# catid/tonk

Measured on AMD Instinct MI355X. Metric: Siamese FEC encode+decode GiB/s (device-resident), 1/2/4/8 MI355X, higher is better.
Workload: dtype u8

## Files before the change

### tonk_amd/csrc/decoder.cpp

```cpp
#include "decoder.h"
#include "prof.h"

#include <algorithm>
#include <stdlib.h>
#include <string.h>

namespace tamd {

static const size_t kMergeAbove = 48;

static inline uint32_t popcount64(uint64_t x) { return (uint32_t)__builtin_popcountll(x); }

static inline uint32_t bits_popcount(uint64_t w, uint32_t start, uint32_t end) {
    if (start >= end) return 0;
    const uint32_t n = end - start;
    const uint64_t mask = n >= 64 ? ~0ull : ((1ull << n) - 1);
    return popcount64((w >> start) & mask);
}
static inline uint32_t bits_first_clear(uint64_t w, uint32_t start) {
    const uint64_t v = (~w) >> start;
    if (start >= 64 || v == 0) return 64;
    return start + (uint32_t)__builtin_ctzll(v);
}
static inline uint32_t bits_first_set(uint64_t w, uint32_t start) {
    const uint64_t v = w >> start;
    if (start >= 64 || v == 0) return 64;
    return start + (uint32_t)__builtin_ctzll(v);
}

Decoder::Decoder(Context* ctx, uint32_t row_bytes, HostRelease release, void* user)
    : ctx_(ctx), row_bytes_(row_bytes), release_(release), user_(user) {
    ctx_->attach(this);
}

Decoder::~Decoder() {
    for (Subwindow* s : subs_) {
        for (unsigned i = 0; i < kSubwindow; ++i) drop_original(s->orig[i]);
        delete s;
    }
    subs_.clear();
    for (size_t i = 0; i < segs_.size(); ++i) release_segment(segs_[i], 0, segs_[i].count);
    segs_.clear();
    Recovery* r = head_;
    while (r) { Recovery* n = r->next; free_recovery(r); r = n; }
    for (Recovery* g : graveyard_) delete g;
    graveyard_.clear();
    for (Recovery* g : pool_) delete g;
    pool_.clear();
    pre_flush();
    for (unsigned l = 0; l < kLanes; ++l) lanes_[l].sums.release(ctx_->rows);
    ctx_->detach(this);
}

void Decoder::pre_flush() {
    for (unsigned l = 0; l < kLanes; ++l) lanes_[l].sums.flush(ctx_->rows, ctx_->pb, ctx_->ex);
}

void Decoder::drop_original(StoredOriginal& o) {
    if (o.owned) ctx_->rows.free_deferred(o.row);
    if (o.host && release_) release_(o.host, user_);
    o.row = kNoRow;
    o.bytes = 0;
    o.owned = 0;
    o.host = nullptr;
    o.run = 0;
}

void Decoder::free_recovery(Recovery* r) {
    if (r->row != kNoRow) ctx_->rows.free_deferred(r->row);
    r->row = kNoRow;
    graveyard_.push_back(r);
}

void Decoder::read_original(RowId row, uint32_t len, uint8_t coef, Sym& out) const {
    ctx_->ex.append(ctx_->rows, row, len, coef, out);
}

void Decoder::release_segment(const Segment& s, uint32_t from, uint32_t n) {
    if (s.owned)
        for (uint32_t j = from; j < from + n; ++j) ctx_->rows.free_deferred(s.row(j));
}

void Decoder::append(uint32_t e0, const RowId* rows, uint32_t k, uint32_t framed_bytes, uint32_t header_bytes,
                     uint8_t owned, uint64_t layout) {
    const RowTable& rt = ctx_->rows;
    uint32_t e = e0, col = to_column(e0);
    if (k >= 2 && col + k - 1 < kColumnPeriod && col != 0 && (layout || consecutive_handles(rows, k))) {
        const uint32_t o0 = layout ? (uint32_t)(layout >> 32) : rt.offset(rows[0]);
        const uint32_t o1 = layout ? o0 + (uint32_t)layout : rt.offset(rows[1]);
        const uint32_t stride = o1 - o0;
        if (o1 > o0 && (layout || rt.affine(rows[0], k, stride))) {
            Segment* last = segs_.empty() ? nullptr : &segs_.back();
            const bool cont = last && last->end() == e0 + base_ && last->bytes == framed_bytes &&
                              last->header_bytes == header_bytes && last->owned == owned &&
                              rows[0] == last->row0 + last->count && o0 > last->off0 &&
                              (last->count == 1 ? o0 - last->off0 == stride
                                                : last->stride == stride && o0 == last->off(last->count));
            if (cont) {
                last->stride = stride;
                last->count += k;
            } else {
                Segment sg;
                sg.first = e0 + base_;
                sg.count = k;
                sg.row0 = rows[0];
                sg.off0 = o0;
                sg.stride = stride;
                sg.bytes = framed_bytes;
                sg.column0 = col;
                sg.header_bytes = (uint8_t)header_bytes;
                sg.owned = owned;
                segs_.push_back(sg);
            }
            const uint32_t id = seg_base_ + (uint32_t)segs_.size() - 1;
            for (uint32_t x = e0; x < e0 + k;) {
                const uint32_t bit = x % kSubwindow;
                const uint32_t n = std::min(kSubwindow - bit, e0 + k - x);
                std::fill_n(subs_[x / kSubwindow]->seg + bit, n, id);
                x += n;
            }
            return;
        }
    }
    uint32_t j = 0;
    while (j < k) {
        Segment* last = segs_.empty() ? nullptr : &segs_.back();
        const uint32_t e_abs = e + base_;
        const RowId r = rows[j];
        const uint32_t off = rt.offset(r);
        const bool cont = last && last->end() == e_abs && last->bytes == framed_bytes &&
                          last->header_bytes == header_bytes && last->owned == owned && r == last->row0 + last->count &&
                          off > last->off0 && col != 0 && (last->count == 1 || off == last->off(last->count));
        if (cont) {
            if (last->count == 1) last->stride = off - last->off0;
            ++last->count;
        } else {
            Segment sg;
            sg.first = e_abs;
            sg.count = 1;
            sg.row0 = r;
            sg.off0 = off;
            sg.bytes = framed_bytes;
            sg.column0 = col;
            sg.header_bytes = (uint8_t)header_bytes;
            sg.owned = owned;
            segs_.push_back(sg);
            last = &segs_.back();
        }
        const uint32_t id = seg_base_ + (uint32_t)segs_.size() - 1;
        subs_[e / kSubwindow]->seg[e % kSubwindow] = id;
        ++e;
        ++j;
        col = col_inc(col);
        if (last->count >= 2) {
            uint32_t n = last->count;
            while (j < k && rows[j] == last->row0 + n && col != 0 && rt.offset(rows[j]) == last->off(n)) {
                subs_[e / kSubwindow]->seg[e % kSubwindow] = id;
                ++e;
                ++j;
                ++n;
                col = col_inc(col);
            }
            last->count = n;
        }
    }
}


bool Decoder::mark_got(uint32_t column) {
    const uint32_t e = to_element(column);
    if (invalid_element(e)) { disabled_ = true; return false; }
    Subwindow* s = subs_[e / kSubwindow];
    s->got_count++;
    s->got |= 1ull << (e % kSubwindow);
    return e == next_expected_;
}

uint32_t Decoder::range_lost(uint32_t start, uint32_t end) {
    if (start >= end) return 0;
    uint32_t lost = 0;
    uint32_t sub = start / kSubwindow;
    const uint32_t bit = start % kSubwindow;
    if (bit > 0) {
        uint32_t bit_end = bit + end - start;
        if (bit_end > kSubwindow) bit_end = kSubwindow;
        lost += (bit_end - bit) - bits_popcount(subs_[sub]->got, bit, bit_end);
        ++sub;
    }
    const uint32_t sub_end = end / kSubwindow;
    for (uint32_t i = sub; i < sub_end; ++i) lost += kSubwindow - subs_[i]->got_count;
    if (sub_end >= sub) {
        const uint32_t last_bits = end - sub_end * kSubwindow;
        if (last_bits > 0) lost += last_bits - bits_popcount(subs_[sub_end]->got, 0, last_bits);
    }
    return lost;
}

uint32_t Decoder::find_next_lost(uint32_t start) {
    if (start >= count_) return count_;
    const uint32_t sub_end = (count_ + kSubwindow - 1) / kSubwindow;
    uint32_t sub = start / kSubwindow, bit = start % kSubwindow;
    while (sub < sub_end) {
        if (subs_[sub]->got_count < kSubwindow) {
            bit = bits_first_clear(subs_[sub]->got, bit);
            if (bit < kSubwindow) {
                uint32_t e = sub * kSubwindow + bit;
                if (e > count_) e = count_;
                return e;
            }
        }
        bit = 0;
        ++sub;
    }
    return count_;
}

uint32_t Decoder::find_next_got(uint32_t start) {
    if (start >= count_) return count_;
    const uint32_t sub_end = (count_ + kSubwindow - 1) / kSubwindow;
    uint32_t sub = start / kSubwindow, bit = start % kSubwindow;
    while (sub < sub_end) {
        if (subs_[sub]->got_count > 0) {
            bit = bits_first_set(subs_[sub]->got, bit);
            if (bit < kSubwindow) {
                uint32_t e = sub * kSubwindow + bit;
                if (e > count_) e = count_;
                return e;
            }
        }
        bit = 0;
        ++sub;
    }
    return count_;
}

void Decoder::iterate_next_expected(uint32_t start) {
    if (next_expected_ >= count_) return;
    next_expected_ = find_next_lost(start);
}

bool Decoder::grow_window(uint32_t end) {
    const uint32_t needed = (end + kLanes + kSubwindow - 1) / kSubwindow;
    while (subs_.size() < needed) subs_.push_back(new Subwindow());
    if (end > count_) count_ = end;
    return true;
}

Result Decoder::add_original(uint32_t packet_num, RowId row, uint32_t framed_bytes, uint32_t header_bytes,
                             uint32_t payload_bytes, void* host, bool* took, bool borrowed) {
    *took = false;
    if (disabled_) return kDisabled;
    const uint32_t e = to_element(packet_num);
    if (col_delta_negative(e)) {
        stats_[6]++;
        return kDuplicateData;
    }
    const bool at_end = e >= count_;
    grow_window(e + 1);
    Subwindow* s = subs_[e / kSubwindow];
    const uint32_t bit = e % kSubwindow;
    if ((s->got >> bit) & 1u) {
        stats_[6]++;
        return kDuplicateData;
    }
    if (at_end && !host) {
        append(e, &row, 1, framed_bytes, header_bytes, borrowed ? 0 : 1);
    } else {
        StoredOriginal& o = s->orig[bit];
        drop_original(o);
        o.row = row;
        o.off = ctx_->rows.offset(row);
        o.bytes = framed_bytes;
        o.column = packet_num;
        o.header_bytes = (uint8_t)header_bytes;
        o.owned = borrowed ? 0 : 1;
        o.host = host;
        o.run = 0;
        o.stride = 0;
        if (o.owned || host) s->held |= 1ull << bit;
        s->singles |= 1ull << bit;
    }
    *took = !borrowed;
    s->got_count++;
    s->got |= 1ull << bit;

    if (e == next_expected_) {
        iterate_next_expected(e + 1);
        list_delete_before(next_expected_);
    }
    if (e >= cr_.element_start && e < cr_.next_check_start) checked_reset();

    stats_[0]++;
    stats_[1] += payload_bytes;
    return kSuccess;
}

bool Decoder::add_run_inorder(uint32_t col0, const RowId* rows, uint32_t k, uint32_t framed_bytes,
                              uint32_t header_bytes, uint32_t payload_bytes, bool borrowed, uint64_t layout) {
    if (disabled_ || has_recovered_ || !k) return false;
    const uint32_t e0 = to_element(col0);
    if (col_delta_negative(e0) || e0 < count_) return false;
    if (head_ && (next_expected_ >= e0 || check_recovery_possible())) return false;
    grow_window(e0 + k);
    append(e0, rows, k, framed_bytes, header_bytes, borrowed ? 0 : 1, layout);
    for (uint32_t e = e0; e < e0 + k;) {
        const uint32_t bit = e % kSubwindow;
        const uint32_t n = std::min(kSubwindow - bit, e0 + k - e);
        Subwindow* s = subs_[e / kSubwindow];
        s->got |= (n == 64 ? ~0ull : ((1ull << n) - 1)) << bit;
        s->got_count += n;
        e += n;
    }
    if (e0 == next_expected_) next_expected_ = find_next_lost(e0 + k);
    if (std::max(e0, cr_.element_start) < std::min(e0 + k, cr_.next_check_start)) checked_reset();
    stats_[0] += k;
    stats_[1] += (uint64_t)payload_bytes * k;
    return true;
}

bool Decoder::plug_sum_holes(uint32_t element_start) {
    for (uint32_t column : recovered_columns_) {
        const uint32_t e = to_element(column);
        if (invalid_element(e)) continue;
        const uint32_t lane = column % kLanes;
        const uint32_t lane_start = next_lane_element(element_start, lane);
        LaneSum& sum = lanes_[lane];
        if (e >= lane_start && e < sum.element_end) {
            const StoredOriginal& o = elem(e);
            if (o.bytes <= 0) return false;
            sum.sums.grow(o.bytes);
            sum.sums.accumulate(ctx_->rows, o.row, o.bytes, column);
        }
    }
    recovered_columns_.clear();
    return true;
}

void Decoder::reset_sums(uint32_t element_start) {
    for (unsigned l = 0; l < kLanes; ++l) {
        const uint32_t ls = next_lane_element(element_start, l);
        LaneSum& sum = lanes_[l];
        sum.element_start = ls;
        sum.element_end = ls;
        sum.sums.reset(ctx_->rows);
    }
    recovered_columns_.clear();
}

bool Decoder::start_sums(uint32_t element_start, uint32_t buffer_bytes) {
    for (unsigned l = 0; l < kLanes; ++l) {
        const uint32_t ls = next_lane_element(element_start, l);
        LaneSum& sum = lanes_[l];
        if (sum.sums.bytes == 0) {
            sum.element_end = ls;
        } else if (sum.element_start != ls) {
            sum.element_end = ls;
            sum.sums.reset(ctx_->rows);
        }
        sum.element_start = ls;
        sum.sums.grow(buffer_bytes);
    }
    if (!recovered_columns_.empty() && !plug_sum_holes(element_start)) return false;
    return true;
}

LaneSums& Decoder::get_lane(uint32_t lane, uint32_t element_end) {
    LaneSum& sum = lanes_[lane];
    uint32_t e = sum.element_end;
    if (e >= element_end) return sum.sums;
    do {
        const uint32_t id = seg_id(e);
        if (id != kSingle) {
            const Segment& sg = segs_[id - seg_base_];
            const uint32_t j = e + base_ - sg.first;
            uint32_t stop = sg.end() - base_;
            if (stop > element_end) stop = element_end;
            const uint32_t n = (stop - 1 - e) / kLanes + 1;
            sum.sums.grow(sg.bytes);
            sum.sums.accumulate_run_level0(sg.row(j), sg.off(j), sg.bytes, col_add(sg.column0, j), n, sg.stride * kLanes);
            e += n * kLanes;
            continue;
        }
        const StoredOriginal& o = elem(e);
        if (o.bytes > 0) {
            sum.sums.grow(o.bytes);
            if (ctx_->rows.level(o.row) == 0) sum.sums.accumulate_level0(o.row, ctx_->rows.offset(o.row), o.bytes, o.column);
            else sum.sums.accumulate(ctx_->rows, o.row, o.bytes, o.column);
        }
        e += kLanes;
    } while (e < element_end);
    sum.element_end = e;
    return sum.sums;
}

void Decoder::list_walk(ListWalk& w) const {
    w.min_start = ~0u;
    w.max_bytes = 0;
    w.seen_sum = false;
    w.target_start = w.target_count = 0;
    w.min_fse = ~0u;
    w.invalid = false;
    for (const Recovery* r = head_; r; r = r->next) {
        const uint32_t sc = r->meta.SumCount, cs = r->meta.ColumnStart;
        if (sc > kCauchyThreshold) {
            if (!w.seen_sum) {
                w.target_start = cs;
                w.target_count = sc;
                w.target_end = r->element_end;
                w.seen_sum = true;
            } else if (cs != w.target_start || sc < w.target_count) {
                const uint32_t fse = to_element(cs);
                if (invalid_element(fse)) {
                    w.invalid = true;
                    return;
                }
                if (w.min_fse > fse) w.min_fse = fse;
            }
        }
        if (w.min_start > r->element_start) w.min_start = r->element_start;
        if (w.max_bytes < r->bytes) w.max_bytes = r->bytes;
    }
}

void Decoder::remove_elements() {
    if (next_expected_ < kRemoveThreshold) return;

    uint32_t first_kept = 0, target_start = 0, target_count = 0, initial_bytes = 0;
    bool seen_sum = false;
    const Recovery* r = head_;
    if (!r) {
        const RecoveryMeta m = last_meta_;
        const uint32_t end = to_element(m.ColumnStart + m.SumCount);
        if (col_delta_negative(end) || end < m.LDPCCount) { disabled_ = true; return; }
        first_kept = end - m.LDPCCount;
        target_start = m.ColumnStart;
        target_count = m.SumCount;
        initial_bytes = last_bytes_;
        if (m.SumCount > kCauchyThreshold) seen_sum = true;
    } else {
        if (!(walk_.valid && walk_.gen == list_gen_ && walk_.column_start == column_start_ && walk_.count == count_)) {
            list_walk(walk_);
            walk_.valid = true;
            walk_.gen = list_gen_;
            walk_.column_start = column_start_;
            walk_.count = count_;
        }
        if (walk_.invalid) { disabled_ = true; return; }
        first_kept = walk_.min_start < walk_.min_fse ? walk_.min_start : walk_.min_fse;
        initial_bytes = walk_.max_bytes;
        seen_sum = walk_.seen_sum;
        target_start = walk_.target_start;
        target_count = walk_.target_count;
    }
    if (first_kept < kRemoveThreshold) return;

    const uint32_t first_kept_sub = first_kept / kSubwindow;
    const uint32_t removed = first_kept_sub * kSubwindow;

    if (seen_sum) {
        uint32_t sum_elem = to_element(target_start);
        if (sum_column_start_ != target_start || sum_column_count_ > target_count) {
            if (invalid_element(sum_elem)) { disabled_ = true; return; }
            reset_sums(sum_elem);
            sum_column_start_ = target_start;
            sum_column_count_ = target_count;
        } else {
            if (invalid_element(sum_elem)) sum_elem = 0;
            if (!start_sums(sum_elem, initial_bytes)) { disabled_ = true; return; }
        }
        for (unsigned l = 0; l < kLanes; ++l) {
            get_lane(l, removed);
            LaneSum& sum = lanes_[l];
            if (sum.element_start >= removed) sum.element_start -= removed;
            else sum.element_start = l;
            sum.element_end -= removed;
        }
    } else {
        sum_column_count_ = 0;
    }

    for (uint32_t i = 0; i < first_kept_sub; ++i) {
        Subwindow* s = subs_[i];
        for (uint64_t m = s->held; m; m &= m - 1) drop_original(s->orig[__builtin_ctzll(m)]);
        for (uint64_t m = s->singles | s->held; m; m &= m - 1)
            memset((void*)&s->orig[__builtin_ctzll(m)], 0, sizeof(StoredOriginal));
        memset(s->seg, 0xff, sizeof(s->seg));
        s->got = 0;
        s->got_count = 0;
        s->held = 0;
        s->singles = 0;
    }
    std::rotate(subs_.begin(), subs_.begin() + first_kept_sub, subs_.end());
    const uint32_t cut = base_ + removed;
    while (!segs_.empty() && segs_.front().end() <= cut) {
        release_segment(segs_.front(), 0, segs_.front().count);
        segs_.pop_front(1);
        ++seg_base_;
    }
    if (!segs_.empty() && segs_.front().first < cut) {
        Segment& f = segs_.front();
        const uint32_t d = cut - f.first;
        release_segment(f, 0, d);
        f.first = cut;
        f.count -= d;
        f.row0 += d;
        f.off0 += d * f.stride;
        f.column0 = col_add(f.column0, d);
    }
    base_ = cut;

    count_ -= removed;
    column_start_ = to_column(removed);
    next_expected_ -= removed;

    ++list_gen_;
    for (Recovery* q = head_; q; q = q->next) {
        q->element_end -= removed;
        q->element_start -= removed;
    }
    checked_decrement(removed);
    prev_next_check_start_ = prev_next_check_start_ > removed ? prev_next_check_start_ - removed : 0;
}


void Decoder::list_insert(Recovery* rec, bool out_of_order) {
    Recovery* prev = tail_;
    Recovery* next = nullptr;
    const uint32_t rs = rec->meta.ColumnStart, re = rec->element_end;
    if (ins_gen_ == list_gen_ && ins_end_ == re && ins_start_ == rs) {
        next = ins_last_;
        prev = ins_last_->prev;
    } else {
        for (; prev; next = prev, prev = prev->prev) {
            const uint32_t ps = prev->meta.ColumnStart, pe = prev->element_end;
            if (re >= pe) {
                if (re > pe) break;
                if (col_delta_negative(col_sub(rs, ps))) break;
            }
        }
    }
    const uint32_t sc = rec->meta.SumCount;
    const bool is_sum = sc > kCauchyThreshold;
    const bool same_target = is_sum && walk_.seen_sum && rs == walk_.target_start && sc == walk_.target_count;
    const bool walk_kept = walk_.valid && walk_.gen == list_gen_ && walk_.column_start == column_start_ &&
                           walk_.count == count_ &&
                           (!is_sum || !walk_.seen_sum || same_target || re > walk_.target_end);
    ins_last_ = rec;
    ins_end_ = re;
    ins_start_ = rs;
    ins_gen_ = ++list_gen_;
    if (walk_kept) {
        if (is_sum && !walk_.seen_sum) {
            walk_.seen_sum = true;
            walk_.target_start = rs;
            walk_.target_count = sc;
            walk_.target_end = re;
        } else if (is_sum && !same_target && (rs != walk_.target_start || sc < walk_.target_count)) {
            const uint32_t fse = to_element(rs);
            if (invalid_element(fse)) walk_.invalid = true;
            else if (walk_.min_fse > fse) walk_.min_fse = fse;
        }
        if (walk_.min_start > rec->element_start) walk_.min_start = rec->element_start;
        if (walk_.max_bytes < rec->bytes) walk_.max_bytes = rec->bytes;
        walk_.gen = list_gen_;
    }
    rec->next = next;
    rec->prev = prev;
    if (prev) prev->next = rec; else head_ = rec;
    if (next) next->prev = rec; else tail_ = rec;
    if (!prev || next) checked_reset();
    ++recovery_count_;
    if (!out_of_order) {
        last_meta_ = rec->meta;
        last_bytes_ = rec->bytes;
    }
}

void Decoder::lazy_write() {
    Recovery* r = lazy_from_;
    for (uint32_t i = 0; i < lazy_n_ && r; ++i, r = r->next) r->lost_count = lazy_lost_;
    lazy_n_ = 0;
    lazy_from_ = nullptr;
}

void Decoder::list_delete_before(uint32_t element) {
    if (lazy_n_) lazy_write();
    ++list_gen_;
    Recovery* r = head_;
    uint32_t deleted = 0;
    while (r) {
        if (r->element_end > element) break;
        Recovery* n = r->next;
        free_recovery(r);
        ++deleted;
        r = n;
    }
    head_ = r;
    if (r) {
        r->prev = nullptr;
        recovery_count_ -= deleted;
    } else {
        tail_ = nullptr;
        recovery_count_ = 0;
    }
}

void Decoder::checked_reset() {
    cr_ = Checked();
    lazy_n_ = 0;
    lazy_from_ = nullptr;
    matrix_reset();
    for (Recovery* r : graveyard_) pool_.push_back(r);
    graveyard_.clear();
}

void Decoder::checked_decrement(uint32_t n) {
    if (cr_.element_start < n || cr_.next_check_start < n) {
        checked_reset();
        return;
    }
    cr_.element_start -= n;
    cr_.next_check_start -= n;
}


void Decoder::matrix_reset() {
    mcols_.clear();
    mrows_.clear();
    pivots_.clear();
    mat_rows_ = mat_cols_ = 0;
    prev_next_check_start_ = 0;
    ge_resume_pivot_ = 0;
}

bool Decoder::matrix_resize(uint32_t rows, uint32_t cols, bool keep) {
    if (keep && rows <= mat_alloc_rows_ && cols <= mat_stride_) {
        mat_rows_ = rows;
        mat_cols_ = cols;
        return true;
    }
    const uint32_t arows = rows + 4;
    const uint32_t acols = (cols + 4 + 31) & ~31u;
    std::vector<uint8_t> m((size_t)arows * acols, 0);
    if (keep && mat_cols_ > 0) {
        const uint32_t copy = mat_cols_ < cols ? mat_cols_ : cols;
        for (uint32_t i = 0; i < mat_rows_; ++i)
            memcpy(&m[(size_t)i * acols], &mat_[(size_t)i * mat_stride_], copy);
    }
    mat_.swap(m);
    mat_alloc_rows_ = arows;
    mat_stride_ = acols;
    mat_rows_ = rows;
    mat_cols_ = cols;
    return true;
}

void Decoder::populate_columns(uint32_t old_cols, uint32_t new_cols) {
    if (old_cols >= new_cols) return;
    mcols_.resize(new_cols);
    uint32_t start = prev_next_check_start_;
    prev_next_check_start_ = cr_.next_check_start;
    const uint32_t end = cr_.next_check_start;
    if (start < cr_.element_start) start = cr_.element_start;
    const uint32_t sub_end = (end + kSubwindow - 1) / kSubwindow;
    uint32_t sub = start / kSubwindow, bit = start % kSubwindow, column = old_cols;
    while (sub < sub_end) {
        Subwindow* s = subs_[sub];
        if (s->got_count < kSubwindow) {
            do {
                bit = bits_first_clear(s->got, bit);
                if (bit >= kSubwindow) break;
                const uint32_t e = sub * kSubwindow + bit;
                MatCol& c = mcols_[column];
                c.column = to_column(e);
                c.orig = &s->orig[bit];
                c.cx = column_value(c.column);
                c.orig->column = column;
                s->singles |= 1ull << bit;
                if (++column >= new_cols) return;
            } while (++bit < kSubwindow);
        }
        bit = 0;
        ++sub;
    }
    disabled_ = true;
}

void Decoder::populate_rows(uint32_t old_rows, uint32_t new_rows) {
    if (old_rows >= new_rows) return;
    mrows_.resize(new_rows);
    Recovery* r = old_rows > 0 ? mrows_[old_rows - 1].rec->next : cr_.first;
    for (uint32_t i = old_rows; i < new_rows; ++i, r = r->next) {
        mrows_[i].rec = r;
        mrows_[i].used = false;
        mrows_[i].mcols = r->lost_count;
    }
}

bool Decoder::generate_matrix() {
    if (lazy_n_) lazy_write();
    const uint32_t columns = cr_.lost_count;
    const uint32_t rows = cr_.recovery_count;
    uint32_t old_rows = (uint32_t)mrows_.size();
    uint32_t old_cols = (uint32_t)mcols_.size();
    if (rows < old_rows || columns < old_cols) {
        matrix_reset();
        old_rows = old_cols = 0;
    }
    matrix_resize(rows, columns, old_rows != 0);
    populate_columns(old_cols, columns);
    populate_rows(old_rows, rows);
    if (disabled_) return false;

    const uint32_t start_row = columns <= old_cols ? old_rows : 0;
    for (uint32_t i = start_row; i < rows; ++i) {
        Recovery* rec = mrows_[i].rec;
        const RecoveryMeta m = rec->meta;
        const uint32_t start_col = i < old_rows ? old_cols : 0;
        if (m.SumCount <= kCauchyThreshold) {
            for (uint32_t j = start_col; j < columns; ++j) {
                const uint32_t column = mcols_[j].column;
                const uint32_t e = col_sub(column, m.ColumnStart);
                if (e >= m.SumCount) {
                    for (; j < columns; ++j) mat(i, j) = 0;
                    break;
                }
                mat(i, j) = m.Row == 0 ? 1 : cauchy_element(m.Row - 1, column % kCauchyMaxColumns);
            }
            continue;
        }
        const uint8_t rx = row_value(m.Row);
        for (uint32_t j = start_col; j < columns; ++j) {
            const uint32_t column = mcols_[j].column;
            const uint32_t e = col_sub(column, m.ColumnStart);
            if (e >= m.SumCount) {
                for (; j < columns; ++j) mat(i, j) = 0;
                break;
            }
            const uint8_t cx = mcols_[j].cx, cx2 = gf_sqr(cx);
            const unsigned op = row_opcode(column % kLanes, m.Row);
            uint8_t v = 0;
            if (op & 1) v ^= 1;
            if (op & 2) v ^= cx;
            if (op & 4) v ^= cx2;
            if (op & 8) v ^= rx;
            if (op & 16) v ^= gf_mul(cx, rx);
            if (op & 32) v ^= gf_mul(cx2, rx);
            mat(i, j) = v;
        }
        Pcg32 prng;
        prng.seed(m.Row, m.LDPCCount);
        const uint32_t es = rec->element_start;
        const uint32_t pairs = (m.LDPCCount + kPairRate - 1) / kPairRate;
        const FastMod ldpc_mod(m.LDPCCount);
        for (uint32_t k = 0; k < pairs; ++k) {
            const uint32_t e1 = es + ldpc_mod(prng.next());
            if (!got(e1)) {
                const uint32_t mc = elem(e1).column;
                if (mc >= columns) { disabled_ = true; return false; }
                if (mc >= start_col) mat(i, mc) ^= 1;
            }
            const uint32_t erx = es + ldpc_mod(prng.next());
            if (!got(erx)) {
                const uint32_t mc = elem(erx).column;
                if (mc >= columns) { disabled_ = true; return false; }
                if (mc >= start_col) mat(i, mc) ^= rx;
            }
        }
    }
    pivots_.resize(rows);
    for (uint32_t i = old_rows; i < rows; ++i) pivots_[i] = i;
    if (ge_resume_pivot_ > 0) resume_ge(old_rows, rows);
    return true;
}

bool Decoder::eliminate_row(uint32_t ge_row, uint32_t rem_row, uint32_t pivot_i, uint32_t column_end, uint8_t val_i) {
    uint8_t* rem = &mat_[(size_t)rem_row * mat_stride_];
    const uint8_t* ge = &mat_[(size_t)ge_row * mat_stride_];
    const uint8_t val_j = rem[pivot_i];
    if (val_j == 0) return false;
    const uint8_t y = gf_div(val_j, val_i);
    rem[pivot_i] = y;
    const uint8_t* ymul = g_gf.mul[y];
    for (uint32_t c = pivot_i + 1; c < column_end; ++c) rem[c] ^= ymul[ge[c]];
    return true;
}

void Decoder::resume_ge(uint32_t old_rows, uint32_t rows) {
    if (old_rows >= rows) return;
    for (uint32_t pi = 0; pi < ge_resume_pivot_; ++pi) {
        const uint32_t ri = pivots_[pi];
        const uint8_t val_i = mat(ri, pi);
        const uint32_t pcc = mrows_[ri].mcols;
        for (uint32_t nr = old_rows; nr < rows; ++nr) {
            if (eliminate_row(ri, nr, pi, pcc, val_i)) {
                if (mrows_[nr].mcols < pcc) mrows_[nr].mcols = pcc;
            }
        }
    }
}

bool Decoder::gaussian_elimination() {
    if (ge_resume_pivot_ > 0) return pivoted_ge(ge_resume_pivot_);
    const uint32_t columns = mat_cols_, rows = mat_rows_;
    for (uint32_t pi = 0; pi < columns; ++pi) {
        const uint8_t val_i = mat(pi, pi);
        if (val_i == 0) return pivoted_ge(pi);
        mrows_[pi].used = true;
        const uint32_t pcc = mrows_[pi].mcols;
        for (uint32_t pj = pi + 1; pj < rows; ++pj) eliminate_row(pi, pj, pi, pcc, val_i);
    }
    return true;
}

bool Decoder::pivoted_ge(uint32_t pivot_i) {
    const uint32_t columns = mat_cols_, rows = mat_rows_;
    uint32_t pj = pivot_i + 1;
    bool resume = true;
    for (; pivot_i < columns; ++pivot_i) {
        if (!resume) pj = pivot_i;
        resume = false;
        bool found = false;
        for (; pj < rows; ++pj) {
            const uint32_t rj = pivots_[pj];
            const uint8_t val_i = mat(rj, pivot_i);
            if (val_i == 0) continue;
            if (pivot_i != pj) std::swap(pivots_[pivot_i], pivots_[pj]);
            mrows_[rj].used = true;
            const uint32_t pcc = mrows_[rj].mcols;
            if (pivot_i >= columns - 1) return true;
            for (uint32_t pk = pivot_i + 1; pk < rows; ++pk) {
                const uint32_t rk = pivots_[pk];
                if (eliminate_row(rj, rk, pivot_i, pcc, val_i)) {
                    if (mrows_[rk].mcols < pcc) mrows_[rk].mcols = pcc;
                }
            }
            found = true;
            break;
        }
        if (!found) {
            ge_resume_pivot_ = pivot_i;
            return false;
        }
    }
    return true;
}


Result Decoder::add_recovery(RowId row, uint32_t total_bytes, const uint8_t* tail, const uint8_t* host,
                             bool* took) {
    *took = false;
    if (disabled_) return kDisabled;
    RecoveryMeta m;
    const uint32_t tl = total_bytes < 8 ? total_bytes : 8;
    const int footer = get_recovery_footer(tail, tl, m);
    if (footer < 0) { disabled_ = true; return kDisabled; }

    stats_[2]++;
    stats_[3] += total_bytes;

    const bool out_of_order = col_delta_negative(m.ColumnStart + m.SumCount - latest_column_);
    if (!out_of_order) latest_column_ = (m.ColumnStart + m.SumCount) % kColumnPeriod;

    uint32_t es, ee;
    if (count_ <= 0) {
        if (out_of_order) { stats_[9]++; return kSuccess; }
        column_start_ = m.ColumnStart;
        grow_window(m.SumCount);
        ee = m.SumCount;
        es = ee - m.LDPCCount;
    } else {
        ee = to_element(m.ColumnStart + m.SumCount);
        if (col_delta_negative(ee)) { stats_[9]++; return kSuccess; }
        if (ee < m.LDPCCount) { stats_[9]++; return kSuccess; }
        es = ee - m.LDPCCount;
        if (ee <= next_expected_) {
            if (out_of_order) { stats_[9]++; return kSuccess; }
            if (es >= kRemoveThreshold) {
                last_meta_ = m;
                last_bytes_ = total_bytes - (uint32_t)footer;
                remove_elements();
            }
            stats_[9]++;
            return kSuccess;
        }
        if (m.SumCount > kCauchyThreshold) {
            if (sum_column_count_ == 0 || sum_column_start_ != m.ColumnStart) {
                if (invalid_element(to_element(m.ColumnStart))) { stats_[9]++; return kSuccess; }
            }
        }
        grow_window(ee);
    }

    if (m.SumCount == 1) {
        if (!add_single_recovery(row, total_bytes - (uint32_t)footer, host, m, took)) {
            disabled_ = true;
            return kDisabled;
        }
        return kSuccess;
    }

    Recovery* r;
    if (!pool_.empty()) {
        r = pool_.back();
        pool_.pop_back();
        r->next = r->prev = nullptr;
        r->lost_count = 0;
        r->buf.clear();
    } else {
        r = new Recovery();
    }
    r->bytes = total_bytes - (uint32_t)footer;
    r->row = row;
    *took = true;
    r->buf.push_back(Term{row, r->bytes, 1});
    r->meta = m;
    r->element_start = es;
    r->element_end = ee;
    list_insert(r, out_of_order);
    if (es >= kRemoveThreshold) remove_elements();
    return kSuccess;
}

bool Decoder::add_single_recovery(RowId row, uint32_t data_bytes, const uint8_t* host,
                                  const RecoveryMeta& m, bool* took) {
    const uint32_t e = to_element(m.ColumnStart);
    if (invalid_element(e)) return false;
    if (got(e)) return true;
    StoredOriginal& o = elem(e);

    uint32_t header = 0, payload = 0;
    if (host) {
        unsigned len = 0;
        const int hb = get_length_header(host, data_bytes, len);
        if (hb < 1 || len == 0 || len + (unsigned)hb != data_bytes) return false;
        header = (uint32_t)hb;
        payload = len;
    }
    drop_original(o);
    o.row = row;
    o.off = ctx_->rows.offset(row);
    o.bytes = data_bytes;
    o.column = m.ColumnStart;
    o.header_bytes = (uint8_t)header;
    o.owned = 1;
    o.run = 0;
    o.stride = 0;
    subs_[e / kSubwindow]->held |= 1ull << (e % kSubwindow);
    subs_[e / kSubwindow]->singles |= 1ull << (e % kSubwindow);
    *took = true;

    if (!has_recovered_) {
        has_recovered_ = true;
        recovered_.clear();
    }
    RecoveredPacket rp;
    rp.packet_num = m.ColumnStart;
    rp.row = row;
    rp.framed_upper = data_bytes;
    rp.header_bytes = header;
    rp.data_bytes = payload;
    recovered_.push_back(rp);
    recovered_columns_.push_back(m.ColumnStart);

    if (e >= cr_.element_start && e < cr_.next_check_start) checked_reset();

    if (mark_got(m.ColumnStart)) {
        iterate_next_expected(e + 1);
        list_delete_before(next_expected_);
        if (cr_.next_check_start >= kRemoveThreshold) remove_elements();
    }
    return true;
}

bool Decoder::check_recovery_possible() {
    if (disabled_) return false;
    Recovery* r;
    uint32_t next_check, rcount, lost;
    if (!cr_.last) {
        r = head_;
        if (!r) return false;
        cr_.first = r;
        cr_.element_start = r->element_start;
        rcount = 1;
        next_check = r->element_end;
        lost = range_lost(r->element_start, next_check);
        cr_.solve_failed = false;
        r->lost_count = lost;
    } else {
        rcount = cr_.recovery_count;
        lost = cr_.lost_count;
        if (rcount >= lost && !cr_.solve_failed) return lost <= kMaxLossRecovery;
        r = cr_.last;
        next_check = cr_.next_check_start;
    }
    while ((rcount < lost || cr_.solve_failed) && r->next) {
        r = r->next;
        ++rcount;
        uint32_t ee = r->element_end;
        if (ee < next_check) ee = next_check;
        lost += range_lost(next_check, ee);
        next_check = ee;
        r->lost_count = lost;
        cr_.solve_failed = false;
    }
    cr_.last = r;
    cr_.recovery_count = rcount;
    cr_.lost_count = lost;
    cr_.next_check_start = next_check;
    if (lost > kMaxLossRecovery) return false;
    return rcount >= lost && !cr_.solve_failed;
}

Result Decoder::is_ready() {
    if (has_recovered_ || check_recovery_possible()) return kSuccess;
    return kNeedMoreData;
}

Result Decoder::decode(std::vector<RecoveredPacket*>& out) {
    if (disabled_) return kDisabled;
    if (has_recovered_) {
        has_recovered_ = false;
        for (RecoveredPacket& p : recovered_) out.push_back(&p);
        return kSuccess;
    }
    if (!check_recovery_possible()) return kNeedMoreData;

    Recovery* r = cr_.last;
    uint32_t next_check = cr_.next_check_start, rcount = cr_.recovery_count, lost = cr_.lost_count;
    bool failed = false;
    for (;;) {
        if (rcount >= lost) {
            if (failed) {
                stats_[8]++;
            } else {
                const Result res = decode_checked_region();
                if (res == kSuccess) {
                    for (RecoveredPacket& p : recovered_) out.push_back(&p);
                    return kSuccess;
                }
                if (res != kNeedMoreData) return res;
                failed = true;
            }
        }
        if (!r->next) break;
        if (failed && cr_.first == head_ && tail_->element_end <= next_check && !lazy_n_) {
            const uint32_t rest = recovery_count_ - rcount;
            stats_[8] += rest;
            lazy_from_ = r->next;
            lazy_n_ = rest;
            lazy_lost_ = lost;
            rcount += rest;
            r = tail_;
            break;
        }
        r = r->next;
        ++rcount;
        uint32_t ee = r->element_end;
        if (ee < next_check) ee = next_check;
        lost += range_lost(next_check, ee);
        r->lost_count = lost;
        next_check = ee;
    }
    cr_.last = r;
    cr_.next_check_start = next_check;
    cr_.recovery_count = rcount;
    cr_.lost_count = lost;
    return kNeedMoreData;
}

Result Decoder::decode_checked_region() {
    {
        TAMD_PROF_SCOPE(kGenMatrix);
        if (!generate_matrix()) { disabled_ = true; return kDisabled; }
    }
    bool solved;
    {
        TAMD_PROF_SCOPE(kGE);
        solved = gaussian_elimination();
    }
    if (!solved) {
        cr_.solve_failed = true;
        stats_[8]++;
        return kNeedMoreData;
    }
    {
        TAMD_PROF_SCOPE(kElim);
        if (!eliminate_original_data()) { disabled_ = true; return kDisabled; }
    }
    {
        TAMD_PROF_SCOPE(kLowerTri);
        if (!multiply_lower_triangle()) { disabled_ = true; return kDisabled; }
    }
    Result res;
    {
        TAMD_PROF_SCOPE(kBackSub);
        res = back_substitution();
    }
    checked_reset();
    return res;
}

bool Decoder::eliminate_original_data() {
    const uint32_t rows = cr_.recovery_count;
    drun_valid_ = false;
    for (uint32_t ri = 0; ri < rows; ++ri) {
        if (!mrows_[ri].used) continue;
        Recovery* rec = mrows_[ri].rec;
        const RecoveryMeta m = rec->meta;
        const uint32_t es = rec->element_start, ee = rec->element_end;
        Sym& buf = rec->buf;

        if (m.SumCount <= kCauchyThreshold) {
            const uint32_t mode = m.Row == 0 ? TAMD_R_CONST : TAMD_R_CAUCHY;
            const uint32_t param = m.Row == 0 ? 1u : m.Row - 1;
            for (uint32_t j = es; j < ee; ++j) {
                const uint32_t id = seg_id(j);
                if (id != kSingle) {
                    const Segment& sg = segs_[id - seg_base_];
                    const uint32_t k = j + base_ - sg.first;
                    const uint32_t n = std::min(sg.end() - base_, ee) - j;
                    if (n >= 2) {
                        const uint32_t add = std::min(sg.bytes, rec->bytes);
                        buf.push_back(ctx_->pb.run_term(mode, param, sg.off(k), sg.stride, n, to_column(j), add));
                        j += n - 1;
                        continue;
                    }
                }
                RowId row;
                uint32_t add;
                if (!packet(j, row, add)) continue;
                if (add > rec->bytes) add = rec->bytes;
                const uint8_t y = m.Row == 0 ? 1 : cauchy_element(m.Row - 1, to_column(j) % kCauchyMaxColumns);
                read_original(row, add, y, buf);
            }
        } else {
            const uint32_t rbytes = rec->bytes;
            uint32_t sum_elem = to_element(m.ColumnStart);
            const bool sum_valid = !invalid_element(sum_elem);
            {
            TAMD_PROF_SCOPE(kElimStart);
            if (m.ColumnStart != sum_column_start_ || m.SumCount < sum_column_count_) {
                if (invalid_element(sum_elem)) return false;
                reset_sums(sum_elem);
                sum_column_start_ = m.ColumnStart;
            } else {
                if (invalid_element(sum_elem)) sum_elem = 0;
                if (!start_sums(sum_elem, rbytes)) return false;
            }
            }
            sum_column_count_ = m.SumCount;
            if (sum_valid && ctx_->direct_elim && eliminate_direct(rec, sum_elem, buf)) {
                if (ctx_->oom) return false;
                if (cr_.lost_count == 1) {
                    if (buf.size() > kMergeAbove) sym_merge(buf);
                    continue;
                }
                TAMD_PROF_SCOPE(kElimFold);
                const RowId p = fold_low_levels(ctx_->rows, ctx_->pb, buf, 3, rec->bytes, row_bytes_);
                if (p != kNoRow) ctx_->temps.push_back(p);
                continue;
            }

            const uint8_t rx = row_value(m.Row);
            {
            TAMD_PROF_SCOPE(kElimSums);
            for (unsigned l = 0; l < kLanes; ++l) {
                const unsigned op = row_opcode(l, m.Row);
                if (!op) continue;
                LaneSums& c = get_lane(l, ee);
                const uint32_t n = c.bytes < rbytes ? c.bytes : rbytes;
                if (!n) continue;
                uint8_t k[3];
                opcode_coefs(op, rx, k);
                c.read(ctx_->rows, ctx_->ex, buf, k, n, &ctx_->pb, ctx_->short_scans);
            }
            }
            TAMD_PROF_SCOPE(kElimPairs);
            Pcg32 prng;
            prng.seed(m.Row, m.LDPCCount);
            const uint32_t pairs = (m.LDPCCount + kPairRate - 1) / kPairRate;
            const FastMod ldpc_mod(m.LDPCCount);
            for (uint32_t i = 0; i < pairs; ++i) {
                RowId row;
                uint32_t b;
                const uint32_t e1 = es + ldpc_mod(prng.next());
                if (packet(e1, row, b)) read_original(row, b < rbytes ? b : rbytes, 1, buf);
                const uint32_t erx = es + ldpc_mod(prng.next());
                if (packet(erx, row, b)) read_original(row, b < rbytes ? b : rbytes, rx, buf);
            }
        }
        if (ctx_->oom) return false;
        if (cr_.lost_count == 1) {
            if (buf.size() > kMergeAbove) sym_merge(buf);
            continue;
        }
        TAMD_PROF_SCOPE(kElimFold);
        const RowId p = fold_low_levels(ctx_->rows, ctx_->pb, buf, 3, rec->bytes, row_bytes_);
        if (p != kNoRow) ctx_->temps.push_back(p);
    }
    return !disabled_ && !ctx_->oom;
}

bool Decoder::eliminate_direct(Recovery* rec, uint32_t sum_elem, Sym& buf) {
    const RecoveryMeta m = rec->meta;
    const uint32_t es = rec->element_start, ee = rec->element_end;
    if (ee <= sum_elem || ee - sum_elem > Encoder::kDirectMax || ee > count_) return false;
    TAMD_PROF_SCOPE(kElimSums);
    const uint32_t rbytes = rec->bytes;
    if (!drun_valid_ || drun_start_ != sum_elem || drun_end_ < ee) {
        drun_.clear();
        for (uint32_t j = sum_elem; j < ee;) {
            const uint32_t id = seg_id(j);
            if (id != kSingle) {
                const Segment& sg = segs_[id - seg_base_];
                const uint32_t k = j + base_ - sg.first;
                const uint32_t stop = std::min(sg.end() - base_, ee);
                if (sg.bytes) drun_.push_back(DirectRun{j, stop - j, sg.off(k), sg.stride, sg.bytes,
                                                        col_add(sg.column0, k), kNoRow});
                j = stop;
                continue;
            }
            const StoredOriginal& o = elem(j);
            if (o.bytes > 0) drun_.push_back(DirectRun{j, 0, 0, 0, o.bytes, to_column(j), o.row});
            ++j;
        }
        drun_valid_ = true;
        drun_start_ = sum_elem;
        drun_end_ = ee;
    }
    size_t nrec = drun_.size();
    while (nrec && drun_[nrec - 1].e0 >= ee) --nrec;
    if (nrec * Encoder::kDirectMinRun > ee - sum_elem) return false;
    druns_.clear();
    for (size_t i = 0; i < nrec; ++i) {
        const DirectRun& r = drun_[i];
        if (r.n) druns_.push_back(DenseRun{r.off, r.stride, std::min(r.n, ee - r.e0), std::min(r.len, rbytes), r.col,
                                           r.e0 - sum_elem});
    }
    const uint8_t rx = row_value(m.Row);
    auto loose_pair = [&](uint64_t pr) {
        RowId row;
        uint32_t b;
        if (packet((uint32_t)(pr >> 8), row, b)) read_original(row, b < rbytes ? b : rbytes, (uint8_t)pr, buf);
    };
    draw_dense_pairs(m.Row, m.LDPCCount, rx, es - sum_elem, sum_elem, druns_.data(), druns_.size(), dkeys_, dpairs_);
    const uint32_t span0 = nrec ? drun_[0].e0 : 0u;
    const uint32_t span1 = nrec ? drun_[nrec - 1].e0 + (drun_[nrec - 1].n ? std::min(drun_[nrec - 1].n, ee - drun_[nrec - 1].e0) : 1u) : 0u;
    {
        size_t keep = 0;
        for (uint64_t pr : dpairs_) {
            const uint32_t e = (uint32_t)(pr >> 8);
            if (e >= span0 && e < span1) dpairs_[keep++] = pr;
            else loose_pair(pr);
        }
        dpairs_.resize(keep);
        sort_pair_keys(dpairs_);
    }
    uint64_t ops = 0;
    uint8_t lk[kLanes][3];
    for (unsigned l = 0; l < kLanes; ++l) {
        const unsigned op = row_opcode(l, m.Row);
        ops |= (uint64_t)op << (6 * l);
        opcode_coefs(op, rx, lk[l]);
    }
    const uint32_t split = ctx_->dense_split;
    const bool chunked = split && ee - sum_elem > split;
    ProgramBuilder& pb = ctx_->pb;
    if (chunked) dparts_.assign((ee - sum_elem + split - 1) / split, kNoRow);
    uint32_t chunk = ~0u;
    size_t pi = 0, ki = 0;
    for (size_t i = 0; i < nrec; ++i) {
        const DirectRun& r = drun_[i];
        while (pi < dpairs_.size() && (uint32_t)(dpairs_[pi] >> 8) < r.e0) loose_pair(dpairs_[pi++]);
        if (!r.n) {
            const uint8_t* k = lk[r.col % kLanes];
            const uint8_t cx = column_value(r.col);
            const uint8_t c = (uint8_t)(k[0] ^ gf_mul(k[1], cx) ^ gf_mul(k[2], gf_sqr(cx)));
            if (c) read_original(r.row, std::min(r.len, rbytes), c, buf);
            continue;
        }
        const uint32_t a = r.e0 - sum_elem, end = a + std::min(r.n, ee - r.e0);
        if (!chunked) {
            const size_t k0 = ki;
            while (ki < dkeys_.size() && (dkeys_[ki] >> 8) < end) ++ki;
            buf.push_back(pb.dense_run_term(r.off, r.stride, end - a, r.col, ops, rx, dkeys_.data() + k0,
                                            (uint32_t)(ki - k0), a, std::min(r.len, rbytes)));
            continue;
        }
        for (uint32_t c = a / split; c * split < end; ++c) {
            if (c == chunk) continue;
            if (chunk != ~0u) buf.push_back(Term{dparts_[chunk], rbytes, 1});
            const RowId part = ctx_->alloc_temp(rbytes);
            if (part == kNoRow) return true;
            dparts_[c] = part;
            chunk = c;
        }
    }
    if (chunk != ~0u) {
        buf.push_back(Term{dparts_[chunk], rbytes, 1});
        const ProgramBuilder::DenseTarget t{ops, rx, ee - sum_elem, dkeys_.data(), (uint32_t)dkeys_.size(), kNoRow,
                                            dparts_.data(), (uint32_t)dparts_.size(), nullptr, 0, nullptr, 0};
        pb.emit_dense_range(druns_.data(), druns_.size(), &t, 1, split, rbytes, true);
    }
    while (pi < dpairs_.size()) loose_pair(dpairs_[pi++]);
    return true;
}

bool Decoder::multiply_lower_triangle() {
    const uint32_t L = cr_.lost_count;
    tri_.assign((size_t)L * L, 0);
    tri_b_.resize(L);
    for (uint32_t i = 0; i < L; ++i) {
        tri_[(size_t)i * L + i] = 1;
        Recovery* r = mrows_[pivots_[i]].rec;
        if (L > 1) sym_merge(r->buf);
        tri_b_[i] = r->bytes;
    }
    for (uint32_t ci = 0; ci + 1 < L; ++ci) {
        const uint8_t* src = &tri_[(size_t)ci * L];
        for (uint32_t cj = ci + 1; cj < L; ++cj) {
            const uint8_t y = mat(pivots_[cj], ci);
            if (y == 0) continue;
            if (tri_b_[cj] < tri_b_[ci]) tri_b_[cj] = tri_b_[ci];
            uint8_t* dst = &tri_[(size_t)cj * L];
            const uint8_t* my = g_gf.mul[y];
            for (uint32_t k = 0; k <= ci; ++k)
                if (src[k]) dst[k] ^= my[src[k]];
        }
    }
    return true;
}

Result Decoder::back_substitution() {
    const uint32_t L = cr_.lost_count;
    recovered_.assign(L, RecoveredPacket());
    if (L == 1) return back_substitution_one();
    tri_clips_.assign(tri_b_.begin(), tri_b_.end());
    std::sort(tri_clips_.begin(), tri_clips_.end());
    tri_clips_.erase(std::unique(tri_clips_.begin(), tri_clips_.end()), tri_clips_.end());
    const uint32_t D = (uint32_t)tri_clips_.size();
    auto clip_index = [this](uint32_t len) {
        return (uint32_t)(std::lower_bound(tri_clips_.begin(), tri_clips_.end(), len) - tri_clips_.begin());
    };
    tri_groups_.clear();
    tri_gstart_.assign((size_t)L + 1, 0);
    std::vector<uint32_t>& gpos = tri_gstart_;
    std::vector<uint32_t> gend(L, 0);
    tri_acc_.resize((size_t)L * D);
    if (L >= ctx_->backsub_rows) {
        for (uint32_t k = 0; k < L; ++k) {
            Recovery* r = mrows_[pivots_[k]].rec;
            if (r->buf.size() <= 1) continue;
            const RowId row = ctx_->alloc_temp(r->bytes);
            if (row == kNoRow) { disabled_ = true; return kDisabled; }
            ctx_->pb.combine(row, r->buf.data(), r->buf.size(), r->bytes);
            r->buf.clear();
            r->buf.push_back(Term{row, r->bytes, 1});
        }
    }
    bool iterate = false;
    for (int ci = (int)L - 1; ci >= 0; --ci) {
        const uint32_t ri = pivots_[ci];
        const uint8_t y = mat(ri, (uint32_t)ci);
        if (y == 0) { disabled_ = true; return kDisabled; }
        const uint8_t inv_y = gf_inv(y);
        const uint32_t bytes = tri_b_[ci];
        const uint32_t bidx = clip_index(bytes);

        std::fill(tri_acc_.begin(), tri_acc_.end(), 0);
        const uint8_t* trow = &tri_[(size_t)ci * L];
        for (uint32_t k = 0; k <= (uint32_t)ci; ++k)
            if (trow[k]) tri_acc_[(size_t)k * D + bidx] ^= trow[k];
        for (uint32_t cj = ci + 1; cj < L; ++cj) {
            const uint8_t x = mat(ri, cj);
            if (x == 0) continue;
            const uint8_t* mx = g_gf.mul[x];
            for (uint32_t g = gpos[cj]; g < gend[cj]; ++g) {
                const Group& gr = tri_groups_[g];
                const uint32_t c = gr.clip < bidx ? gr.clip : bidx;
                tri_acc_[(size_t)gr.k * D + c] ^= mx[gr.coef];
            }
        }
        gpos[ci] = (uint32_t)tri_groups_.size();
        const uint8_t* my = g_gf.mul[inv_y];
        for (uint32_t k = 0; k < L; ++k)
            for (uint32_t c = 0; c < D; ++c) {
                const uint8_t a = tri_acc_[(size_t)k * D + c];
                if (a) tri_groups_.push_back(Group{k, c, my[a]});
            }
        gend[ci] = (uint32_t)tri_groups_.size();

        Sym& value = value_;
        value.clear();
        for (uint32_t g = gpos[ci]; g < gend[ci]; ++g) {
            const Group& gr = tri_groups_[g];
            sym_add(value, mrows_[pivots_[gr.k]].rec->buf, tri_clips_[gr.clip], gr.coef);
        }
        sym_merge(value);
        if (!store_recovered((uint32_t)ci, value, bytes, iterate)) return kDisabled;
    }
    return finish_solve(iterate);
}

Result Decoder::back_substitution_one() {
    const uint32_t ri = pivots_[0];
    const uint8_t y = mat(ri, 0);
    if (y == 0) { disabled_ = true; return kDisabled; }
    Recovery* rec = mrows_[ri].rec;
    Sym& value = value_;
    value.swap(rec->buf);
    sym_scale(value, gf_inv(y));
    bool iterate = false;
    if (!store_recovered(0, value, tri_b_[0], iterate)) return kDisabled;
    return finish_solve(iterate);
}

bool Decoder::store_recovered(uint32_t ci, Sym& value, uint32_t bytes, bool& iterate) {
    StoredOriginal* o = mcols_[ci].orig;
    const RowId out_row = ctx_->alloc(bytes);
    if (out_row == kNoRow) { disabled_ = true; return false; }
    ctx_->pb.combine(out_row, value.data(), value.size(), bytes);
    ctx_->ex.take(out_row, value);

    drop_original(*o);
    o->row = out_row;
    o->off = ctx_->rows.offset(out_row);
    o->bytes = bytes;
    o->column = mcols_[ci].column;
    o->header_bytes = 0;
    o->owned = 1;
    o->run = 0;
    o->stride = 0;
    {
        const uint32_t e = to_element(o->column);
        subs_[e / kSubwindow]->held |= 1ull << (e % kSubwindow);
        subs_[e / kSubwindow]->singles |= 1ull << (e % kSubwindow);
    }

    RecoveredPacket& rp = recovered_[ci];
    rp.packet_num = o->column;
    rp.row = out_row;
    rp.framed_upper = bytes;
    recovered_columns_.push_back(o->column);
    iterate |= mark_got(o->column);
    return true;
}

Result Decoder::finish_solve(bool iterate) {
    const uint32_t L = cr_.lost_count;
    for (uint32_t ci = 0; ci < L; ++ci) {
        Recovery* rec = mrows_[pivots_[ci]].rec;
        rec->buf.clear();
        rec->bytes = 0;
    }
    if (!iterate) { disabled_ = true; return kDisabled; }
    iterate_next_expected(cr_.next_check_start);
    list_delete_before(next_expected_);
    if (cr_.next_check_start >= kRemoveThreshold) remove_elements();
    stats_[7]++;
    return kSuccess;
}

void Decoder::set_recovered_length(uint32_t packet_num, uint32_t framed_bytes, uint32_t header_bytes, void* host) {
    const uint32_t e = to_element(packet_num);
    if (invalid_element(e) || seg_id(e) != kSingle) { if (host && release_) release_(host, user_); return; }
    StoredOriginal& o = elem(e);
    if (o.column != packet_num || o.bytes == 0) { if (host && release_) release_(host, user_); return; }
    o.bytes = framed_bytes;
    o.header_bytes = (uint8_t)header_bytes;
    if (o.host && release_) release_(o.host, user_);
    o.host = host;
}

Result Decoder::get(uint32_t packet_num, StoredOriginal** out, bool recovered_now) {
    *out = nullptr;
    if (disabled_ && !recovered_now) return kDisabled;
    const uint32_t e = to_element(packet_num);
    if (invalid_element(e)) return kNeedMoreData;
    const uint32_t id = seg_id(e);
    if (id != kSingle) {
        const Segment& sg = segs_[id - seg_base_];
        const uint32_t j = e + base_ - sg.first;
        view_ = StoredOriginal();
        view_.row = sg.row(j);
        view_.off = sg.off(j);
        view_.bytes = sg.bytes;
        view_.column = packet_num;
        view_.header_bytes = sg.header_bytes;
        *out = &view_;
        return kSuccess;
    }
    StoredOriginal& o = elem(e);
    if (o.bytes <= 0) return kNeedMoreData;
    *out = &o;
    return kSuccess;
}

Result Decoder::ack(uint8_t* buffer, uint32_t limit, uint32_t* used) {
    if (disabled_) return kDisabled;
    const uint32_t wc = count_;
    if (wc == 0) { *used = 0; return kNeedMoreData; }
    uint8_t* start = buffer;
    const uint32_t nee = next_expected_;
    const uint32_t hb = put_pnum_header(to_column(nee), buffer);
    buffer += hb;
    limit -= hb;
    if (invalid_element(nee)) {
        *used = (uint32_t)(buffer - start);
        stats_[4]++;
        stats_[5] += *used;
        return kSuccess;
    }
    uint32_t off = nee;
    while (limit >= kMaxLossRangeBytes) {
        const uint32_t rs = find_next_lost(off);
        if (rs >= wc) {
            if (wc >= off) buffer += put_nack_range(wc - off, 0, buffer);
            break;
        }
        const uint32_t re = find_next_got(rs + 1);
        const uint32_t n = put_nack_range(rs - off, re - rs - 1, buffer);
        off = re + 1;
        buffer += n;
        limit -= n;
    }
    *used = (uint32_t)(buffer - start);
    stats_[4]++;
    stats_[5] += *used;
    return kSuccess;
}

void Decoder::stats(uint64_t* out, unsigned n) {
    if (n > 11) n = 11;
    stats_[10] = ctx_->rows.bytes_in_use();
    for (unsigned i = 0; i < n; ++i) out[i] = stats_[i];
}

}
```

### tonk_amd/csrc/encoder.cpp

```cpp
#include "encoder.h"
#include "prof.h"

#include <algorithm>
#include <stdlib.h>
#include <string.h>
#include <time.h>

namespace tamd {

static uint64_t (*g_clock_fn)() = nullptr;
void set_clock_source(uint64_t (*fn)()) { g_clock_fn = fn; }

uint64_t time_msec() {
    if (g_clock_fn) return g_clock_fn();
    timespec ts;
    clock_gettime(CLOCK_REALTIME, &ts);
    return (uint64_t)ts.tv_sec * 1000u + (uint64_t)ts.tv_nsec / 1000000u;
}

Encoder::Encoder(Context* ctx, uint32_t row_bytes, HostRelease release, void* user)
    : ctx_(ctx), row_bytes_(row_bytes), release_(release), user_(user) {
    for (unsigned l = 0; l < kLanes; ++l) lanes_[l].next_abs = l;
    ctx_->attach(this);
}

Encoder::~Encoder() {
    pre_flush();
    drop_all();
    for (unsigned l = 0; l < kLanes; ++l) lanes_[l].sums.release(ctx_->rows);
    ctx_->detach(this);
}

void Encoder::release_segment(const Segment& s, uint32_t from, uint32_t n) {
    if (s.owned)
        for (uint32_t j = from; j < from + n; ++j) ctx_->rows.free_deferred(s.row(j));
    if (s.host && release_ && from == 0 && n == s.count) release_(s.host, user_);
}

void Encoder::drop_all() {
    if (held_)
        for (size_t i = 0; i < segs_.size(); ++i) release_segment(segs_[i], 0, segs_[i].count);
    held_ = 0;
    seg_base_ += (uint32_t)segs_.size();
    segs_.clear();
    win_.clear();
    base_ = 0;
}

StoredOriginal Encoder::view(uint32_t e) const {
    const Segment& s = seg_of(e);
    const uint32_t j = e + base_ - s.first;
    StoredOriginal o;
    o.row = s.row(j);
    o.bytes = s.bytes;
    o.column = to_column(e);
    o.send_msec = win_[e].send_msec;
    o.off = s.off(j);
    o.header_bytes = s.header_bytes;
    o.owned = s.owned;
    o.host = s.host;
    return o;
}

void Encoder::pre_flush() {
    emit_cauchy_group();
    emit_dense_group();
    for (unsigned l = 0; l < kLanes; ++l) lanes_[l].sums.flush(ctx_->rows, ctx_->pb, ctx_->ex);
}

void Encoder::append(const RowId* rows, uint32_t k, uint32_t framed_bytes, uint32_t header_bytes, uint8_t owned,
                     void* host, uint32_t now, uint64_t layout) {
    const RowTable& rt = ctx_->rows;
    uint32_t e_abs = base_ + (uint32_t)win_.size();
    uint32_t col = next_column_;
    win_.reserve_more(k);
    Slot* wb = win_.slot_base();
    const size_t mask = win_.slot_mask();
    size_t idx = win_.slot_index(win_.size());
    if (k >= 2 && !host && col + k - 1 < kColumnPeriod && col != 0 && (layout || consecutive_handles(rows, k))) {
        const uint32_t o0 = layout ? (uint32_t)(layout >> 32) : rt.offset(rows[0]);
        const uint32_t o1 = layout ? o0 + (uint32_t)layout : rt.offset(rows[1]);
        const uint32_t stride = o1 - o0;
        if (o1 > o0 && (layout || rt.affine(rows[0], k, stride))) {
            Segment* last = segs_.empty() ? nullptr : &segs_.back();
            const bool cont = last && !last->host && last->row0 != kNoRow && last->end() == e_abs &&
                              last->bytes == framed_bytes && last->header_bytes == header_bytes &&
                              last->owned == owned && rows[0] == last->row0 + last->count && o0 > last->off0 &&
                              (last->count == 1 ? o0 - last->off0 == stride
                                                : last->stride == stride && o0 == last->off(last->count));
            if (cont) {
                last->stride = stride;
                last->count += k;
            } else {
                Segment sg;
                sg.first = e_abs;
                sg.count = k;
                sg.row0 = rows[0];
                sg.off0 = o0;
                sg.stride = stride;
                sg.bytes = framed_bytes;
                sg.column0 = col;
                sg.header_bytes = (uint8_t)header_bytes;
                sg.owned = owned;
                segs_.push_back(sg);
                if (owned) ++held_;
            }
            const Slot v{seg_base_ + (uint32_t)segs_.size() - 1, now};
            for (uint32_t x = 0; x < k; ++x) wb[(idx + x) & mask] = v;
            win_.commit(k);
            return;
        }
    }
    uint32_t j = 0;
    while (j < k) {
        Segment* last = segs_.empty() ? nullptr : &segs_.back();
        const RowId r = rows[j];
        const uint32_t off = rt.offset(r);
        const bool cont = last && !host && !last->host && last->row0 != kNoRow && last->end() == e_abs &&
                          last->bytes == framed_bytes && last->header_bytes == header_bytes && last->owned == owned &&
                          r == last->row0 + last->count && off > last->off0 && col != 0 &&
                          (last->count == 1 || off == last->off(last->count));
        if (cont) {
            if (last->count == 1) last->stride = off - last->off0;
            ++last->count;
        } else {
            Segment sg;
            sg.first = e_abs;
            sg.count = 1;
            sg.row0 = r;
            sg.off0 = off;
            sg.bytes = framed_bytes;
            sg.column0 = col;
            sg.header_bytes = (uint8_t)header_bytes;
            sg.owned = owned;
            sg.host = host;
            segs_.push_back(sg);
            if (owned || host) ++held_;
            last = &segs_.back();
        }
        const uint32_t id = seg_base_ + (uint32_t)segs_.size() - 1;
        wb[idx] = Slot{id, now};
        idx = (idx + 1) & mask;
        ++e_abs;
        col = col_inc(col);
        ++j;
        if (last->count >= 2) {
            uint32_t n = last->count;
            while (j < k && rows[j] == last->row0 + n && col != 0 && rt.offset(rows[j]) == last->off(n)) {
                wb[idx] = Slot{id, now};
                idx = (idx + 1) & mask;
                ++n;
                ++j;
                col = col_inc(col);
            }
            e_abs += n - last->count;
            last->count = n;
        }
    }
    win_.commit(k);
}

Result Encoder::add(RowId row, uint32_t framed_bytes, uint32_t header_bytes, uint32_t payload_bytes,
                    void* host, uint32_t* packet_num, bool borrowed) {
    if (disabled_) return kDisabled;
    if (remaining_slots() <= 0) return kMaxPacketsReached;
    *packet_num = add_first(row, framed_bytes, header_bytes, payload_bytes, host, borrowed);
    return kSuccess;
}

uint32_t Encoder::add_first(RowId row, uint32_t framed_bytes, uint32_t header_bytes, uint32_t payload_bytes,
                            void* host, bool borrowed) {
    const uint32_t column = next_column_;
    const uint32_t now = (uint32_t)now_msec();
    if (count_ > 0) {
        ++count_;
    } else {
        start_new_window(column);
        const uint32_t element = column % kLanes;
        if (element) {
            Segment ph;
            ph.first = base_;
            ph.count = element;
            ph.column0 = column - element;
            segs_.push_back(ph);
            for (uint32_t e = 0; e < element; ++e)
                win_.push_back(Slot{seg_base_ + (uint32_t)segs_.size() - 1, placeholder_msec_[e]});
        }
    }
    append(&row, 1, framed_bytes, header_bytes, borrowed ? 0 : 1, host, now);
    next_column_ = col_inc(next_column_);
    Lane& lane = lanes_[column % kLanes];
    if (lane.longest < framed_bytes) lane.longest = framed_bytes;
    if (longest_ < framed_bytes) longest_ = framed_bytes;
    stats_[0]++;
    stats_[1] += payload_bytes;
    return column;
}

bool Encoder::add_run(const RowId* rows, uint32_t k, uint32_t framed_bytes, uint32_t header_bytes,
                      uint32_t payload_bytes, bool borrowed, uint32_t* first_col, uint64_t layout) {
    if (disabled_ || remaining_slots() < k || !k) return false;
    uint32_t skip = 0;
    if (count_ == 0) {
        *first_col = add_first(rows[0], framed_bytes, header_bytes, payload_bytes, nullptr, borrowed);
        if (k == 1) return true;
        skip = 1;
    } else {
        *first_col = next_column_;
    }
    const uint32_t m = k - skip;
    append(rows + skip, m, framed_bytes, header_bytes, borrowed ? 0 : 1, nullptr, (uint32_t)now_msec(),
           layout && skip ? layout + ((layout & 0xffffffffull) << 32) : layout);
    count_ += m;
    const uint32_t first = next_column_;
    next_column_ = col_add(next_column_, m);
    for (uint32_t j = 0; j < m && j < kLanes; ++j) {
        Lane& lane = lanes_[(first + j) % kLanes];
        if (lane.longest < framed_bytes) lane.longest = framed_bytes;
    }
    if (longest_ < framed_bytes) longest_ = framed_bytes;
    stats_[0] += m;
    stats_[1] += (uint64_t)payload_bytes * m;
    return true;
}

void Encoder::start_new_window(uint32_t column) {
    for (uint32_t e = 0; e < kLanes; ++e) placeholder_msec_[e] = e < win_.size() ? win_[e].send_msec : placeholder_msec_[e];
    ++window_gen_;
    drop_all();
    const uint32_t element = column % kLanes;
    column_start_ = column - element;
    sum_start_ = element;
    sum_end_ = element;
    first_unremoved_ = element;
    count_ = element + 1;
    longest_ = 0;
    for (unsigned l = 0; l < kLanes; ++l) lanes_[l].longest = 0;
}

void Encoder::remove_before(uint32_t first_kept_column) {
    if (disabled_) return;
    const uint32_t e = to_element(first_kept_column);
    if (e >= count_) {
        if (!col_delta_negative(e)) count_ = 0;
    } else if (first_unremoved_ < e) {
        first_unremoved_ = e;
    }
}

void Encoder::reset_sums(uint32_t element_start) {
    for (unsigned l = 0; l < kLanes; ++l) {
        lanes_[l].next_abs = base_ + next_lane_element(element_start, l);
        lanes_[l].sums.reset(ctx_->rows);
    }
    sum_start_ = element_start;
    sum_end_ = element_start;
    sum_column_start_ = to_column(element_start);
    sum_erased_ = 0;
    drop_segments_below(base_);
}

void Encoder::drop_segments_below(uint32_t drop) {
    while (!segs_.empty() && (int32_t)(segs_.front().end() - drop) <= 0) {
        const Segment& f = segs_.front();
        if (f.owned || f.host) {
            release_segment(f, 0, f.count);
            --held_;
        }
        segs_.pop_front(1);
        ++seg_base_;
    }
    if (!segs_.empty() && (int32_t)(segs_.front().first - drop) < 0) {
        Segment& f = segs_.front();
        const uint32_t d = drop - f.first;
        release_segment(f, 0, d);
        f.first = drop;
        f.count -= d;
        if (f.row0 != kNoRow) f.row0 += d;
        f.off0 += d * f.stride;
        f.column0 = col_add(f.column0, d);
    }
}

void Encoder::remove_elements() {
    TAMD_PROF_SCOPE(kEncRemove);
    const uint32_t first_kept_sub = first_unremoved_ / kSubwindow;
    const uint32_t removed = first_kept_sub * kSubwindow;

    const uint32_t cut = base_ + removed;
    uint32_t drop = cut;
    if (sum_end_ > sum_start_) {
        const uint32_t keep = sum_abs_start();
        if ((int32_t)(keep - drop) < 0) drop = keep;
        if (removed > sum_start_) sum_erased_ += removed - sum_start_;
        sum_end_ = sum_end_ > removed ? sum_end_ - removed : 0;
        sum_start_ = sum_start_ > removed ? sum_start_ - removed : 0;
    }

    drop_segments_below(drop);
    win_.pop_front(removed);
    base_ = cut;
    count_ -= removed;
    column_start_ = to_column(removed);
    first_unremoved_ -= removed;

    uint32_t longest = 0, lane_longest[kLanes] = {0, 0, 0, 0, 0, 0, 0, 0};
    if (first_unremoved_ < count_) {
        const uint32_t lo = base_ + first_unremoved_, hi = base_ + count_;
        for (uint32_t i = win_[first_unremoved_].seg - seg_base_; i < segs_.size(); ++i) {
            const Segment& sg = segs_[i];
            if (sg.first >= hi) break;
            const uint32_t a = sg.first > lo ? sg.first : lo, b = sg.end() < hi ? sg.end() : hi;
            if (a >= b || !sg.bytes) continue;
            if (longest < sg.bytes) longest = sg.bytes;
            for (uint32_t x = a; x < b && x < a + kLanes; ++x) {
                const uint32_t l = (x - base_) % kLanes;
                if (lane_longest[l] < sg.bytes) lane_longest[l] = sg.bytes;
            }
        }
    }
    longest_ = longest;
    for (unsigned l = 0; l < kLanes; ++l) lanes_[l].longest = lane_longest[l];

    if (sum_end_ <= sum_start_) reset_sums(first_unremoved_);
}

LaneSums& Encoder::get_lane(uint32_t lane_index, uint32_t element_end) {
    Lane& lane = lanes_[lane_index];
    LaneSums& sums = lane.sums;
    uint32_t a = lane.next_abs;
    const uint32_t end = base_ + element_end;
    if ((int32_t)(end - a) > 0) {
        if (lane.longest > 0) sums.grow(lane.longest);
        size_t si = seg_index_at(a);
        do {
            const Segment& sg = segs_[si];
            const uint32_t j = a - sg.first;
            const uint32_t stop = (int32_t)(sg.end() - end) < 0 ? sg.end() : end;
            const uint32_t n = (stop - 1 - a) / kLanes + 1;
            if (sg.bytes) {
                sums.grow(sg.bytes);
                sums.accumulate_run_level0(sg.row(j), sg.off(j), sg.bytes, col_add(sg.column0, j), n,
                                           sg.stride * kLanes);
            }
            a += n * kLanes;
            while (si + 1 < segs_.size() && (int32_t)(segs_[si].end() - a) <= 0) ++si;
        } while ((int32_t)(end - a) > 0);
        lane.next_abs = a;
    }
    return sums;
}


bool Encoder::on_ack_data(const uint8_t* data, uint32_t bytes) {
    unsigned next = 0;
    const int hb = get_pnum_header(data, (int)bytes, next);
    if (hb < 1) return false;
    data += hb;
    bytes -= (uint32_t)hb;

    if (col_delta_negative(col_sub(next, ack_.next_expected))) return true;

    if (ack_.next_expected == next && ack_.have_data && bytes == ack_.data_bytes &&
        (bytes == 0 || memcmp(data, ack_.data.data(), bytes) == 0))
        return true;

    ack_.next_expected = next;
    ack_.offset = 0;
    ack_.loss_column = next;
    ack_.loss_count = 0;
    ack_.data_bytes = bytes;
    if (bytes > 0) {
        ack_.data.assign(data, data + bytes);
        ack_.data.resize((size_t)bytes + 8, 0);
        ack_.have_data = true;
        if (!decode_next_range()) return false;
    }
    update_rto();
    remove_before(ack_.next_expected);
    return true;
}

void Encoder::rtt_update(uint32_t value, uint64_t now, uint64_t window) {
    auto* s = ack_.max_rtt;
    auto expired = [&](int i, uint64_t w) { return (uint64_t)(now - s[i].ts) > w; };
    if (s[0].value == 0 || value >= s[0].value || expired(2, window)) {
        s[0].value = s[1].value = s[2].value = value;
        s[0].ts = s[1].ts = s[2].ts = now;
        return;
    }
    if (value >= s[1].value) { s[1].value = s[2].value = value; s[1].ts = s[2].ts = now; }
    else if (value >= s[2].value) { s[2].value = value; s[2].ts = now; }
    if (expired(0, window)) {
        if (expired(1, window)) { s[0] = s[2]; s[1].value = value; s[1].ts = now; }
        else { s[0] = s[1]; s[1] = s[2]; }
        s[2].value = value;
        s[2].ts = now;
        return;
    }
    if (s[1].value == s[0].value && expired(1, window / 4)) {
        s[1].value = s[2].value = value;
        s[1].ts = s[2].ts = now;
        return;
    }
    if (s[2].value == s[1].value && expired(2, window / 2)) { s[2].value = value; s[2].ts = now; }
}

void Encoder::update_rto() {
    const uint32_t window_count = count_;
    uint32_t first_loss = to_element(ack_.next_expected);
    if (first_loss >= window_count) return;

    const uint64_t now64 = now_msec();
    const uint32_t now = (uint32_t)now64;
    uint32_t longest = 0;

    uint32_t element = to_element(ack_.next_rto_column);
    if (element >= window_count) element = first_unremoved_;

    for (; element < first_loss; ++element) {
        const int32_t d = (int32_t)(now - win_[element].send_msec);
        if ((uint32_t)d > longest && d > 0) longest = (uint32_t)d;
    }

    uint32_t remaining = ack_.data_bytes;
    const uint8_t* data = ack_.data.data();
    while (remaining > 0) {
        unsigned rel = 0, lossM1 = 0;
        const int n = get_nack_range(data, remaining + 8, rel, lossM1);
        if (n < 0 || n > (int)remaining) return;
        data += n;
        remaining -= (uint32_t)n;
        if (element + 1 < first_loss) element = first_loss - 1;
        first_loss += rel;
        for (; element < first_loss; ++element) {
            if (element >= window_count) return;
            const int32_t d = (int32_t)(now - win_[element].send_msec);
            if ((uint32_t)d > longest && d > 0) longest = (uint32_t)d;
        }
        first_loss += lossM1 + 2;
    }
    ack_.next_rto_column = to_column(element);
    if (longest <= 0) return;

    uint64_t window = (uint64_t)ack_.rto_msec * 2;
    if (window < 100) window = 100;
    else if (window > 4000) window = 4000;
    rtt_update(longest, now64, window);
    ack_.rto_msec = (ack_.max_rtt[0].value * 3) / 2;
    if (ack_.rto_msec < 20) ack_.rto_msec = 20;
}

bool Encoder::decode_next_range() {
    if (ack_.offset >= ack_.data_bytes) return false;
    unsigned rel = 0, lossM1 = 0;
    const int n = get_nack_range(ack_.data.data() + ack_.offset, ack_.data_bytes + 8 - ack_.offset, rel, lossM1);
    if (n < 0) return false;
    ack_.offset += (uint32_t)n;
    if (ack_.offset > ack_.data_bytes) return false;
    ack_.loss_column = col_add(ack_.loss_column, rel);
    ack_.loss_count = lossM1 + 1;
    return true;
}

bool Encoder::next_loss_column(uint32_t& column) {
    if (ack_.loss_count <= 0) {
        ack_.loss_column = col_inc(ack_.loss_column);
        if (!decode_next_range()) return false;
    }
    column = ack_.loss_column;
    ack_.loss_column = col_inc(ack_.loss_column);
    --ack_.loss_count;
    return true;
}

void Encoder::restart_loss_iterator() {
    ack_.offset = 0;
    ack_.loss_column = ack_.next_expected;
    ack_.loss_count = 0;
    decode_next_range();
}

Result Encoder::acknowledge(const uint8_t* data, uint32_t bytes, uint32_t* next_expected) {
    if (disabled_) return kDisabled;
    if (!on_ack_data(data, bytes)) return kInvalidInput;
    *next_expected = ack_.next_expected;
    stats_[6]++;
    stats_[7] += bytes;
    return kSuccess;
}

Result Encoder::attempt_retransmit(uint32_t e, StoredOriginal* out) {
    const StoredOriginal o = view(e);
    if (o.header_bytes == 0 || o.bytes <= o.header_bytes) { disabled_ = true; return kDisabled; }
    *out = o;
    stats_[4]++;
    stats_[5] += o.bytes - o.header_bytes;
    return kSuccess;
}

Result Encoder::retransmit(StoredOriginal* out) {
    if (disabled_) return kDisabled;
    if (unacked() == 0) {
        ack_.found_oldest = false;
        return kNeedMoreData;
    }
    const uint32_t first = col_sub(ack_.next_expected, column_start_);
    const uint32_t count = count_;
    if (col_delta_negative(first) || first < first_unremoved_ || first >= count) return kNeedMoreData;

    const uint32_t now = (uint32_t)now_msec();
    const uint32_t rto = ack_.rto_msec;

    if (ack_.found_oldest) {
        const uint32_t e = col_sub(ack_.oldest_column, column_start_);
        if (!col_delta_negative(e) && e >= first && e < count) {
            Slot& o = win_[e];
            if ((uint32_t)(now - o.send_msec) < rto) return kNeedMoreData;
            o.send_msec = now;
            ack_.found_oldest = false;
            return attempt_retransmit(e, out);
        }
        ack_.found_oldest = false;
    }

    uint32_t nack_element = first;
    uint32_t oldest = nack_element;
    uint32_t oldest_msec = win_[oldest].send_msec;
    if ((uint32_t)(now - oldest_msec) >= rto) {
        win_[oldest].send_msec = now;
        return attempt_retransmit(oldest, out);
    }

    if (ack_.data_bytes > 0) {
        restart_loss_iterator();
        uint32_t column = 0;
        while (next_loss_column(column)) {
            nack_element = to_element(column);
            if (nack_element >= count) break;
            Slot& o = win_[nack_element];
            const uint32_t last = o.send_msec;
            if ((uint32_t)(now - last) >= rto) {
                o.send_msec = now;
                return attempt_retransmit(nack_element, out);
            }
            if ((int32_t)(oldest_msec - last) > 0) { oldest = nack_element; oldest_msec = last; }
        }
    }

    for (uint32_t e = nack_element + 1; e < count; ++e) {
        Slot& o = win_[e];
        const uint32_t last = o.send_msec;
        if ((uint32_t)(now - last) >= rto) {
            o.send_msec = now;
            return attempt_retransmit(e, out);
        }
        if ((int32_t)(oldest_msec - last) > 0) { oldest = e; oldest_msec = last; }
    }
    ack_.found_oldest = true;
    ack_.oldest_column = to_column(oldest);
    return kNeedMoreData;
}

Result Encoder::get(uint32_t packet_num, StoredOriginal* out) {
    if (disabled_) return kDisabled;
    const uint32_t e = to_element(packet_num);
    if (e >= count_) return kNeedMoreData;
    const StoredOriginal o = view(e);
    if (o.bytes == 0) return kNeedMoreData;
    if (o.header_bytes == 0 || o.bytes <= o.header_bytes) { disabled_ = true; return kDisabled; }
    *out = o;
    return kSuccess;
}


Result Encoder::emit(Sym& terms, uint32_t len, const RecoveryMeta& meta, RecoveryOut& out, bool distinct) {
    TAMD_PROF_SCOPE(kEncEmit);
    if (!distinct) sym_merge(terms);
    out.meta = meta;
    out.footer_len = put_recovery_footer(meta, out.footer);
    out.data_len = len;
    out.row = ctx_->alloc(len + out.footer_len);
    if (out.row == kNoRow) { disabled_ = true; return kDisabled; }
    ctx_->pb.combine(out.row, terms.data(), terms.size(), len, out.footer, out.footer_len);
    stats_[2]++;
    stats_[3] += out.total();
    return kSuccess;
}

Result Encoder::generate_single(RecoveryOut& out) {
    const StoredOriginal o = view(first_unremoved_);
    RecoveryMeta m;
    m.SumCount = 1;
    m.LDPCCount = 1;
    m.ColumnStart = o.column;
    m.Row = 0;
    Sym& t = scratch_;
    t.clear();
    t.push_back(Term{o.row, o.bytes, 1});
    return emit(t, o.bytes, m, out, true);
}

Result Encoder::generate_cauchy(RecoveryOut& out) {
    TAMD_PROF_SCOPE(kEncCauchy);
    const uint32_t first = first_unremoved_;
    RecoveryMeta m;
    m.SumCount = unacked();
    m.LDPCCount = m.SumCount;
    m.ColumnStart = to_column(first);
    uint32_t mode, crow = 0;
    const uint32_t next_parity = to_element(next_parity_column_);
    if (next_parity <= first || col_delta_negative(next_parity)) {
        next_parity_column_ = col_add(m.ColumnStart, m.SumCount);
        m.Row = 0;
        mode = TAMD_R_CONST;
    } else {
        crow = next_cauchy_row_;
        m.Row = crow + 1;
        if (++next_cauchy_row_ >= kCauchyMaxRows) next_cauchy_row_ = 0;
        mode = TAMD_R_CAUCHY;
    }

    std::vector<Run>& runs = runs_;
    runs.clear();
    uint32_t used = 0;
    {
        const uint32_t lo = base_ + first, hi = base_ + count_;
        for (uint32_t i = win_[first].seg - seg_base_; i < segs_.size(); ++i) {
            const Segment& sg = segs_[i];
            if (sg.first >= hi) break;
            const uint32_t a = sg.first > lo ? sg.first : lo, b = sg.end() < hi ? sg.end() : hi;
            if (a >= b || !sg.bytes) continue;
            const uint32_t j = a - sg.first;
            if (used < sg.bytes) used = sg.bytes;
            runs.push_back(Run{sg.row(j), sg.off(j), sg.stride, b - a, sg.bytes, col_add(sg.column0, j)});
        }
    }

    out.meta = m;
    out.footer_len = put_recovery_footer(m, out.footer);
    out.data_len = used;
    out.row = ctx_->alloc(used + out.footer_len);
    if (out.row == kNoRow) { disabled_ = true; return kDisabled; }
    ctx_->rows.set_level(out.row, 1);
    const uint32_t max_group = 3;
    const uint32_t span = kGroupSpan;
    const uint32_t end_col = to_column(count_);
    const bool alone = count_ - first >= span || runs.size() * 4 > count_ - first;
    if (grp_n_ && (alone || grp_n_ >= max_group || grp_gen_ != window_gen_ ||
                   col_sub(end_col, grp_[0].first_col) >= span))
        emit_cauchy_group();
    grp_gen_ = window_gen_;
    CauchyTarget& t = grp_[grp_n_++];
    t.row = out.row;
    t.used = used;
    t.first_col = m.ColumnStart;
    t.end_col = end_col;
    t.kind = mode;
    t.param = mode == TAMD_R_CONST ? 1 : crow;
    t.flen = out.footer_len;
    memcpy(t.footer, out.footer, sizeof(t.footer));
    t.runs.swap(runs);
    if (alone) emit_cauchy_group();
    stats_[2]++;
    stats_[3] += out.total();
    return kSuccess;
}

void Encoder::emit_cauchy_group() {
    const uint32_t n = grp_n_;
    if (!n) return;
    grp_n_ = 0;
    ProgramBuilder& pb = ctx_->pb;
    pb.begin_op();
    if (n == 1) {
        const CauchyTarget& t = grp_[0];
        for (const Run& r : t.runs) {
            if (r.count == 1) {
                const uint8_t c = t.kind == TAMD_R_CONST ? 1 : cauchy_element(t.param, r.col % kCauchyMaxColumns);
                pb.op_acc(r.row, c, r.len);
            } else {
                pb.op_accr(t.kind, t.param, r.off, r.stride, r.count, r.len, r.col, 1);
            }
        }
        pb.finish_combine(t.row, t.used, t.footer, t.flen);
        return;
    }
    const uint32_t base = grp_[0].first_col;
    std::vector<Run>& u = grp_union_;
    u.clear();
    for (uint32_t a = 0; a < n; ++a) {
        const uint32_t stop = a + 1 < n ? col_sub(grp_[a + 1].first_col, base) : ~0u;
        for (const Run& r : grp_[a].runs) {
            const uint32_t at = col_sub(r.col, base);
            if (at >= stop) continue;
            Run c = r;
            if (at + c.count > stop) c.count = stop - at;
            u.push_back(c);
        }
    }
    for (const Run& r : u) {
        const uint32_t at = col_sub(r.col, base);
        uint32_t tw[3] = {0, 0, 0};
        for (uint32_t a = 0; a < n; ++a) {
            const uint32_t f = col_sub(grp_[a].first_col, base), e = col_sub(grp_[a].end_col, base);
            const uint32_t lo = f > at ? f - at : 0u;
            const uint32_t hi = e - at < r.count ? e - at : r.count;
            if (e > at && lo < hi) tw[a] = grp_[a].kind | grp_[a].param << 2 | lo << 10 | hi << 21;
        }
        if (tw[0] | tw[1] | tw[2]) pb.op_accr_multi(r.off, r.stride, r.count, r.len, r.col, 1, tw);
    }
    for (uint32_t a = 0; a < n; ++a) pb.op_store(grp_[a].row, grp_[a].used, a, grp_[a].footer, grp_[a].flen);
    pb.end_op(1);
}

void Encoder::add_dense(uint32_t row, uint32_t recovery_bytes, Sym& rec) {
    const uint8_t rx = row_value(row);
    for (unsigned l = 0; l < kLanes; ++l) {
        const unsigned op = row_opcode(l, row);
        if (!op) continue;
        LaneSums& c = get_lane(l, count_);
        const uint32_t n = c.bytes < recovery_bytes ? c.bytes : recovery_bytes;
        if (!n) continue;
        uint8_t k[3];
        opcode_coefs(op, rx, k);
        c.read(ctx_->rows, ctx_->ex, rec, k, n, nullptr, ctx_->short_scans);
    }
    sum_end_ = count_;
}

bool Encoder::defer_dense(uint32_t row, uint32_t recovery_bytes, const RecoveryOut& out) {
    const uint32_t max_group = 3;
    const uint32_t max_work = kDenseGroupWork;
    const uint32_t lo = sum_abs_start(), hi = base_ + count_;
    const uint32_t split = ctx_->dense_split;
    const uint32_t rows = split && hi - lo > split ? split : hi - lo;
    if (dgrp_n_ && (lo != dgrp_lo_ || recovery_bytes != dgrp_len_ || window_gen_ != dgrp_gen_ ||
                    rows * (dgrp_n_ + 1) > max_work))
        emit_dense_group();
    std::vector<DenseRun>& runs = dgrp_runs_;
    runs.clear();
    for (size_t i = seg_index_at(lo); i < segs_.size(); ++i) {
        const Segment& sg = segs_[i];
        if ((int32_t)(sg.first - hi) >= 0) break;
        const uint32_t a = (int32_t)(sg.first - lo) > 0 ? sg.first : lo;
        const uint32_t b = (int32_t)(sg.end() - hi) < 0 ? sg.end() : hi;
        if ((int32_t)(b - a) <= 0 || !sg.bytes) continue;
        const uint32_t j = a - sg.first;
        runs.push_back(DenseRun{sg.off(j), sg.stride, b - a, sg.bytes < recovery_bytes ? sg.bytes : recovery_bytes,
                                col_add(sg.column0, j), a - lo});
    }
    if (!dgrp_n_) {
        dgrp_lo_ = lo;
        dgrp_len_ = recovery_bytes;
        dgrp_gen_ = window_gen_;
    }
    DenseTarget& t = dgrp_[dgrp_n_];
    t.row = out.row;
    t.ops = 0;
    for (unsigned l = 0; l < kLanes; ++l) t.ops |= (uint64_t)row_opcode(l, row) << (6 * l);
    t.rx = row_value(row);
    t.hi = hi - lo;
    t.flen = out.footer_len;
    memcpy(t.footer, out.footer, sizeof(t.footer));
    {
        TAMD_PROF_SCOPE(kEncLight);
        const uint32_t start = base_ + first_unremoved_;
        draw_dense_pairs(row, sum_end_ - first_unremoved_, t.rx, start - lo, lo, runs.data(), runs.size(), t.pairs,
                         pairs_);
        sort_pair_keys(pairs_);
        t.loose.clear();
        for (uint64_t pr : pairs_) {
            const uint32_t e = (uint32_t)(pr >> 8);
            const Segment& sg = seg_of(e - base_);
            t.loose.push_back(Term{sg.row(e - sg.first), sg.bytes, (uint8_t)(pr & 0xffu)});
        }
    }
    const uint32_t chunks = split && t.hi > split ? (t.hi + split - 1) / split : 1u;
    t.parts.clear();
    for (uint32_t c = 1; chunks > 1 && c <= chunks; ++c) {
        const RowId pr = ctx_->alloc_temp(recovery_bytes);
        if (pr == kNoRow) return false;
        t.parts.push_back(pr);
    }
    ctx_->rows.set_level(out.row, chunks > 1 ? 2 : 1);
    if (++dgrp_n_ >= max_group) emit_dense_group();
    return true;
}

void Encoder::emit_dense_group() {
    const uint32_t n = dgrp_n_;
    if (!n) return;
    dgrp_n_ = 0;
    ProgramBuilder::DenseTarget tg[3];
    for (uint32_t a = 0; a < n; ++a) {
        const DenseTarget& d = dgrp_[a];
        tg[a] = ProgramBuilder::DenseTarget{d.ops, d.rx, d.hi, d.pairs.data(), (uint32_t)d.pairs.size(), d.row,
                                            d.parts.empty() ? nullptr : d.parts.data(), (uint32_t)d.parts.size(),
                                            d.loose.data(), (uint32_t)d.loose.size(), d.footer, d.flen};
    }
    ctx_->pb.emit_dense_range(dgrp_runs_.data(), dgrp_runs_.size(), tg, n, ctx_->dense_split, dgrp_len_, false);
}

void Encoder::add_light(uint32_t row, Sym& rec) {
    const uint32_t start = first_unremoved_;
    const uint32_t count = sum_end_ - start;
    const uint8_t rx = row_value(row);
    Pcg32 prng;
    prng.seed(row, count);
    const uint32_t pairs = (count + kPairRate - 1) / kPairRate;
    const size_t at = rec.size();
    rec.resize(at + 2 * (size_t)pairs);
    Term* t = rec.data() + at;
    const FastMod mod(count);
    for (uint32_t i = 0; i < pairs; ++i) {
        const uint32_t e1 = start + mod(prng.next());
        const uint32_t erx = start + mod(prng.next());
        const Segment& s1 = seg_of(e1);
        const Segment& srx = seg_of(erx);
        t[2 * i] = Term{s1.row(e1 + base_ - s1.first), s1.bytes, 1};
        t[2 * i + 1] = Term{srx.row(erx + base_ - srx.first), srx.bytes, rx};
    }
}

bool Encoder::direct_sums() const {
    const uint32_t range = count_ + sum_erased_ - sum_start_;
    bool direct = range <= kDirectMax;
    if (direct && range) direct = (segs_.size() - seg_index_at(sum_abs_start())) * kDirectMinRun <= range;
    return direct;
}

bool Encoder::encode_is_quiet() const {
    if (disabled_ || count_ <= 0 || first_unremoved_ >= kRemoveThreshold) return false;
    const uint32_t un = unacked();
    if (un == 1) return true;
    const uint32_t ub = count_ - sum_start_ + sum_erased_;
    if (sum_end_ <= sum_start_ || ub >= kMaxPackets) return un <= kCauchyThreshold;
    if (un <= kSumResetThreshold || ub <= kCauchyThreshold) return true;
    if (direct_sums()) return true;
    for (unsigned l = 0; l < kLanes; ++l)
        if ((int32_t)(base_ + count_ - lanes_[l].next_abs) > 0 || !lanes_[l].sums.idle()) return false;
    return true;
}

Result Encoder::encode(RecoveryOut& out) {
    out = RecoveryOut();
    if (disabled_) return kDisabled;
    if (count_ <= 0) return kNeedMoreData;
    if (first_unremoved_ >= kRemoveThreshold) remove_elements();

    const uint32_t un = unacked();
    if (un == 1) return generate_single(out);

    const uint32_t ub = count_ - sum_start_ + sum_erased_;
    if (sum_end_ <= sum_start_ || ub >= kMaxPackets) {
        if (un <= kCauchyThreshold) return generate_cauchy(out);
        reset_sums(first_unremoved_);
    } else if (un <= kSumResetThreshold || ub <= kCauchyThreshold) {
        sum_end_ = sum_start_;
        return generate_cauchy(out);
    }

    const uint32_t row = next_row_;
    if (++next_row_ >= kRowPeriod) next_row_ = 0;

    const uint32_t recovery_bytes = longest_;
    Sym& rec = rec_;
    rec.clear();
    const bool direct = direct_sums();
    if (!direct) {
        TAMD_PROF_SCOPE(kEncDense);
        add_dense(row, recovery_bytes, rec);
    } else {
        sum_end_ = count_;
    }
    if (!direct) {
        TAMD_PROF_SCOPE(kEncLight);
        add_light(row, rec);
    }

    RecoveryMeta m;
    m.SumCount = sum_end_ - sum_start_ + sum_erased_;
    m.LDPCCount = un;
    m.ColumnStart = sum_column_start_;
    m.Row = row;
    if (direct) {
        out.meta = m;
        out.footer_len = put_recovery_footer(m, out.footer);
        out.data_len = recovery_bytes;
        out.row = ctx_->alloc(recovery_bytes + out.footer_len);
        if (out.row == kNoRow) { disabled_ = true; return kDisabled; }
        if (!defer_dense(row, recovery_bytes, out)) {
            disabled_ = true;
            ctx_->rows.free_deferred(out.row);
            out = RecoveryOut();
            return kDisabled;
        }
        stats_[2]++;
        stats_[3] += out.total();
        return kSuccess;
    }
    return emit(rec, recovery_bytes, m, out, true);
}

void Encoder::stats(uint64_t* out, unsigned n) {
    if (n > 9) n = 9;
    stats_[8] = ctx_->rows.bytes_in_use();
    for (unsigned i = 0; i < n; ++i) out[i] = stats_[i];
}

}
```

### tonk_amd/csrc/encoder.h

```cpp
#pragma once

#include <stdio.h>

#include "engine.h"
#include "ring.h"
#include "serial.h"

#include <stdint.h>

namespace tamd {

enum Result {
    kSuccess = 0, kInvalidInput = 1, kNeedMoreData = 2, kMaxPacketsReached = 3,
    kDuplicateData = 4, kDisabled = 5
};

struct RecoveryOut {
    RowId row = kNoRow;
    uint32_t data_len = 0;
    uint32_t footer_len = 0;
    uint8_t footer[8] = {0, 0, 0, 0, 0, 0, 0, 0};
    RecoveryMeta meta;
    uint32_t total() const { return data_len + footer_len; }
};

struct StoredOriginal {
    RowId row = kNoRow;
    uint32_t bytes = 0;
    uint32_t column = 0;
    uint32_t send_msec = 0;
    uint32_t off = 0;
    uint32_t stride = 0;
    uint16_t run = 0;
    uint8_t header_bytes = 0;
    uint8_t owned = 0;
    void* host = nullptr;
};

typedef void (*HostRelease)(void* host, void* user);

inline bool consecutive_handles(const RowId* rows, uint32_t k) {
    uint32_t bad = 0;
    for (uint32_t j = 0; j < k; ++j) bad |= rows[j] ^ (rows[0] + j);
    return bad == 0;
}

struct Segment {
    uint32_t first = 0;
    uint32_t count = 0;
    RowId row0 = kNoRow;
    uint32_t off0 = 0, stride = 0;
    uint32_t bytes = 0;
    uint32_t column0 = 0;
    uint8_t header_bytes = 0;
    uint8_t owned = 0;
    void* host = nullptr;
    uint32_t end() const { return first + count; }
    RowId row(uint32_t j) const { return row0 == kNoRow ? kNoRow : row0 + j; }
    uint32_t off(uint32_t j) const { return off0 + j * stride; }
};

class Encoder : public FlushClient {
public:
    static const uint32_t kDenseSplit = 48;
    static const uint32_t kDirectMax = 512;
    static const uint32_t kDirectMinRun = 8;
    Encoder(Context* ctx, uint32_t row_bytes, HostRelease release = nullptr, void* user = nullptr);
    ~Encoder();

    unsigned remaining_slots() const { return kMaxPackets - count_; }

    Result add(RowId row, uint32_t framed_bytes, uint32_t header_bytes, uint32_t payload_bytes,
               void* host, uint32_t* packet_num, bool borrowed = false);
    bool add_run(const RowId* rows, uint32_t k, uint32_t framed_bytes, uint32_t header_bytes,
                 uint32_t payload_bytes, bool borrowed, uint32_t* first_col,
                 uint64_t layout = 0);
    Result get(uint32_t packet_num, StoredOriginal* out);
    void remove_before(uint32_t first_kept_column);
    Result acknowledge(const uint8_t* data, uint32_t bytes, uint32_t* next_expected);
    Result retransmit(StoredOriginal* out);
    Result encode(RecoveryOut& out);
    void stats(uint64_t* out, unsigned n);
    struct Mark {
        uint32_t next_row, next_parity_column, next_cauchy_row, sum_end;
        uint64_t recoveries, recovery_bytes;
        bool disabled;
    };
    bool encode_is_quiet() const;
    Mark mark() const {
        return Mark{next_row_, next_parity_column_, next_cauchy_row_, sum_end_, stats_[2], stats_[3], disabled_};
    }
    void rewind(const Mark& m) {
        next_row_ = m.next_row;
        next_parity_column_ = m.next_parity_column;
        next_cauchy_row_ = m.next_cauchy_row;
        sum_end_ = m.sum_end;
        stats_[2] = m.recoveries;
        stats_[3] = m.recovery_bytes;
        disabled_ = m.disabled;
    }
    void set_clock(const uint64_t* msec) { clock_ = msec; }

    bool disabled() const { return disabled_; }
    void set_disabled() { disabled_ = true; }
    uint64_t stat(unsigned i) const { return stats_[i]; }

    void pre_flush() override;
    void post_flush() override {}

private:
    Context* ctx_;
    uint32_t row_bytes_;
    HostRelease release_;
    void* user_;
    uint64_t stats_[9] = {0, 0, 0, 0, 0, 0, 0, 0, 0};
    bool disabled_ = false;
    const uint64_t* clock_ = nullptr;
    uint64_t now_msec() const;

    struct Slot { uint32_t seg, send_msec; };
    Ring<Slot> win_;
    Ring<Segment> segs_;
    uint32_t seg_base_ = 0;
    uint32_t base_ = 0;
    const Segment& seg_of(uint32_t e) const { return segs_[win_[e].seg - seg_base_]; }
    RowId row_of(uint32_t e) const {
        const Segment& s = seg_of(e);
        return s.row(e + base_ - s.first);
    }
    StoredOriginal view(uint32_t e) const;
    size_t seg_index_at(uint32_t a) const {
        if ((int32_t)(a - base_) >= 0) return win_[a - base_].seg - seg_base_;
        size_t i = 0;
        while (i + 1 < segs_.size() && (int32_t)(segs_[i].end() - a) <= 0) ++i;
        return i;
    }
    uint32_t sum_abs_start() const { return base_ + sum_start_ - sum_erased_; }
    void append(const RowId* rows, uint32_t k, uint32_t framed_bytes, uint32_t header_bytes, uint8_t owned,
                void* host, uint32_t now,
                uint64_t layout = 0);
    void release_segment(const Segment& s, uint32_t from, uint32_t n);
    void drop_all();
    void drop_segments_below(uint32_t drop);
    uint32_t placeholder_msec_[8] = {0, 0, 0, 0, 0, 0, 0, 0};
    uint32_t next_column_ = 0, count_ = 0, column_start_ = 0, longest_ = 0;
    uint32_t held_ = 0;
    uint32_t first_unremoved_ = 0;
    uint32_t sum_start_ = 0, sum_end_ = 0, sum_column_start_ = 0, sum_erased_ = 0;
    struct Lane {
        uint32_t next_abs = 0;
        LaneSums sums;
        uint32_t longest = 0;
    } lanes_[kLanes];

    struct Ack {
        std::vector<uint8_t> data;
        bool have_data = false;
        uint32_t data_bytes = 0, offset = 0, loss_column = 0, loss_count = 0;
        uint32_t next_expected = 0, next_rto_column = 0;
        bool found_oldest = false;
        uint32_t oldest_column = 0;
        uint32_t rto_msec = 500;
        struct Sample { uint32_t value; uint64_t ts; } max_rtt[3] = {{0, 0}, {0, 0}, {0, 0}};
    } ack_;

    uint32_t next_row_ = 0, next_parity_column_ = 0, next_cauchy_row_ = 0;

    uint32_t to_element(uint32_t column) const { return col_sub(column, column_start_); }
    uint32_t to_column(uint32_t element) const { return col_add(element, column_start_); }
    uint32_t unacked() const { return count_ - first_unremoved_; }
public:
    int debug_state(char* buf, size_t n) const {
        const uint32_t now = (uint32_t)now_msec();
        const uint32_t first = col_sub(ack_.next_expected, column_start_);
        const uint32_t age = first < count_ && first < win_.size() ? now - win_[first].send_msec : 0;
        return snprintf(buf, n,
                        "count=%u first_unremoved=%u next_column=%u column_start=%u ack_next=%u ack_bytes=%u "
                        "rto=%u found_oldest=%d first_age_ms=%u disabled=%d",
                        count_, first_unremoved_, next_column_, column_start_, ack_.next_expected, ack_.data_bytes,
                        ack_.rto_msec, (int)ack_.found_oldest, age, (int)disabled_);
    }
private:
    uint32_t next_lane_element(uint32_t element, uint32_t lane) const {
        uint32_t n = element - (element % kLanes) + lane;
        if (n < element) n += kLanes;
        return n;
    }

    uint32_t add_first(RowId row, uint32_t framed_bytes, uint32_t header_bytes, uint32_t payload_bytes, void* host,
                       bool borrowed);
    void start_new_window(uint32_t column);
    void reset_sums(uint32_t element_start);
    void remove_elements();
    LaneSums& get_lane(uint32_t lane, uint32_t element_end);

    bool decode_next_range();
    bool next_loss_column(uint32_t& column);
    void restart_loss_iterator();
    bool on_ack_data(const uint8_t* data, uint32_t bytes);
    void update_rto();
    void rtt_update(uint32_t value, uint64_t now, uint64_t window);
    Result attempt_retransmit(uint32_t e, StoredOriginal* out);

    Result generate_single(RecoveryOut& out);
    Result generate_cauchy(RecoveryOut& out);
    bool direct_sums() const;
    void add_dense(uint32_t row, uint32_t recovery_bytes, Sym& rec);
    void add_light(uint32_t row, Sym& rec);
    std::vector<uint64_t> pairs_;
    Result emit(Sym& terms, uint32_t len, const RecoveryMeta& meta, RecoveryOut& out, bool distinct);
    Sym scratch_, rec_;
    struct Run { RowId row; uint32_t off, stride, count, len, col; };
    std::vector<Run> runs_;
    struct CauchyTarget {
        RowId row = kNoRow;
        uint32_t used = 0, first_col = 0, end_col = 0, kind = 0, param = 0, flen = 0;
        uint8_t footer[8] = {0, 0, 0, 0, 0, 0, 0, 0};
        std::vector<Run> runs;
    };
    static const uint32_t kGroupSpan = 160;
    CauchyTarget grp_[3];
    uint32_t grp_n_ = 0, grp_gen_ = 0, window_gen_ = 0;
    std::vector<Run> grp_union_;
    void emit_cauchy_group();

    struct DenseTarget {
        RowId row = kNoRow;
        uint64_t ops = 0;
        uint32_t hi = 0, flen = 0;
        uint8_t rx = 0;
        uint8_t footer[8] = {0, 0, 0, 0, 0, 0, 0, 0};
        std::vector<uint32_t> pairs;
        Sym loose;
        std::vector<RowId> parts;
    };
    static const uint32_t kDenseGroupWork = 144;
    DenseTarget dgrp_[3];
    uint32_t dgrp_n_ = 0, dgrp_lo_ = 0, dgrp_len_ = 0, dgrp_gen_ = 0;
    std::vector<DenseRun> dgrp_runs_;
    bool defer_dense(uint32_t row, uint32_t recovery_bytes, const RecoveryOut& out);
    void emit_dense_group();
};

uint64_t time_msec();
void set_clock_source(uint64_t (*fn)());
inline uint64_t Encoder::now_msec() const { return clock_ ? *clock_ : time_msec(); }

}
```

### tonk_amd/csrc/engine.h

```cpp
#pragma once

#include "program.h"
#include "gf256.h"

#include <stdint.h>
#include <vector>
#include <algorithm>
#include <memory>
#include <utility>

namespace tamd {

using RowId = uint32_t;
static const RowId kNoRow = 0xffffffffu;

struct Term {
    RowId row;
    uint32_t len;
    uint8_t coef;
};
static const RowId kRunFlag = 0x80000000u;
inline bool is_run(RowId r) { return (r & kRunFlag) != 0; }

template <class T>
struct NoInitAlloc : std::allocator<T> {
    template <class U>
    struct rebind { typedef NoInitAlloc<U> other; };
    NoInitAlloc() = default;
    template <class U>
    NoInitAlloc(const NoInitAlloc<U>&) noexcept {}
    template <class U>
    void construct(U* p) noexcept { ::new ((void*)p) U; }
    template <class U, class... A>
    void construct(U* p, A&&... a) { ::new ((void*)p) U(std::forward<A>(a)...); }
};

typedef std::vector<Term, NoInitAlloc<Term>> Sym;
typedef std::vector<tamd_instr, NoInitAlloc<tamd_instr>> InstrVec;

extern const uint32_t g_slice_bytes;
inline uint32_t slice_bytes() { return g_slice_bytes; }
inline uint32_t op_slices(uint32_t span) {
    const uint32_t n = g_slice_bytes == TAMD_SLICE_BYTES_X ? (span + TAMD_SLICE_BYTES_X - 1) / TAMD_SLICE_BYTES_X
                                                            : (span + TAMD_SLICE_BYTES - 1) / TAMD_SLICE_BYTES;
    return n ? n : 1u;
}

class SegmentSource {
public:
    virtual ~SegmentSource() {}
    virtual bool get(uint32_t min_units, uint64_t* base_units, uint32_t* units) = 0;
    virtual void put(uint64_t base_units, uint32_t units) = 0;
};

class RowTable {
public:
    ~RowTable();
    void init(uint64_t bytes, uint64_t base_units = 0);
    void init_segmented(SegmentSource* src);

    RowId alloc(uint32_t bytes);
    void free_deferred(RowId r) {
        if (r != kNoRow) pending_.push_back(Pending{open_epoch_, r});
    }
    void release_up_to(uint64_t completed_epoch);
    void seal_epoch(uint64_t epoch);

    uint32_t offset(RowId r) const { return off_[r]; }
    bool affine(RowId r0, uint32_t k, uint32_t stride) const {
        if ((size_t)r0 + k > off_.size()) return false;
        const uint32_t* o = off_.data() + r0;
        const uint32_t o0 = o[0];
        uint32_t bad = 0;
        for (uint32_t j = 0; j < k; ++j) bad |= o[j] ^ (o0 + j * stride);
        return bad == 0;
    }
    uint32_t cap_bytes(RowId r) const { return units_[r] * TAMD_ROW_UNIT; }
    uint32_t units(RowId r) const { return units_[r]; }
    uint32_t level(RowId r) const { return ((hot_[r >> 6] >> (r & 63)) & 1u) ? level_[r] : 0u; }
    void set_level(RowId r, uint32_t l) {
        if (l) {
            hot_[r >> 6] |= 1ull << (r & 63);
            level_[r] = l;
        } else {
            hot_[r >> 6] &= ~(1ull << (r & 63));
        }
    }
    size_t live_rows() const { return live_; }
    uint64_t bytes_in_use() const { return (uint64_t)used_units_ * TAMD_ROW_UNIT; }
    void leak_segments() { src_ = nullptr; segments_.clear(); }

private:
    std::vector<uint32_t> off_, units_, level_;
    std::vector<uint64_t> hot_;
    std::vector<RowId> free_handles_;
    std::vector<std::vector<uint32_t>> free_offsets_;
    std::vector<std::pair<uint32_t, uint32_t>> free_big_;
    struct Pending { uint64_t epoch; RowId row; };
    std::vector<Pending> pending_;
    size_t pending_head_ = 0;
    uint64_t open_epoch_ = 1;
    uint32_t bump_ = 0, bump_end_ = 0;
    SegmentSource* src_ = nullptr;
    std::vector<std::pair<uint64_t, uint32_t>> segments_;
    uint64_t used_units_ = 0;
    size_t live_ = 0;
    void release(RowId r);
};

struct DenseRun { uint32_t off, stride, count, len, col, e0; };

void draw_dense_pairs(uint32_t row, uint32_t count, uint8_t rx, uint32_t first_rel, uint32_t origin,
                      const DenseRun* runs, size_t nruns, std::vector<uint32_t>& in, std::vector<uint64_t>& loose);
inline void sort_pair_keys(std::vector<uint64_t>& v) {
    for (size_t i = 1; i < v.size(); ++i) {
        const uint64_t x = v[i];
        size_t j = i;
        for (; j > 0 && v[j - 1] > x; --j) v[j] = v[j - 1];
        v[j] = x;
    }
}

class ProgramBuilder {
public:
    explicit ProgramBuilder(RowTable* rows);

    tamd_instr* reserve(size_t n) {
        const size_t at = instrs_.size();
        instrs_.resize(at + n);
        return instrs_.data() + at;
    }
    void commit(const tamd_instr* end) { instrs_.resize((size_t)(end - instrs_.data())); }

    uint32_t combine(RowId dst, const Term* terms, size_t n, uint32_t len,
                     const uint8_t* footer = nullptr, uint32_t footer_len = 0);

    void begin_op();
    void op_acc(RowId src, uint8_t coef, uint32_t len, uint32_t acc = 0);
    void op_acc3_off(uint32_t off, uint8_t c1, uint8_t c2, uint32_t len);
    void op_accr(uint32_t mode, uint32_t param, uint32_t row0, uint32_t stride, uint32_t count, uint32_t len,
                 uint32_t col0, uint32_t cstep);
    void op_accr_multi(uint32_t row0, uint32_t stride, uint32_t count, uint32_t len, uint32_t col0, uint32_t cstep,
                       const uint32_t t[3]);
    void op_accr_dense(uint32_t row0, uint32_t stride, uint32_t count, uint32_t len, uint32_t col0, uint64_t ops,
                       uint8_t rx, const uint32_t* adj = nullptr, uint32_t nadj = 0, uint8_t scale = 1);
    struct DenseTarget {
        uint64_t ops;
        uint8_t rx;
        uint32_t hi;
        const uint32_t* pairs;
        uint32_t npairs;
        RowId dst;
        const RowId* parts;
        uint32_t nparts;
        const Term* loose;
        uint32_t nloose;
        const uint8_t* footer;
        uint32_t flen;
    };
    void emit_dense_range(const DenseRun* runs, size_t nruns, const DenseTarget* t, uint32_t n, uint32_t split,
                          uint32_t len, bool skip_empty);
    void op_store_shared(RowId dst, uint32_t len, uint32_t acc, const uint8_t* footer, uint32_t footer_len);
    Term run_term(uint32_t mode, uint32_t p, uint32_t off0, uint32_t stride, uint32_t count, uint32_t col0,
                  uint32_t len) {
        runs_.push_back(RunRef{mode, p, off0, stride, count, col0, 0, 0, 0});
        return Term{kRunFlag | (uint32_t)(runs_.size() - 1), len, 1};
    }
    Term dense_run_term(uint32_t off0, uint32_t stride, uint32_t count, uint32_t col0, uint64_t ops, uint8_t rx,
                        const uint32_t* keys, uint32_t nadj, uint32_t rel0, uint32_t len) {
        const uint32_t at = (uint32_t)run_adj_.size();
        run_adj_.resize(at + nadj);
        for (uint32_t i = 0; i < nadj; ++i) run_adj_[at + i] = ((keys[i] >> 8) - rel0) << 16 | (keys[i] & 0xffu) << 8;
        runs_.push_back(RunRef{TAMD_R_DENSE, rx, off0, stride, count, col0, ops, at, nadj});
        return Term{kRunFlag | (uint32_t)(runs_.size() - 1), len, 1};
    }
    uint32_t finish_combine(RowId dst, uint32_t len, const uint8_t* footer, uint32_t footer_len);
    void op_store(RowId dst, uint32_t len, uint32_t acc = 0, const uint8_t* footer = nullptr, uint32_t footer_len = 0);
    void op_storec(RowId dst, uint32_t len, const uint8_t* c);
    void op_storec_part(RowId dst, uint32_t units, uint32_t len, uint32_t cap, const uint8_t* c, bool first);
    void op_acc_part(RowId src, uint32_t units, uint8_t coef, uint32_t len, uint32_t acc);
    uint32_t end_op(uint32_t min_level = 1) {
        return close_op((uint32_t)instrs_.size(), min_level);
    }

    bool empty() const { return ops_.empty(); }
    void clear();
    void swap_contents(ProgramBuilder& o) {
        ops_.swap(o.ops_);
        instrs_.swap(o.instrs_);
        levels_.swap(o.levels_);
        pure_.swap(o.pure_);
        written_.swap(o.written_);
        level_ops_.swap(o.level_ops_);
        level_items_.swap(o.level_items_);
        std::swap(max_level_, o.max_level_);
        std::swap(acc_bytes_, o.acc_bytes_);
        std::swap(store_bytes_, o.store_bytes_);
    }
    uint32_t max_level() const { return max_level_; }

    const std::vector<tamd_op>& ops() const { return ops_; }
    const InstrVec& instrs() const { return instrs_; }
    const std::vector<uint32_t>& op_levels() const { return levels_; }
    const std::vector<uint8_t>& op_pure() const { return pure_; }
    const std::vector<RowId>& written_rows() const { return written_; }
    const std::vector<uint32_t>& level_ops() const { return level_ops_; }
    const std::vector<uint32_t>& level_items() const { return level_items_; }

    uint64_t acc_bytes() const { return acc_bytes_; }
    uint64_t store_bytes() const { return store_bytes_; }

private:
    RowTable* rows_;
    std::vector<tamd_op> ops_;
    InstrVec instrs_;
    std::vector<uint32_t> levels_;
    std::vector<uint8_t> pure_;
    std::vector<RowId> written_;
    std::vector<uint32_t> level_ops_, level_items_;
    uint32_t max_level_ = 0;
    uint32_t cur_first_ = 0, cur_span_ = 0, cur_level_in_ = 0, cur_full_ = ~0u, cur_runs_ = 0;
    bool cur_pure_ = true;
    bool cur_multi_ = false;
    struct RunRef { uint32_t mode, p, off0, stride, count, col0; uint64_t ops; uint32_t adj0, nadj; };
    std::vector<RunRef> runs_;
    std::vector<uint32_t> run_adj_;
    size_t cur_written_begin_ = 0;
    uint64_t acc_bytes_ = 0, store_bytes_ = 0, cur_acc_begin_ = 0;
    static constexpr uint64_t kClsRowsDiv = 2, kClsT1 = 64, kClsT2 = 32, kClsT3 = 12, kClsRows0 = 48;
    uint32_t close_op(uint32_t end, uint32_t min_level);
};

inline void sym_add(Sym& dst, const Term* src, size_t n, uint32_t limit, uint8_t coef = 1) {
    if (coef == 0) return;
    for (size_t i = 0; i < n; ++i) {
        Term t = src[i];
        if (t.len > limit) t.len = limit;
        if (t.len == 0) continue;
        t.coef = coef == 1 ? t.coef : gf_mul(t.coef, coef);
        if (t.coef) dst.push_back(t);
    }
}
inline void sym_add(Sym& dst, const Sym& src, uint32_t limit, uint8_t coef = 1) {
    sym_add(dst, src.data(), src.size(), limit, coef);
}
inline void sym_scale(Sym& s, uint8_t coef) {
    if (coef == 1) return;
    size_t k = 0;
    for (size_t i = 0; i < s.size(); ++i) {
        Term t = s[i];
        t.coef = gf_mul(t.coef, coef);
        if (t.coef) s[k++] = t;
    }
    s.resize(k);
}
inline void sym_clip(Sym& s, uint32_t limit) {
    size_t k = 0;
    for (size_t i = 0; i < s.size(); ++i) {
        Term t = s[i];
        if (t.len > limit) t.len = limit;
        if (t.len) s[k++] = t;
    }
    s.resize(k);
}
void sym_merge(Sym& s);

class ExpansionTable;

class LaneSums {
public:
    uint32_t bytes = 0;

    void reset(RowTable& rows);
    void grow(uint32_t b) { if (b > bytes) bytes = b; }
    void accumulate(RowTable& rows, RowId row, uint32_t len, uint32_t column) {
        if (!len) return;
        if (rows.level(row) != 0) {
            if (len > content_) content_ = len;
            dyn_.push_back(T{row, len, 0, 0, 1, column});
            return;
        }
        accumulate_level0(row, rows.offset(row), len, column);
    }
    void accumulate_level0(RowId row, uint32_t off, uint32_t len, uint32_t column) {
        if (!len) return;
        if (len > content_) content_ = len;
        if (!terms_.empty()) {
            T& b = terms_.back();
            if (b.len == len && b.col + 8u * b.count == column) {
                if (b.count == 1 && off > b.off) {
                    b.stride = off - b.off;
                    b.count = 2;
                    ++n_;
                    return;
                }
                if (b.count > 1 && off == b.off + b.stride * b.count) {
                    ++b.count;
                    ++n_;
                    return;
                }
            }
        }
        terms_.push_back(T{row, len, off, 0, 1, column});
        ++n_;
    }
    void accumulate_run_level0(RowId row, uint32_t off, uint32_t len, uint32_t column, uint32_t count,
                               uint32_t stride) {
        if (!len || !count) return;
        if (count == 1) {
            accumulate_level0(row, off, len, column);
            return;
        }
        if (len > content_) content_ = len;
        n_ += count;
        if (!terms_.empty()) {
            T& b = terms_.back();
            if (b.len == len && b.col + 8u * b.count == column) {
                if (b.count == 1 && off > b.off && off - b.off == stride) {
                    b.stride = stride;
                    b.count = 1 + count;
                    return;
                }
                if (b.count > 1 && b.stride == stride && off == b.off + b.stride * b.count) {
                    b.count += count;
                    return;
                }
            }
        }
        terms_.push_back(T{row, len, off, stride, count, column});
    }
    void read(RowTable& rows, const ExpansionTable& ex, Sym& out, const uint8_t* c, uint32_t limit,
              ProgramBuilder* pb = nullptr, bool short_scan = false);
    bool idle() const { return terms_.empty() && dyn_.empty(); }
    void flush(RowTable& rows, ProgramBuilder& pb, const ExpansionTable& ex);
    void release(RowTable& rows);

private:
public:
    struct T { RowId row; uint32_t len, off, stride, count, col; };
    static constexpr uint32_t kChunk = 64;
    static constexpr uint32_t kDynFoldAbove = 2;
    static constexpr uint32_t kInlineMax = 3;
    static const uint32_t kSnapLevel = 2;
    static uint32_t snap_level(const RowTable& rows, const RowId* base, uint32_t l = kSnapLevel) {
        for (unsigned s = 0; s < 3; ++s)
            if (base[s] != kNoRow && rows.level(base[s]) + 1 > l) l = rows.level(base[s]) + 1;
        return l;
    }

private:
    struct Snap { RowId row; uint32_t after; uint8_t c[3]; uint8_t level; };
    uint32_t n_ = 0;
    RowId base_[3] = {kNoRow, kNoRow, kNoRow};
    uint32_t content_ = 0;
    std::vector<T> terms_;
    std::vector<Snap> snaps_;
    std::vector<T> dyn_;
    RowId fold_[3] = {kNoRow, kNoRow, kNoRow};
    uint32_t fold_len_ = 0;
    bool fold_dyn(RowTable& rows, ProgramBuilder& pb, const ExpansionTable& ex);
    void drop_fold(RowTable& rows);
    struct Closed { RowId base[3]; std::vector<T> terms; std::vector<Snap> snaps; };
    std::vector<Closed> closed_;
    size_t n_closed_ = 0;
    static void emit_scan(RowTable& rows, ProgramBuilder& pb, const RowId* base, const std::vector<T>& terms,
                          const std::vector<Snap>& snaps, const RowId* final_rows);
};

inline uint8_t sum_coef(unsigned s, uint8_t cx) { return s == 0 ? 1 : (s == 1 ? cx : gf_sqr(cx)); }
inline void opcode_coefs(unsigned op, uint8_t rx, uint8_t* c) {
    for (unsigned s = 0; s < 3; ++s)
        c[s] = (uint8_t)(((op >> s) & 1u) ^ (((op >> (s + 3)) & 1u) ? rx : 0u));
}

class ExpansionTable {
public:
    uint32_t expand_limit = ~0u;
    void set(RowId r, const Sym& s);
    void take(RowId r, Sym& s);
    bool has(RowId r) const { return r < index_.size() && index_[r] >= 0; }
    const Sym& get(RowId r) const { return pool_[index_[r]]; }
    void clear();
    void append(const RowTable& rows, RowId r, uint32_t len, uint8_t coef, Sym& out) const;

private:
    std::vector<int32_t> index_;
    std::vector<Sym> pool_;
    size_t n_pool_ = 0;
    std::vector<RowId> used_;
};

RowId fold_low_levels(RowTable& rows, ProgramBuilder& pb, Sym& s, uint32_t keep_level,
                      uint32_t len, uint32_t row_bytes);

class FlushClient {
public:
    virtual ~FlushClient() {}
    virtual void pre_flush() = 0;
    virtual void post_flush() = 0;
    bool dirty = false;
};

struct Context {
    RowTable rows;
    ProgramBuilder pb{&rows};
    ProgramBuilder closed{&rows};
    ExpansionTable ex;
    std::vector<RowId> temps;
    std::vector<FlushClient*> clients;
    uint64_t epoch = 1;
    uint64_t arena_base_units = 0;
    bool oom = false;
    uint32_t backsub_rows = ~0u;
    uint32_t dense_split = 0;
    bool direct_elim = default_direct_elim();
    static bool default_direct_elim() {
        static const bool on = !(getenv("TONK_AMD_DEC_DIRECT") && atoi(getenv("TONK_AMD_DEC_DIRECT")) == 0);
        return on;
    }
    bool short_scans = false;
    static const uint32_t kPipeDepth = 1;
    bool pipeline = false;
    std::vector<RowId> inherited;
    std::vector<uint64_t> written_mark;

    RowId alloc(uint32_t bytes) {
        const RowId r = rows.alloc(bytes);
        if (r == kNoRow) oom = true;
        return r;
    }
    RowId alloc_temp(uint32_t bytes) {
        const RowId r = alloc(bytes);
        if (r != kNoRow) temps.push_back(r);
        return r;
    }
    void attach(FlushClient* c) { clients.push_back(c); }
    void detach(FlushClient* c) {
        clients.erase(std::remove(clients.begin(), clients.end(), c), clients.end());
        dirty.erase(std::remove(dirty.begin(), dirty.end(), c), dirty.end());
    }
    bool track_dirty = false;
    std::vector<FlushClient*> dirty;
    void touch(FlushClient* c) {
        if (!c->dirty) {
            c->dirty = true;
            dirty.push_back(c);
        }
    }
    void prepare_flush() {
        for (FlushClient* c : track_dirty ? dirty : clients) c->pre_flush();
    }
    void finish_flush(bool keep_closed = false) {
        const std::vector<RowId>& w = pb.written_rows();
        if (pipeline) {
            if (!inherited.empty()) {
                for (RowId r : w) {
                    if ((r >> 6) >= written_mark.size()) written_mark.resize((r >> 6) + 1024, 0);
                    written_mark[r >> 6] |= 1ull << (r & 63);
                }
                size_t keep = 0;
                for (RowId r : inherited) {
                    if ((r >> 6) < written_mark.size() && ((written_mark[r >> 6] >> (r & 63)) & 1u)) continue;
                    const uint32_t l = rows.level(r);
                    if (l > kPipeDepth) {
                        rows.set_level(r, l - kPipeDepth);
                        inherited[keep++] = r;
                    } else {
                        rows.set_level(r, 0);
                    }
                }
                inherited.resize(keep);
                for (RowId r : w) written_mark[r >> 6] = 0;
            }
            for (RowId r : w) {
                const uint32_t l = rows.level(r);
                if (l > kPipeDepth) {
                    rows.set_level(r, l - kPipeDepth);
                    inherited.push_back(r);
                } else {
                    rows.set_level(r, 0);
                }
            }
        } else {
            for (RowId r : w) rows.set_level(r, 0);
        }
        for (RowId r : temps) rows.free_deferred(r);
        temps.clear();
        ex.clear();
        for (FlushClient* c : track_dirty ? dirty : clients) c->post_flush();
        for (FlushClient* c : dirty) c->dirty = false;
        dirty.clear();
        rows.seal_epoch(epoch);
        ++epoch;
        if (keep_closed) closed.swap_contents(pb);
        pb.clear();
    }
};

}
```

### tonk_amd/csrc/gf256.cpp

```cpp
#include "gf256.h"

#include <string.h>

namespace tamd {

GF g_gf;

static bool self_test() {
    for (unsigned i = 0; i < 256; ++i) {
        for (unsigned j = 0; j < 256; ++j) {
            const uint8_t p = gf_mul((uint8_t)i, (uint8_t)j);
            if (i && j) {
                if (gf_div(p, (uint8_t)i) != j || gf_div(p, (uint8_t)j) != i) return false;
            } else if (p != 0) {
                return false;
            }
            if (j == 1 && p != i) return false;
        }
    }
    return gf_mul(2, 0x80) == 0x4d && gf_mul(0xaa, 0x6c) == 0x7c && gf_inv(2) == 0xa6 && gf_sqr(3) == 5;
}

bool gf_init() {
    if (g_gf.ready) return true;
    const unsigned poly = 0x14d;
    uint8_t exp[1024];
    uint16_t log[256];
    memset(exp, 0, sizeof(exp));
    log[0] = 512;
    unsigned v = 1;
    for (unsigned j = 0; j < 255; ++j) {
        exp[j] = (uint8_t)v;
        log[v] = (uint16_t)j;
        v <<= 1;
        if (v & 0x100) v ^= poly;
    }
    for (unsigned j = 255; j < 510; ++j) exp[j] = exp[j - 255];
    exp[510] = 1;

    for (unsigned x = 0; x < 256; ++x) {
        g_gf.mul[0][x] = 0;
        g_gf.div[0][x] = 0;
    }
    for (unsigned y = 1; y < 256; ++y) {
        const unsigned ly = log[y];
        for (unsigned x = 0; x < 256; ++x) {
            if (x == 0) { g_gf.mul[y][0] = 0; g_gf.div[y][0] = 0; continue; }
            g_gf.mul[y][x] = exp[log[x] + ly];
            g_gf.div[y][x] = exp[log[x] + 255 - ly];
        }
    }
    for (unsigned x = 0; x < 256; ++x) {
        g_gf.inv[x] = g_gf.div[x][1];
        g_gf.sqr[x] = g_gf.mul[x][x];
    }
    for (unsigned c = 0; c < 256; ++c) {
        uint8_t t[3][8];
        for (unsigned i = 0; i < 8; ++i) {
            t[0][i] = g_gf.mul[c][i];
            t[1][i] = g_gf.mul[c][i << 3];
            t[2][i] = i < 4 ? g_gf.mul[c][i << 6] : 0;
        }
        memcpy(&g_gf.perm[c][0], t, 24);
        g_gf.perm[c][6] = 0;
        g_gf.perm[c][7] = 0;
    }
    g_gf.ready = self_test();
    return g_gf.ready;
}

}
```

### tonk_amd/csrc/gf256.h

```cpp
#pragma once
#include <stdint.h>

namespace tamd {

struct GF {
    uint8_t mul[256][256];
    uint8_t div[256][256];
    uint8_t inv[256];
    uint8_t sqr[256];
    uint32_t perm[256][8];
    bool ready = false;
};

extern GF g_gf;

bool gf_init();

inline uint8_t gf_mul(uint8_t x, uint8_t y) { return g_gf.mul[y][x]; }
inline uint8_t gf_div(uint8_t x, uint8_t y) { return g_gf.div[y][x]; }
inline uint8_t gf_inv(uint8_t x) { return g_gf.inv[x]; }
inline uint8_t gf_sqr(uint8_t x) { return g_gf.sqr[x]; }

static const unsigned kMaxLossRecovery = 255;
static const unsigned kColumnPeriod    = 0x400000;
static const unsigned kRowPeriod       = 255;
static const unsigned kLanes           = 8;
static const unsigned kSums            = 3;
static const unsigned kPairRate        = 16;
static const unsigned kSubwindow       = 64;
static const unsigned kCauchyThreshold = 64;
static const unsigned kSumResetThreshold = 32;
static const unsigned kCauchyMaxColumns = 64;
static const unsigned kCauchyMaxRows   = 256 - 64;
static const unsigned kMaxPackets      = 16000;
static const unsigned kRemoveThreshold = 2 * kSubwindow;

inline uint8_t column_value(unsigned column) { return (uint8_t)(3u + (column * 199u) % 253u); }
inline uint8_t row_value(unsigned row) { return (uint8_t)(1u + (row + 1u) % 255u); }

inline unsigned row_opcode(unsigned lane, unsigned row) {
    uint32_t k = lane + (row + 3u) * kLanes;
    k += ~(k << 15);
    k ^= (k >> 10);
    k += (k << 3);
    k ^= (k >> 6);
    k += ~(k << 11);
    k ^= (k >> 16);
    const uint32_t op = k & 63u;
    return op == 0 ? 16u : op;
}

inline uint8_t cauchy_element(unsigned row, unsigned column) {
    return gf_inv((uint8_t)((uint8_t)column ^ (uint8_t)(row + kCauchyMaxColumns)));
}

inline bool col_delta_negative(unsigned d) { return d >= kColumnPeriod / 2; }
inline unsigned col_sub(unsigned a, unsigned b) { return (a - b) % kColumnPeriod; }
inline unsigned col_add(unsigned a, unsigned b) { return (a + b) % kColumnPeriod; }
inline unsigned col_inc(unsigned a) { return col_add(a, 1); }

struct Pcg32 {
    uint64_t state = 0, inc = 0;
    void seed(uint64_t y, uint64_t x) {
        state = 0;
        inc = (y << 1u) | 1u;
        next();
        state += x;
        next();
    }
    uint32_t next() {
        const uint64_t old = state;
        state = old * 6364136223846793005ULL + inc;
        const uint32_t xs = (uint32_t)(((old >> 18) ^ old) >> 27);
        const uint32_t rot = (uint32_t)(old >> 59);
        return (xs >> rot) | (xs << ((uint32_t)(-(int32_t)rot) & 31u));
    }
};

struct FastMod {
    uint64_t m;
    uint32_t d;
    explicit FastMod(uint32_t divisor) : m(divisor ? ~0ull / divisor + 1 : 0), d(divisor) {}
    uint32_t operator()(uint32_t x) const { return (uint32_t)(((unsigned __int128)(m * x) * d) >> 64); }
};

}
```

### tonk_amd/csrc/resident_backend.h

```cpp
#pragma once

#include "decoder.h"
#include "prof.h"
#include "workload.h"

#include <memory>

namespace tamd {

struct ResidentBackend {
    struct RecRef { RecoveryOut out; };
    struct DecRef {};

    Context* ctx = nullptr;
    std::unique_ptr<Encoder> enc;
    std::unique_ptr<Decoder> dec;
    std::vector<RowId> enc_rows, dec_rows;
    uint32_t pool = 0;
    bool pool_affine = false;
    uint32_t pool_off[2] = {0, 0}, pool_stride = 0;
    bool nobatch = false;
    bool contig = true;
    uint64_t alg_bytes = 0, payload_bytes = 0;
    std::vector<RecoveredPacket*> got_;

    bool alloc_inputs(uint32_t n, uint32_t pool_n, uint32_t row_bytes) {
        enc_rows.assign(n, kNoRow);
        dec_rows.assign(n, kNoRow);
        for (int side = 0; side < 2; ++side) {
            std::vector<RowId>& rows = side ? dec_rows : enc_rows;
            for (uint32_t i = 0; i < pool_n; ++i)
                if ((rows[i] = ctx->alloc(row_bytes)) == kNoRow) return false;
            for (uint32_t i = pool_n; i < n; ++i) rows[i] = rows[i - pool_n];
        }
        pool = pool_n;
        pool_affine = pool >= 2;
        for (int side = 0; side < 2 && pool_affine; ++side) {
            const std::vector<RowId>& rows = side ? dec_rows : enc_rows;
            const uint32_t o0 = ctx->rows.offset(rows[0]), stride = ctx->rows.offset(rows[1]) - o0;
            pool_affine = consecutive_handles(rows.data(), pool) && stride > 0 &&
                          ctx->rows.affine(rows[0], pool, stride) && (!side || stride == pool_stride);
            pool_off[side] = o0;
            pool_stride = stride;
        }
        return true;
    }
    uint64_t layout(int side, uint32_t index, uint32_t k) const {
        if (!pool_affine || !contig || index % pool + k > pool) return 0;
        return (uint64_t)(pool_off[side] + (index % pool) * pool_stride) << 32 | pool_stride;
    }

    int enc_add(uint32_t index, uint32_t len, uint32_t* col) {
        const uint32_t hb = length_header_bytes(len);
        TAMD_PROF_SCOPE(kEncAdd);
        const Result r = enc->add(enc_rows[index], hb + len, hb, len, nullptr, col, true);
        if (r == kSuccess) {
            alg_bytes += hb + len;
            payload_bytes += len;
        }
        return r;
    }
    bool enc_add_run(uint32_t index, uint32_t k, uint32_t len, uint32_t* col0) {
        if (nobatch) return false;
        const uint32_t hb = length_header_bytes(len);
        TAMD_PROF_SCOPE(kEncAdd);
        if (!enc->add_run(&enc_rows[index], k, hb + len, hb, len, true, col0, layout(0, index, k))) return false;
        alg_bytes += (uint64_t)(hb + len) * k;
        payload_bytes += (uint64_t)len * k;
        return true;
    }
    bool dec_add_run(uint32_t col0, uint32_t index, uint32_t k, uint32_t len) {
        if (nobatch) return false;
        const uint32_t hb = length_header_bytes(len);
        TAMD_PROF_SCOPE(kDecAddOrig);
        if (!dec->add_run_inorder(col0, &dec_rows[index], k, hb + len, hb, len, true, layout(1, index, k))) return false;
        alg_bytes += (uint64_t)(hb + len) * k;
        return true;
    }
    int enc_encode(RecRef& r) {
        TAMD_PROF_SCOPE(kEncEncode);
        const Result rc = enc->encode(r.out);
        if (rc == kSuccess) alg_bytes += r.out.total();
        return rc;
    }
    int enc_ack(const uint8_t* buf, uint32_t n, uint32_t* next) {
        TAMD_PROF_SCOPE(kEncAck);
        return enc->acknowledge(buf, n, next);
    }
    int enc_is_ready() { return enc->remaining_slots() <= 2 ? (int)kMaxPacketsReached : 0; }
    int dec_add_original(uint32_t col, uint32_t index, uint32_t len) {
        const uint32_t hb = length_header_bytes(len);
        TAMD_PROF_SCOPE(kDecAddOrig);
        bool took = false;
        const Result r = dec->add_original(col, dec_rows[index], hb + len, hb, len, nullptr, &took, true);
        alg_bytes += hb + len;
        return r;
    }
    void recovery_lost(const RecRef& r) { ctx->rows.free_deferred(r.out.row); }
    int dec_add_recovery(const RecRef& r) {
        uint8_t tail[8] = {0, 0, 0, 0, 0, 0, 0, 0};
        const uint32_t tl = r.out.total() < 8 ? r.out.total() : 8;
        memcpy(tail + tl - r.out.footer_len, r.out.footer, r.out.footer_len);
        TAMD_PROF_SCOPE(kDecAddRec);
        bool took = false;
        const Result rc = dec->add_recovery(r.out.row, r.out.total(), tail, nullptr, &took);
        if (!took) ctx->rows.free_deferred(r.out.row);
        alg_bytes += r.out.total();
        return rc;
    }
    int dec_is_ready() {
        TAMD_PROF_SCOPE(kDecIsReady);
        return dec->is_ready();
    }
    int dec_decode(std::vector<uint32_t>& nums, DecRef&) {
        TAMD_PROF_SCOPE(kDecDecode);
        got_.clear();
        const Result rc = dec->decode(got_);
        if (rc != kSuccess) got_.clear();
        for (RecoveredPacket* rp : got_) {
            nums.push_back(rp->packet_num);
            alg_bytes += rp->framed_upper;
        }
        return rc;
    }
    int dec_ack(uint8_t* buf, uint32_t limit, uint32_t* used) {
        TAMD_PROF_SCOPE(kDecAck);
        return dec->ack(buf, limit, used);
    }
    void stats(uint64_t e[9], uint64_t d[11]) { enc->stats(e, 9); dec->stats(d, 11); }
    uint64_t vclock = 0;
    void set_time(uint64_t ms) {
        if (!vclock) enc->set_clock(&vclock);
        vclock = ms;
    }
    int enc_retransmit(uint32_t* num, uint32_t* bytes, const uint8_t** data) {
        StoredOriginal o;
        const Result rc = enc->retransmit(&o);
        if (rc == kSuccess) {
            *num = o.column;
            *bytes = o.bytes - o.header_bytes;
            *data = nullptr;
        }
        return rc;
    }
};

}
```

### tonk_amd/csrc/ring.h

```cpp
#pragma once
#include <stddef.h>
#include <vector>

namespace tamd {

template <class T>
class Ring {
public:
    size_t size() const { return n_; }
    bool empty() const { return n_ == 0; }
    T& back() { return buf_[(head_ + n_ - 1) & mask_]; }
    const T& back() const { return buf_[(head_ + n_ - 1) & mask_]; }
    T& front() { return buf_[head_]; }
    T& operator[](size_t i) { return buf_[(head_ + i) & mask_]; }
    const T& operator[](size_t i) const { return buf_[(head_ + i) & mask_]; }
    void push_back(const T& v) {
        if (n_ == buf_.size()) grow();
        buf_[(head_ + n_) & mask_] = v;
        ++n_;
    }
    void reserve_more(size_t k) {
        while (n_ + k > buf_.size()) grow();
    }
    T* slot_base() { return buf_.data(); }
    size_t slot_index(size_t i) const { return (head_ + i) & mask_; }
    size_t slot_mask() const { return mask_; }
    void commit(size_t k) { n_ += k; }
    T& push_slot() {
        if (n_ == buf_.size()) grow();
        return buf_[(head_ + n_++) & mask_];
    }
    void pop_front(size_t k) {
        if (k > n_) k = n_;
        head_ = (head_ + k) & mask_;
        n_ -= k;
    }
    void clear() { pop_front(n_); head_ = 0; }

private:
    std::vector<T> buf_;
    size_t head_ = 0, n_ = 0, mask_ = 0;
    void grow() {
        const size_t cap = buf_.empty() ? 64 : buf_.size() * 2;
        std::vector<T> nb(cap);
        for (size_t i = 0; i < n_; ++i) nb[i] = (*this)[i];
        buf_.swap(nb);
        head_ = 0;
        mask_ = cap - 1;
    }
};

}
```

### tonk_amd/csrc/session.cpp

```cpp
#include "../../include/tonk_amd.h"

#include "device.h"
#include "resident_backend.h"
#include "transcript.h"

#include <hip/hip_runtime.h>

#include <chrono>
#include <atomic>
#include <algorithm>
#include <condition_variable>
#include <functional>
#include <memory>
#include <mutex>
#include <string>
#include <thread>
#include <pthread.h>
#include <sched.h>
#include <stdio.h>
#include <stdlib.h>
#include <string.h>

using namespace tamd;

namespace {

std::vector<int> parse_cpulist(const char* text) {
    std::vector<int> out;
    std::string line(text ? text : "");
    size_t at = 0;
    while (at < line.size()) {
        size_t end = line.find_first_of(",\n", at);
        if (end == std::string::npos) end = line.size();
        int a = 0, b = 0;
        const int n = sscanf(line.substr(at, end - at).c_str(), "%d-%d", &a, &b);
        if (n >= 1) {
            if (n == 1) b = a;
            for (int c = a; c <= b && c >= 0 && c < CPU_SETSIZE; ++c) out.push_back(c);
        }
        at = end + 1;
    }
    return out;
}

std::vector<int> node_core_share(const std::vector<std::string>& dev_cpulists, unsigned device,
                                 const std::vector<int>& node_cores, const char* slot_override,
                                 unsigned* slot_out = nullptr, unsigned* nslots_out = nullptr) {
    unsigned slot = 0, nslots = 1;
    unsigned k = 0, n = 0;
    if (slot_override && sscanf(slot_override, "%u/%u", &k, &n) == 2 && n >= 1 && k < n) {
        slot = k;
        nslots = n;
    } else if (device < dev_cpulists.size()) {
        nslots = 0;
        for (size_t d = 0; d < dev_cpulists.size(); ++d) {
            if (dev_cpulists[d] != dev_cpulists[device]) continue;
            if (d < device) ++slot;
            ++nslots;
        }
    }
    if (slot_out) *slot_out = slot;
    if (nslots_out) *nslots_out = nslots;
    const size_t N = node_cores.size();
    if (nslots <= 1 || N < nslots) return node_cores;
    const size_t base = N / nslots, extra = N % nslots;
    const size_t begin = slot * base + (slot < extra ? slot : extra);
    const size_t len = base + (slot < extra ? 1 : 0);
    return std::vector<int>(node_cores.begin() + begin, node_cores.begin() + begin + len);
}

std::string read_line(const std::string& path) {
    FILE* f = fopen(path.c_str(), "r");
    if (!f) return std::string();
    char line[4096] = {0};
    const bool ok = fgets(line, sizeof(line), f) != nullptr;
    fclose(f);
    std::string s = ok ? std::string(line) : std::string();
    while (!s.empty() && (s.back() == '\n' || s.back() == ' ')) s.pop_back();
    return s;
}

std::string device_cpulist(int device) {
    char bus[64] = {0};
    if (hipDeviceGetPCIBusId(bus, sizeof(bus), device) != hipSuccess) return std::string();
    for (char* c = bus; *c; ++c) *c = (char)tolower(*c);
    return read_line(std::string("/sys/bus/pci/devices/") + bus + "/local_cpulist");
}

std::vector<int> device_local_cpus(int device) {
    std::vector<int> out;
    const std::string mine = device_cpulist(device);
    if (mine.empty()) return out;
    cpu_set_t allowed;
    CPU_ZERO(&allowed);
    if (sched_getaffinity(0, sizeof(allowed), &allowed) != 0) return out;
    for (int c : parse_cpulist(mine.c_str())) {
        if (!CPU_ISSET(c, &allowed)) continue;
        char tp[128];
        snprintf(tp, sizeof(tp), "/sys/devices/system/cpu/cpu%d/topology/thread_siblings_list", c);
        const std::vector<int> sib = parse_cpulist(read_line(tp).c_str());
        if (!sib.empty() && sib[0] != c) continue;
        out.push_back(c);
    }
    int n = 0;
    if (hipGetDeviceCount(&n) != hipSuccess) n = 0;
    std::vector<std::string> lists;
    for (int d = 0; d < n; ++d) lists.push_back(device_cpulist(d));
    return node_core_share(lists, (unsigned)device, out, getenv("TONK_AMD_CPU_SLOT"));
}

std::vector<uint64_t> cpu_busy_jiffies() {
    std::vector<uint64_t> busy;
    FILE* f = fopen("/proc/stat", "r");
    if (!f) return busy;
    char line[512];
    while (fgets(line, sizeof(line), f)) {
        if (strncmp(line, "cpu", 3) != 0 || line[3] < '0' || line[3] > '9') continue;
        unsigned c = 0;
        unsigned long long v[8] = {0, 0, 0, 0, 0, 0, 0, 0};
        if (sscanf(line + 3, "%u %llu %llu %llu %llu %llu %llu %llu %llu", &c, &v[0], &v[1], &v[2], &v[3], &v[4],
                   &v[5], &v[6], &v[7]) < 5)
            continue;
        if (c >= busy.size()) busy.resize(c + 1, 0);
        busy[c] = v[0] + v[1] + v[2] + v[5] + v[6] + v[7];
    }
    fclose(f);
    return busy;
}

std::vector<int> pick_idle(const std::vector<int>& share, const std::vector<uint64_t>& busy_delta, size_t want) {
    if (share.size() <= want) return share;
    std::vector<int> order(share);
    auto busy = [&](int c) { return (size_t)c < busy_delta.size() ? busy_delta[c] : 0; };
    std::stable_sort(order.begin(), order.end(), [&](int a, int b) { return busy(a) < busy(b); });
    order.resize(want);
    std::sort(order.begin(), order.end());
    return order;
}

std::vector<int> idle_cpus(const std::vector<int>& share, size_t want) {
    if (share.size() <= want) return share;
    const std::vector<uint64_t> a = cpu_busy_jiffies();
    std::this_thread::sleep_for(std::chrono::milliseconds(50));
    const std::vector<uint64_t> b = cpu_busy_jiffies();
    std::vector<uint64_t> d(b.size(), 0);
    for (size_t i = 0; i < b.size() && i < a.size(); ++i) d[i] = b[i] - a[i];
    return pick_idle(share, d, want);
}

struct Stream : ResidentBackend {
    wl::Params p;
    bool record = false;
    wl::DeferredTranscript tr;
    size_t reg_enc = 0, reg_dec = 0;
    uint32_t stage = 0;
    std::vector<std::pair<RowId, uint32_t>> out_rows;
    uint64_t recv_bytes = 0;

    int enc_encode(RecRef& r) {
        const int rc = ResidentBackend::enc_encode(r);
        if (rc == 0 && (stage & 1u)) out_rows.push_back(std::make_pair(r.out.row, r.out.total()));
        return rc;
    }
    int dec_add_recovery(const RecRef& r) {
        if (stage & 2u) recv_bytes += r.out.total();
        return ResidentBackend::dec_add_recovery(r);
    }
    int dec_decode(std::vector<uint32_t>& nums, DecRef& d) {
        const int rc = ResidentBackend::dec_decode(nums, d);
        if ((stage & 2u) || record)
            for (RecoveredPacket* rp : got_) {
                if (stage & 2u) out_rows.push_back(std::make_pair(rp->row, rp->framed_upper));
                if (record) tr.recovered(rp->row, rp->framed_upper);
            }
        return rc;
    }

    void on_encode(int rc, const RecRef& r) {
        if (record)
            tr.encode(rc, r.out.row, r.out.total(), r.out.meta.Row, r.out.meta.ColumnStart, r.out.meta.SumCount,
                      r.out.meta.LDPCCount);
    }
    void on_decode(int rc, const std::vector<uint32_t>& nums, const DecRef&) { if (record) tr.decode(rc, nums); }
    void on_ack(int rd, const uint8_t* buf, uint32_t used, int re, uint32_t next) {
        if (record) tr.ack(rd, buf, used, re, next);
    }
    void on_event(char kind, int rc, uint32_t a, uint32_t b) { if (record) tr.event(kind, rc, a, b); }
    void on_retransmit(int rc, uint32_t num, uint32_t bytes, uint64_t h) { if (record) tr.retransmit(rc, num, bytes, h); }
    void on_stats(const uint64_t e[9], const uint64_t d[11]) { if (record) tr.stats(e, d); }
    template <class NextTag>
    void register_verify(std::vector<Device::VerifyDesc>& d, NextTag next_tag) {
        for (; reg_enc < tr.pend_enc.size(); ++reg_enc) {
            wl::DeferredTranscript::Enc& e = tr.pend_enc[reg_enc];
            e.tag = next_tag();
            d.push_back(Device::VerifyDesc{(uint32_t)ctx->rows.offset(e.row), e.total, 0, 0});
        }
        for (; reg_dec < tr.pend_dec.size(); ++reg_dec) {
            wl::DeferredTranscript::Dec& e = tr.pend_dec[reg_dec];
            e.tag = next_tag();
            d.push_back(Device::VerifyDesc{(uint32_t)ctx->rows.offset(e.row), e.upper, 1, 0});
        }
    }

    std::unique_ptr<wl::Runner<Stream, Stream>> runner;

    std::atomic<uint32_t> next_step{0};
    std::atomic<uint8_t> busy{0};
    uint64_t clock = 0;
    static const unsigned kParts = 8;
    Device::Part parts[kParts];
};

struct Session {
    tamd_session_params prm;
    Device dev;
    std::vector<std::unique_ptr<Stream>> streams;
    std::vector<std::unique_ptr<Context>> ctxs;
    std::vector<double> busy_ms;
    std::vector<double> fill_ms;
    std::vector<std::pair<uint64_t, uint64_t>> epoch_ticket;
    uint64_t last_ticket = 0, released_epoch = 0;
    double host_ms[6] = {0, 0, 0, 0, 0, 0};
    uint64_t clock_msec = 0;
    uint32_t row_cap = 0;
    uint8_t* host_in = nullptr;
    size_t host_in_bytes = 0;
    uint8_t* host_out = nullptr;
    size_t host_out_cap = 0;
    uint64_t h2d_bytes = 0, d2h_bytes = 0;
    bool finished = false;
    std::string error;

    std::vector<std::thread> threads;
    std::vector<int> cpus;
    size_t threads_wanted = 0;
    std::mutex mu;
    std::condition_variable cv_start, cv_done;
    std::atomic<bool> main_sleeping{false};
    const std::function<void(size_t, size_t)>* job = nullptr;
    std::atomic<bool> quit{false};

    ~Session() {
        if (fr_running) fr_drain();
        quit.store(true);
        {
            std::lock_guard<std::mutex> lk(mu);
            gen.fetch_add(1);
        }
        cv_start.notify_all();
        for (auto& t : threads) t.join();
        dev.synchronize();
        dev.sync_staging();
        if (host_in) hipHostFree(host_in);
        if (host_out) hipHostFree(host_out);
        for (auto& s : streams) {
            s->runner.reset();
            s->enc.reset();
            s->dec.reset();
        }
    }

    std::vector<uint32_t> order;
    std::vector<double> stream_ms;

    std::vector<std::atomic<uint8_t>> claimed;
    void drain(const std::function<void(size_t, size_t)>& f, size_t ti) {
        const size_t T = threads.size(), n = streams.size();
        if (T == 0) {
            for (size_t k = 0; k < n; ++k) f(order.empty() ? k : order[k], ti);
            return;
        }
        if (order.empty()) {
            for (size_t s = ti; s < n; s += T)
                if (!claimed[s].exchange(1)) f(s, ti);
        } else {
            for (size_t k = 0; k < n; ++k) {
                const size_t s = order[k];
                if (s % T == ti && !claimed[s].exchange(1)) f(s, ti);
            }
        }
        for (size_t k = 0; k < n; ++k) {
            const size_t s = order.empty() ? k : order[k];
            if (!claimed[s].exchange(1)) f(s, ti);
        }
    }

    static constexpr uint64_t kSpinNs = 100000;
    std::atomic<uint64_t> gen{0};
    std::atomic<size_t> left{0};
    std::atomic<int> sleepers{0};

    void pool_loop(size_t ti) {
        dev.bind_thread();
        if (!cpus.empty()) {
            cpu_set_t set;
            CPU_ZERO(&set);
            if (cpus.size() < threads_wanted) {
                for (int c : cpus) CPU_SET(c, &set);
            } else {
                CPU_SET(cpus[ti % cpus.size()], &set);
            }
            pthread_setaffinity_np(pthread_self(), sizeof(set), &set);
        }
        uint64_t seen = 0;
        for (;;) {
            if (gen.load(std::memory_order_acquire) == seen) {
                const auto until = std::chrono::steady_clock::now() + std::chrono::nanoseconds(kSpinNs);
                unsigned k = 0;
                while (gen.load(std::memory_order_acquire) == seen) {
                    __builtin_ia32_pause();
                    if ((++k & 255) == 0 && std::chrono::steady_clock::now() > until) break;
                }
            }
            if (gen.load(std::memory_order_acquire) == seen) {
                std::unique_lock<std::mutex> lk(mu);
                sleepers.fetch_add(1);
                cv_start.wait(lk, [&] { return gen.load() != seen; });
                sleepers.fetch_sub(1);
            }
            seen = gen.load(std::memory_order_acquire);
            if (quit.load(std::memory_order_acquire)) return;
            if (job_kind.load(std::memory_order_acquire) == 1) fr_loop(ti);
            else drain(*job, ti);
            if (left.fetch_sub(1, std::memory_order_acq_rel) == 1 && main_sleeping.load()) {
                std::lock_guard<std::mutex> lk(mu);
                cv_done.notify_one();
            }
        }
    }

    void run_all(const std::function<void(size_t, size_t)>& f) {
        if (fr_running) fr_drain();
        if (threads.empty()) {
            drain(f, 0);
            return;
        }
        if (claimed.size() != streams.size()) claimed = std::vector<std::atomic<uint8_t>>(streams.size());
        for (auto& c : claimed) c.store(0, std::memory_order_relaxed);
        job = &f;
        job_kind.store(0, std::memory_order_relaxed);
        left.store(threads.size(), std::memory_order_relaxed);
        gen.fetch_add(1, std::memory_order_seq_cst);
        if (sleepers.load(std::memory_order_seq_cst) > 0) {
            std::lock_guard<std::mutex> lk(mu);
            cv_start.notify_all();
        }
        wait_pass_end();
    }

    void wait_pass_end() {
        const auto until = std::chrono::steady_clock::now() + std::chrono::microseconds(20);
        unsigned k = 0;
        while (left.load(std::memory_order_acquire) != 0) {
            __builtin_ia32_pause();
            if ((++k & 255) == 0 && std::chrono::steady_clock::now() > until) {
                std::unique_lock<std::mutex> lk(mu);
                main_sleeping.store(true);
                cv_done.wait(lk, [&] { return left.load() == 0; });
                main_sleeping.store(false);
                break;
            }
        }
    }

    struct FrProg {
        uint32_t originals = 0;
        bool finish = false;
        int handle = -1;
        uint64_t epoch = 0, clock = 0;
        std::atomic<uint32_t> remaining{0};
    };
    static const unsigned kFrRing = Stream::kParts;
    FrProg fr_progs[kFrRing];
    bool fr_mode = false, fr_running = false;
    std::atomic<int> job_kind{0};
    std::atomic<bool> fr_stop{false};
    std::atomic<uint32_t> fr_published{0};
    uint32_t fr_launched = 0;
    static constexpr uint32_t fr_ahead = 2;
    uint64_t fr_next_epoch = 1;
    std::atomic<uint64_t> fr_released{0};
    std::mutex fr_mu;
    std::condition_variable cv_fr, cv_main;
    std::atomic<int> fr_sleepers{0};
    std::atomic<bool> fr_main_waiting{false};
    std::vector<std::vector<uint64_t>> fr_vbase;

    void start_fr() {
        if (fr_running) return;
        fr_stop.store(false);
        job_kind.store(1, std::memory_order_relaxed);
        left.store(threads.size(), std::memory_order_relaxed);
        gen.fetch_add(1, std::memory_order_seq_cst);
        if (sleepers.load(std::memory_order_seq_cst) > 0) {
            std::lock_guard<std::mutex> lk(mu);
            cv_start.notify_all();
        }
        fr_running = true;
    }

    void stop_fr() {
        if (!fr_running) return;
        fr_stop.store(true, std::memory_order_seq_cst);
        {
            std::lock_guard<std::mutex> lk(fr_mu);
            cv_fr.notify_all();
        }
        wait_pass_end();
        fr_running = false;
        job_kind.store(0);
        double sum = 0, mx = 0;
        for (double b : busy_ms) {
            sum += b;
            if (b > mx) mx = b;
        }
        host_ms[1] += sum;
        host_ms[5] += mx;
        std::fill(busy_ms.begin(), busy_ms.end(), 0.0);
        for (double f : fill_ms) host_ms[3] += f;
        std::fill(fill_ms.begin(), fill_ms.end(), 0.0);
    }

    std::atomic<uint32_t> fr_launched_pub{0};
    int fr_pick(size_t ti) {
        const int best = fr_scan(ti);
        if (best < 0) return -1;
        const uint32_t pub = fr_published.load(std::memory_order_acquire);
        Stream& st = *streams[best];
        if (st.busy.exchange(1, std::memory_order_acq_rel)) return -2;
        if (st.next_step.load(std::memory_order_acquire) < pub) return best;
        st.busy.store(0, std::memory_order_release);
        return -2;
    }
    int fr_scan(size_t ti) {
        const uint32_t pub = fr_published.load(std::memory_order_acquire);
        const uint32_t oldest = fr_launched_pub.load(std::memory_order_acquire);
        const size_t T = threads.size(), n = streams.size();
        const size_t group = ti / 8;
        for (int pass = 0; pass < 3; ++pass) {
            int best = -1;
            uint32_t bk = ~0u;
            for (size_t s = pass ? 0 : ti; s < n; s += pass ? 1 : T) {
                if (pass == 1 && (s % T) / 8 != group) continue;
                Stream& st = *streams[s];
                const uint32_t k = st.next_step.load(std::memory_order_acquire);
                if (pass == 2 && k != oldest) continue;
                if (k < pub && k < bk && !st.busy.load(std::memory_order_relaxed)) {
                    best = (int)s;
                    bk = k;
                }
            }
            if (best >= 0) return best;
        }
        return -1;
    }

    void fr_loop(size_t ti) {
        for (;;) {
            if (fr_stop.load(std::memory_order_acquire)) return;
            const int s = fr_pick(ti);
            if (s >= 0) {
                fr_run(s, ti);
                continue;
            }
            if (s == -2) continue;
            const uint32_t seen = fr_published.load(std::memory_order_acquire);
            const uint32_t seen_l = fr_launched_pub.load(std::memory_order_acquire);
            const uint32_t seen_h = fr_handback.load(std::memory_order_acquire);
            auto changed = [&] {
                return fr_stop.load(std::memory_order_acquire) || fr_published.load(std::memory_order_acquire) != seen ||
                       fr_launched_pub.load(std::memory_order_acquire) != seen_l ||
                       fr_handback.load(std::memory_order_acquire) != seen_h;
            };
            const auto until = std::chrono::steady_clock::now() + std::chrono::nanoseconds(kSpinNs);
            unsigned k = 0;
            bool woke = false;
            while (!(woke = changed())) {
                __builtin_ia32_pause();
                if ((++k & 255) == 0 && std::chrono::steady_clock::now() > until) break;
            }
            if (woke) continue;
            std::unique_lock<std::mutex> lk(fr_mu);
            fr_sleepers.fetch_add(1);
            cv_fr.wait(lk, [&] { return changed() || fr_scan(ti) >= 0; });
            fr_sleepers.fetch_sub(1);
        }
    }
    std::atomic<uint32_t> fr_handback{0};
    void fr_wake_workers() {
        if (fr_sleepers.load(std::memory_order_seq_cst) > 0) {
            std::lock_guard<std::mutex> lk(fr_mu);
            cv_fr.notify_all();
        }
    }

    void fr_run(int s, size_t ti) {
        typedef std::chrono::steady_clock clk;
        const auto w0 = clk::now();
        Stream& st = *streams[s];
        const uint32_t k = st.next_step.load(std::memory_order_relaxed);
        FrProg& P = fr_progs[k % kFrRing];
        Context& c = *ctxs[s];
        c.rows.release_up_to(fr_released.load(std::memory_order_acquire));
        st.clock = P.clock;
        if (P.finish) st.runner->finish();
        else st.runner->advance(P.originals);
        c.prepare_flush();
        Device::Part& part = st.parts[k % kFrRing];
        dev.add_part(P.handle, c.pb, part);
        part.verify.clear();
        if (st.record) {
            uint64_t local = 0;
            st.register_verify(part.verify, [&] { return ((uint64_t)k << 32) | local++; });
        }
        c.finish_flush(false);
        busy_ms[ti] += std::chrono::duration<double, std::milli>(clk::now() - w0).count();
        const bool stolen = (size_t)s % threads.size() != ti;
        if (stolen) fill_ms[ti] += 1.0;
        st.next_step.store(k + 1, std::memory_order_release);
        st.busy.store(0, std::memory_order_release);
        if (stolen && k + 1 < fr_published.load(std::memory_order_acquire)) {
            fr_handback.fetch_add(1, std::memory_order_seq_cst);
            fr_wake_workers();
        }
        if (P.remaining.fetch_sub(1, std::memory_order_acq_rel) == 1 && fr_main_waiting.load()) {
            std::lock_guard<std::mutex> lk(fr_mu);
            cv_main.notify_one();
        }
    }

    void fr_launch_ready() {
        typedef std::chrono::steady_clock clk;
        const uint32_t pub = fr_published.load(std::memory_order_relaxed);
        std::vector<Device::Part*> parts(streams.size());
        while (fr_launched < pub) {
            FrProg& P = fr_progs[fr_launched % kFrRing];
            if (P.remaining.load(std::memory_order_acquire) != 0) break;
            const auto t0 = clk::now();
            for (size_t i = 0; i < streams.size(); ++i) parts[i] = &streams[i]->parts[fr_launched % kFrRing];
            if (prm.record) {
                std::vector<uint64_t> base(streams.size());
                for (size_t i = 0; i < streams.size(); ++i) {
                    base[i] = verify_count;
                    verify_count += parts[i]->verify.size();
                }
                if (fr_vbase.size() <= fr_launched) fr_vbase.resize(fr_launched + 1);
                fr_vbase[fr_launched].swap(base);
            }
            last_ticket = dev.close_program(P.handle, parts.data(), parts.size());
            epoch_ticket.push_back(std::make_pair(P.epoch, last_ticket));
            ++fr_launched;
            fr_launched_pub.store(fr_launched, std::memory_order_seq_cst);
            fr_wake_workers();
            fr_released.store(completed_epoch(), std::memory_order_release);
            host_ms[4] += std::chrono::duration<double, std::milli>(clk::now() - t0).count();
        }
    }

    void fr_wait_one() {
        typedef std::chrono::steady_clock clk;
        const auto t0 = clk::now();
        FrProg& P = fr_progs[fr_launched % kFrRing];
        const auto until = t0 + std::chrono::microseconds(20);
        unsigned k = 0;
        while (P.remaining.load(std::memory_order_acquire) != 0) {
            __builtin_ia32_pause();
            if ((++k & 255) == 0 && clk::now() > until) {
                std::unique_lock<std::mutex> lk(fr_mu);
                fr_main_waiting.store(true);
                cv_main.wait(lk, [&] { return P.remaining.load() == 0; });
                fr_main_waiting.store(false);
                break;
            }
        }
        host_ms[0] += std::chrono::duration<double, std::milli>(clk::now() - t0).count();
        fr_launch_ready();
    }

    void fr_bounds(uint32_t originals, bool finish, size_t* recs, size_t* items) const {
        uint64_t n = originals;
        if (finish) {
            n = 0;
            for (const auto& sp : streams) {
                const uint64_t left = sp->p.n_originals - sp->runner->position() + sp->p.flush_max;
                if (left > n) n = left;
            }
        }
        *recs = streams.size() * (size_t)(16 * n + 8192);
        *items = streams.size() * (size_t)(n / 2 + 2048);
    }

    void fr_step(uint32_t originals, bool finish) {
        typedef std::chrono::steady_clock clk;
        size_t recs = 0, items = 0;
        fr_bounds(originals, finish, &recs, &items);
        if (!dev.assembly_fits(recs, items)) {
            fr_drain();
            if (!dev.ensure_assembly(recs, items)) error = dev.error();
        }
        start_fr();
        while (fr_published.load(std::memory_order_relaxed) - fr_launched >= fr_ahead) fr_wait_one();
        const uint32_t k = fr_published.load(std::memory_order_relaxed);
        FrProg& P = fr_progs[k % kFrRing];
        P.originals = originals;
        P.finish = finish;
        P.clock = time_msec();
        P.epoch = fr_next_epoch++;
        const auto t0 = clk::now();
        P.handle = dev.open_program();
        host_ms[2] += std::chrono::duration<double, std::milli>(clk::now() - t0).count();
        P.remaining.store((uint32_t)streams.size(), std::memory_order_relaxed);
        fr_published.store(k + 1, std::memory_order_seq_cst);
        fr_wake_workers();
        fr_launch_ready();
    }

    void fr_drain() {
        if (!fr_mode) return;
        while (fr_launched < fr_published.load(std::memory_order_relaxed)) fr_wait_one();
        stop_fr();
    }

    uint64_t completed_epoch() {
        size_t k = 0;
        while (k < epoch_ticket.size() && dev.completed(epoch_ticket[k].second)) {
            released_epoch = epoch_ticket[k].first;
            ++k;
        }
        epoch_ticket.erase(epoch_ticket.begin(), epoch_ticket.begin() + k);
        return released_epoch;
    }

    bool deferred = false;
    bool have_closed = false;
    std::atomic<size_t> fills_left{0};
    uint64_t closed_epoch = 0;

    void step(uint32_t originals, bool finish) {
        if (fr_mode) { fr_step(originals, finish); return; }
        if (deferred) { step_deferred(originals, finish); return; }
        typedef std::chrono::steady_clock clk;
        auto ms = [](clk::time_point a, clk::time_point b) {
            return std::chrono::duration<double, std::milli>(b - a).count();
        };
        const auto t0 = clk::now();
        clock_msec = time_msec();
        if (host_in && !finish) stage_inputs(originals);
        const uint64_t rel = completed_epoch();
        std::fill(busy_ms.begin(), busy_ms.end(), 0.0);
        init_order();
        run_all([this, originals, finish, rel, &ms](size_t i, size_t ti) {
            const auto w0 = clk::now();
            Context& c = *ctxs[i];
            streams[i]->clock = clock_msec;
            c.rows.release_up_to(rel);
            if (finish) streams[i]->runner->finish();
            else streams[i]->runner->advance(originals);
            c.prepare_flush();
            const double t = ms(w0, clk::now());
            busy_ms[ti] += t;
            stream_ms[i] = t;
        });
        sort_order();
        const auto t1 = clk::now();
        account_busy();
        std::vector<Context*> cs;
        for (auto& c : ctxs) cs.push_back(c.get());
        dev.begin(cs.data(), cs.size());
        const auto t2 = clk::now();
        const uint64_t epoch = ctxs.empty() ? 0 : ctxs[0]->epoch;
        run_all([this](size_t i, size_t) {
            dev.fill(i);
            ctxs[i]->finish_flush();
        });
        const auto t3 = clk::now();
        if (host_in) dev.h2d_fence();
        if (prm.record) register_verify();
        last_ticket = dev.launch();
        if (host_in) stage_outputs();
        const auto t4 = clk::now();
        host_ms[0] += ms(t0, t1);
        host_ms[2] += ms(t1, t2);
        host_ms[3] += ms(t2, t3);
        host_ms[4] += ms(t3, t4);
        epoch_ticket.push_back(std::make_pair(epoch, last_ticket));
    }

    void init_order() {
        if (order.size() != streams.size()) {
            order.resize(streams.size());
            for (size_t i = 0; i < order.size(); ++i) order[i] = (uint32_t)i;
            stream_ms.assign(streams.size(), 0.0);
        }
    }
    void sort_order() {
        std::sort(order.begin(), order.end(), [this](uint32_t a, uint32_t b) { return stream_ms[a] > stream_ms[b]; });
    }
    void account_busy() {
        double mx = 0;
        for (double b : busy_ms) {
            host_ms[1] += b;
            if (b > mx) mx = b;
        }
        host_ms[5] += mx;
    }

    void step_deferred(uint32_t originals, bool finish) {
        typedef std::chrono::steady_clock clk;
        auto ms = [](clk::time_point a, clk::time_point b) {
            return std::chrono::duration<double, std::milli>(b - a).count();
        };
        const auto t0 = clk::now();
        clock_msec = time_msec();
        const uint64_t rel = completed_epoch();
        std::fill(busy_ms.begin(), busy_ms.end(), 0.0);
        std::fill(fill_ms.begin(), fill_ms.end(), 0.0);
        init_order();
        const bool fill = have_closed;
        if (fill) fills_left.store(streams.size(), std::memory_order_relaxed);
        run_all([this, originals, finish, rel, fill, &ms](size_t i, size_t ti) {
            const auto w0 = clk::now();
            Context& c = *ctxs[i];
            if (fill) {
                dev.fill(i);
                fill_ms[ti] += ms(w0, clk::now());
                if (fills_left.fetch_sub(1, std::memory_order_acq_rel) == 1) launch_closed();
            }
            c.rows.release_up_to(rel);
            streams[i]->clock = clock_msec;
            if (finish) streams[i]->runner->finish();
            else streams[i]->runner->advance(originals);
            c.prepare_flush();
            c.finish_flush(true);
            const double t = ms(w0, clk::now());
            busy_ms[ti] += t;
            stream_ms[i] = t;
        });
        sort_order();
        const auto t1 = clk::now();
        account_busy();
        for (double f : fill_ms) host_ms[3] += f / (double)fill_ms.size();
        const auto t2 = clk::now();
        std::vector<Context*> cs;
        for (auto& c : ctxs) cs.push_back(c.get());
        dev.begin(cs.data(), cs.size(), true);
        if (prm.record) register_verify();
        have_closed = true;
        closed_epoch = ctxs.empty() ? 0 : ctxs[0]->epoch - 1;
        const auto t3 = clk::now();
        host_ms[0] += ms(t0, t1);
        host_ms[4] += ms(t1, t2);
        host_ms[2] += ms(t2, t3);
    }

    void launch_closed() {
        last_ticket = dev.launch();
        have_closed = false;
        epoch_ticket.push_back(std::make_pair(closed_epoch, last_ticket));
    }

    void flush_closed() {
        fr_drain();
        if (!have_closed) return;
        run_all([this](size_t i, size_t) { dev.fill(i); });
        launch_closed();
    }

    void stage_inputs(uint32_t originals) {
        const size_t side_bytes = (size_t)streams[0]->p.n_originals * row_cap;
        for (size_t i = 0; i < streams.size(); ++i) {
            Stream& st = *streams[i];
            const uint32_t next = (uint32_t)st.runner->summary().originals;
            const uint32_t n = next + originals <= st.p.n_originals ? originals : st.p.n_originals - next;
            if (!n) continue;
            for (int side = 0; side < 2; ++side) {
                if (!((prm.stage_host >> side) & 1u)) continue;
                const RowId r = (side ? st.dec_rows : st.enc_rows)[next];
                const uint8_t* src = host_in + (2 * i + side) * side_bytes + (size_t)next * row_cap;
                dev.h2d((uint64_t)st.ctx->rows.offset(r) * TAMD_ROW_UNIT, src, (size_t)n * row_cap);
                h2d_bytes += (uint64_t)n * row_cap;
            }
        }
    }

    void stage_outputs() {
        std::vector<Device::GatherDesc> d;
        size_t bytes = 0, recv = 0;
        for (auto& sp : streams) {
            for (const auto& o : sp->out_rows) {
                Device::GatherDesc g;
                g.row = sp->ctx->rows.offset(o.first);
                g.len = o.second;
                g.out = (uint32_t)bytes;
                d.push_back(g);
                bytes += (o.second + 15u) & ~15u;
            }
            sp->out_rows.clear();
            recv += sp->recv_bytes;
            sp->recv_bytes = 0;
        }
        if (bytes > host_out_cap) {
            dev.sync_staging();
            if (host_out) hipHostFree(host_out);
            host_out_cap = bytes + bytes / 2 + 4096;
            if (hipHostMalloc((void**)&host_out, host_out_cap, hipHostMallocDefault) != hipSuccess) {
                host_out = nullptr;
                host_out_cap = 0;
                error = "pinned staging allocation failed";
                return;
            }
        }
        dev.d2h_gather(d, bytes, host_out);
        d2h_bytes += bytes;
        if (recv > bytes) recv = bytes;
        dev.h2d_after_d2h(host_out, recv);
        h2d_bytes += recv;
    }

    void release_all() {
        const uint64_t rel = completed_epoch();
        run_all([this, rel](size_t i, size_t) { ctxs[i]->rows.release_up_to(rel); });
    }

    uint64_t verify_count = 0, verify_base = 0;
    void register_verify() {
        std::vector<Device::VerifyDesc> d;
        for (auto& sp : streams) sp->register_verify(d, [this] { return verify_count++; });
        dev.verify_next(d);
    }

    void resolve_transcripts() {
        if (!fr_mode) register_verify();
        std::vector<Device::VerifyOut> res;
        dev.verify_results(res);
        if (verify_base + res.size() != verify_count) {
            error = "verification digests missing";
            return;
        }
        size_t si = 0;
        auto get = [&](uint64_t v) -> const Device::VerifyOut& {
            if (fr_mode) v = fr_vbase[v >> 32][si] + (v & 0xffffffffu);
            return res[v - verify_base];
        };
        for (auto& sp : streams) {
            Stream& s = *sp;
            for (size_t k = 0; k < s.tr.pend_enc.size(); ++k) s.tr.resolve_enc(k, get(s.tr.pend_enc[k].tag).hash);
            for (size_t k = 0; k < s.tr.pend_dec.size(); ++k) {
                const Device::VerifyOut& o = get(s.tr.pend_dec[k].tag);
                if (o.ok) s.tr.resolve_dec(k, o.len, o.hash);
                else error = "recovered row with a corrupt length header";
            }
            s.tr.resolved();
            s.reg_enc = s.reg_dec = 0;
            ++si;
        }
        verify_base = verify_count;
        dev.verify_reset();
    }
};

}

extern "C" {

void* tamd_session_create(const tamd_session_params* p, char* err, size_t err_len) {
    auto fail = [&](const std::string& m) -> void* {
        if (err && err_len) snprintf(err, err_len, "%s", m.c_str());
        return nullptr;
    };
    if (!p || p->n_streams == 0) return fail("bad parameters");
    if (!gf_init()) return fail("gf self test failed");
    std::unique_ptr<Session> s(new Session());
    s->prm = *p;
    const bool pipe = !p->stage_host;
    uint32_t nthreads = p->n_threads ? (p->n_threads < p->n_streams ? p->n_threads : p->n_streams) : 1;
    std::vector<int> share;
    if (nthreads > 1) {
        share = device_local_cpus((int)p->device);
        if (!share.empty() && share.size() < nthreads) nthreads = (uint32_t)share.size();
    }
    s->fr_mode = pipe && nthreads > 1;
    s->dev.set_small_uploads(p->n_streams <= 4);
    if (s->fr_mode) s->dev.set_assembly_slots(8, p->n_streams <= 4 ? 8 : 24);
    else {
        const size_t slots = pipe ? (p->n_streams <= 4 ? 12 : 6) : 2;
        s->dev.set_program_slots(slots, (p->n_streams <= 4 ? 2u : 16u) << 20);
    }
    if (!s->dev.init((int)p->device, p->arena_bytes)) return fail(s->dev.error());
    s->dev.set_pipelined(pipe);
    if (!s->dev.gf_selftest()) return fail("device GF(256) self test failed");

    const uint64_t range = (s->dev.arena_bytes() / p->n_streams) & ~(uint64_t)(TAMD_ROW_UNIT - 1);
    s->row_cap = ((p->payload_max + 4 + 63) / 64) * 64;
    s->busy_ms.assign(nthreads, 0.0);
    s->fill_ms.assign(nthreads, 0.0);
    s->deferred = pipe;
    Session* raw = s.get();
    if (nthreads > 1) {
        raw->cpus = idle_cpus(share.empty() ? device_local_cpus((int)p->device) : share, nthreads);
        raw->threads_wanted = nthreads;
        for (uint32_t t = 0; t < nthreads; ++t) raw->threads.emplace_back([raw, t] { raw->pool_loop(t); });
    }
    s->streams.resize(p->n_streams);
    s->ctxs.resize(p->n_streams);
    s->run_all([raw, p, range, pipe](size_t i, size_t) {
        std::unique_ptr<Context> ctx(new Context());
        ctx->rows.init(range, (range / TAMD_ROW_UNIT) * i);
        ctx->pipeline = pipe;
        if (pipe) ctx->ex.expand_limit = p->n_streams <= 4 ? 16u : ~0u;
        ctx->backsub_rows = p->n_streams <= 4 ? 2u : ~0u;
        ctx->dense_split = p->n_streams <= 4 ? 0u : Encoder::kDenseSplit;
        ctx->short_scans = p->n_streams <= 4;
        std::unique_ptr<Stream> st(new Stream());
        st->ctx = ctx.get();
        wl::Params& q = st->p;
        q.stream_id = p->stream_base + (uint32_t)i;
        q.n_originals = p->n_originals;
        q.payload_min = p->payload_min;
        q.payload_max = p->payload_max;
        q.loss_thresh = p->loss_thresh;
        q.ge_enable = p->ge_enable;
        q.gb_thresh = p->gb_thresh;
        q.bg_thresh = p->bg_thresh;
        q.loss_on_recovery = p->loss_on_recovery;
        q.fec_rate_q16 = p->fec_rate_q16;
        q.ack_every = p->ack_every;
        q.ack_bytes = p->ack_bytes ? p->ack_bytes : 256;
        q.arq_lag = p->arq_lag;
        q.flush_max = p->flush_max;
        q.rtx_every = p->rtx_every;
        q.rtx_msec = p->rtx_msec ? p->rtx_msec : 1;
        q.hold_full = p->hold_full;
        q.seed_data = 1000 + q.stream_id;
        q.seed_loss = 2000 + q.stream_id;
        st->enc.reset(new Encoder(ctx.get(), raw->row_cap));
        st->enc->set_clock(&st->clock);
        st->dec.reset(new Decoder(ctx.get(), raw->row_cap));
        st->record = p->record != 0;
        st->runner.reset(new wl::Runner<Stream, Stream>(st->p, *st, *st));
        raw->streams[i] = std::move(st);
        raw->ctxs[i] = std::move(ctx);
    });
    return s.release();
}

int tamd_session_generate(void* sp) {
    Session* s = (Session*)sp;
    std::vector<std::vector<Device::GenDesc>> per(s->streams.size());
    std::atomic<bool> full{false};
    s->run_all([s, &per, &full](size_t si, size_t) {
        Stream& st = *s->streams[si];
        std::vector<Device::GenDesc>& d = per[si];
        const uint32_t n = st.p.n_originals;
        st.runner->pregenerate();
        const uint32_t pool = s->prm.input_pool && s->prm.input_pool < n && !s->prm.record &&
                                      !s->prm.stage_host && st.p.payload_min == st.p.payload_max
                                  ? s->prm.input_pool : n;
        if (!st.alloc_inputs(n, pool, s->row_cap)) { full = true; return; }
        d.reserve(2 * (size_t)pool);
        for (int side = 0; side < 2; ++side)
            for (uint32_t i = 0; i < pool; ++i) {
                const RowId r = (side ? st.dec_rows : st.enc_rows)[i];
                Device::GenDesc g;
                g.row = st.ctx->rows.offset(r);
                g.index = i;
                g.len = wl::payload_length(st.p, i);
                g.cap = st.ctx->rows.cap_bytes(r);
                g.seed = st.p.seed_data;
                d.push_back(g);
            }
    });
    if (full) { s->error = "arena too small for the session inputs"; return -1; }
    std::vector<Device::GenDesc> d;
    size_t total = 0;
    for (auto& v : per) total += v.size();
    d.reserve(total);
    for (auto& v : per) {
        d.insert(d.end(), v.begin(), v.end());
        std::vector<Device::GenDesc>().swap(v);
    }
    s->dev.generate_rows(d, s->row_cap);
    if (!s->dev.error().empty()) return -2;
    if (s->prm.stage_host) {
        const size_t side_bytes = (size_t)s->streams[0]->p.n_originals * s->row_cap;
        s->host_in_bytes = 2 * s->streams.size() * side_bytes;
        if (!s->dev.enable_staging() ||
            hipHostMalloc((void**)&s->host_in, s->host_in_bytes, hipHostMallocDefault) != hipSuccess) {
            s->host_in = nullptr;
            s->error = "pinned input staging allocation failed";
            return -3;
        }
        for (size_t i = 0; i < s->streams.size(); ++i) {
            Stream& st = *s->streams[i];
            st.stage = s->prm.stage_host & 3u;
            for (int side = 0; side < 2; ++side) {
                const std::vector<RowId>& rows = side ? st.dec_rows : st.enc_rows;
                const uint64_t base = st.ctx->rows.offset(rows[0]);
                for (uint32_t k = 0; k < st.p.n_originals; ++k)
                    if (st.ctx->rows.offset(rows[k]) != base + (uint64_t)k * (s->row_cap / TAMD_ROW_UNIT)) {
                        s->error = "input rows are not contiguous";
                        return -3;
                    }
                s->dev.download(s->host_in + (2 * i + side) * side_bytes, base * TAMD_ROW_UNIT, side_bytes);
            }
        }
    }
    return 0;
}

int tamd_session_step(void* sp, uint32_t originals) {
    Session* s = (Session*)sp;
    s->step(originals, false);
    for (auto& c : s->ctxs) if (c->oom) { s->error = "arena exhausted"; return -1; }
    return s->error.empty() && s->dev.error().empty() ? 0 : -1;
}

int tamd_session_wait(void* sp) {
    Session* s = (Session*)sp;
    s->flush_closed();
    s->dev.synchronize();
    s->dev.sync_staging();
    if (s->prm.record) s->resolve_transcripts();
    s->release_all();
    return s->dev.error().empty() && s->error.empty() ? 0 : -1;
}

int tamd_session_finish(void* sp) {
    Session* s = (Session*)sp;
    if (!s->finished) {
        s->step(0, true);
        s->finished = true;
    }
    return tamd_session_wait(sp);
}

int tamd_session_summary(void* sp, uint64_t* out, unsigned n) {
    Session* s = (Session*)sp;
    uint64_t v[TAMD_SUM_COUNT] = {0};
    for (auto& stp : s->streams) {
        const wl::Summary& q = stp->runner->summary();
        v[TAMD_SUM_ORIGINALS] += q.originals;
        v[TAMD_SUM_LOST_ORIGINALS] += q.lost_originals;
        v[TAMD_SUM_RECOVERIES] += q.recoveries;
        v[TAMD_SUM_LOST_RECOVERIES] += q.lost_recoveries;
        v[TAMD_SUM_RECOVERED] += q.recovered;
        v[TAMD_SUM_ARQ] += q.arq_redelivered;
        v[TAMD_SUM_MISSING_AT_END] += q.missing_at_end;
        v[TAMD_SUM_PAYLOAD_BYTES] += stp->payload_bytes;
        v[TAMD_SUM_ALG_BYTES] += stp->alg_bytes;
        v[TAMD_SUM_DISABLED_CODECS] += (stp->enc->disabled() ? 1 : 0) + (stp->dec->disabled() ? 1 : 0);
    }
    const DeviceStats& ds = s->dev.stats();
    v[TAMD_SUM_PROGRAMS] = ds.programs;
    v[TAMD_SUM_LAUNCHES] = ds.launches;
    v[TAMD_SUM_OPS] = ds.ops;
    v[TAMD_SUM_INSTRS] = ds.instrs;
    v[TAMD_SUM_UPLOAD_BYTES] = ds.upload_bytes;
    v[TAMD_SUM_ACC_BYTES] = ds.acc_bytes;
    v[TAMD_SUM_STORE_BYTES] = ds.store_bytes;
    v[TAMD_SUM_H2D_BYTES] = s->h2d_bytes;
    v[TAMD_SUM_D2H_BYTES] = s->d2h_bytes;
    v[TAMD_SUM_D2H_COPY_US] = (uint64_t)(ds.d2h_copy_ms * 1e3);
    if (n > TAMD_SUM_COUNT) n = TAMD_SUM_COUNT;
    for (unsigned i = 0; i < n; ++i) out[i] = v[i];
    return s->error.empty() ? 0 : -1;
}

void tamd_session_set_timing(void* sp, int on) { ((Session*)sp)->dev.set_timing(on != 0); }

double tamd_session_kernel_ms(void* sp, uint64_t* launches) {
    Session* s = (Session*)sp;
    s->dev.collect_timing();
    if (launches) *launches = s->dev.stats().timed_launches;
    return s->dev.stats().kernel_ms;
}

size_t tamd_session_transcript(void* sp, uint32_t stream, char* buf, size_t cap) {
    Session* s = (Session*)sp;
    if (stream >= s->streams.size()) return 0;
    std::string all;
    for (const std::string& l : s->streams[stream]->tr.lines) { all += l; all += '\n'; }
    if (buf && cap) {
        const size_t n = all.size() < cap - 1 ? all.size() : cap - 1;
        memcpy(buf, all.data(), n);
        buf[n] = 0;
    }
    return all.size() + 1;
}

void tamd_session_host_ms(void* sp, double out[10]) {
    Session* s = (Session*)sp;
    for (int i = 0; i < 6; ++i) out[i] = s->host_ms[i];
    out[6] = s->dev.stats().slot_wait_ms;
    out[7] = s->dev.stats().upload_enqueue_ms;
    out[8] = s->dev.stats().upload_enqueue_max_ms;
    out[9] = (double)s->dev.stats().slot_reallocs;
}

void tamd_session_arena(void* sp, uint64_t* base, uint64_t* bytes) {
    Session* s = (Session*)sp;
    if (base) *base = (uint64_t)(uintptr_t)s->dev.arena();
    if (bytes) *bytes = s->dev.arena_bytes();
}

void tamd_session_destroy(void* sp) { delete (Session*)sp; }

const char* tamd_session_error(void* sp) {
    Session* s = (Session*)sp;
    if (!s->error.empty()) return s->error.c_str();
    return s->dev.error().c_str();
}

void tamd_set_clock(uint64_t (*fn)(void)) { set_clock_source(fn); }

int tamd_session_schedule(void* sp) { return ((Session*)sp)->fr_mode ? 1 : 0; }

unsigned tamd_session_cpus(void* sp, int* out, unsigned cap) {
    Session* s = (Session*)sp;
    for (unsigned i = 0; i < cap && i < s->cpus.size(); ++i) out[i] = s->cpus[i];
    return (unsigned)s->cpus.size();
}

unsigned tamd_cpu_share(const char* dev_cpulists, unsigned device, const char* node_cores, const char* slot_override,
                        int* out, unsigned cap) {
    std::vector<std::string> lists;
    const std::string all(dev_cpulists ? dev_cpulists : "");
    size_t at = 0;
    while (at <= all.size() && !all.empty()) {
        size_t end = all.find(';', at);
        if (end == std::string::npos) end = all.size();
        lists.push_back(all.substr(at, end - at));
        at = end + 1;
    }
    const std::vector<int> share = node_core_share(lists, device, parse_cpulist(node_cores), slot_override);
    for (unsigned i = 0; i < cap && i < share.size(); ++i) out[i] = share[i];
    return (unsigned)share.size();
}

int tamd_device_selftest(uint32_t device, char* err, size_t err_len) {
    Device d;
    if (!d.init((int)device, 1 << 20)) {
        if (err && err_len) snprintf(err, err_len, "%s", d.error().c_str());
        return -1;
    }
    if (!d.gf_selftest()) {
        if (err && err_len) snprintf(err, err_len, "v_perm GF(256) multiply mismatch");
        return -2;
    }
    return 0;
}

}
```

Before: 981.5.

## Replace per-element encoder window slots with run-length send-time runs and affine row pools

Replaces the per-element window ring (segment id plus send time) in the encoder with a run-length vector of send-time runs and a cursor-cached segment lookup, so appends no longer write one slot per original. Per-row lane opcode and coefficient computation is replaced by lookups in a precomputed global table. Input row vectors are dropped when the pool is affine, and row handles are computed from a base plus slot via a cursor. This aims to cut host-side bookkeeping per packet at the cost of extra search logic and possible vector inserts in the retransmit path.

```diff
diff --git a/tonk_amd/csrc/decoder.cpp b/tonk_amd/csrc/decoder.cpp
--- a/tonk_amd/csrc/decoder.cpp
+++ b/tonk_amd/csrc/decoder.cpp
@@ -122,11 +122,12 @@
             return;
         }
     }
+    auto row_at = [&](uint32_t x) { return layout ? rows[0] + x : rows[x]; };
     uint32_t j = 0;
     while (j < k) {
         Segment* last = segs_.empty() ? nullptr : &segs_.back();
         const uint32_t e_abs = e + base_;
-        const RowId r = rows[j];
+        const RowId r = row_at(j);
         const uint32_t off = rt.offset(r);
         const bool cont = last && last->end() == e_abs && last->bytes == framed_bytes &&
                           last->header_bytes == header_bytes && last->owned == owned && r == last->row0 + last->count &&
@@ -154,7 +155,7 @@
         col = col_inc(col);
         if (last->count >= 2) {
             uint32_t n = last->count;
-            while (j < k && rows[j] == last->row0 + n && col != 0 && rt.offset(rows[j]) == last->off(n)) {
+            while (j < k && row_at(j) == last->row0 + n && col != 0 && rt.offset(row_at(j)) == last->off(n)) {
                 subs_[e / kSubwindow]->seg[e % kSubwindow] = id;
                 ++e;
                 ++j;
@@ -1257,13 +1258,8 @@
         dpairs_.resize(keep);
         sort_pair_keys(dpairs_);
     }
-    uint64_t ops = 0;
-    uint8_t lk[kLanes][3];
-    for (unsigned l = 0; l < kLanes; ++l) {
-        const unsigned op = row_opcode(l, m.Row);
-        ops |= (uint64_t)op << (6 * l);
-        opcode_coefs(op, rx, lk[l]);
-    }
+    const uint64_t ops = g_gf.row_ops[m.Row];
+    const uint8_t (*lk)[3] = g_gf.row_lk[m.Row];
     const uint32_t split = ctx_->dense_split;
     const bool chunked = split && ee - sum_elem > split;
     ProgramBuilder& pb = ctx_->pb;
diff --git a/tonk_amd/csrc/encoder.cpp b/tonk_amd/csrc/encoder.cpp
--- a/tonk_amd/csrc/encoder.cpp
+++ b/tonk_amd/csrc/encoder.cpp
@@ -43,8 +43,63 @@
     held_ = 0;
     seg_base_ += (uint32_t)segs_.size();
     segs_.clear();
-    win_.clear();
+    times_.clear();
+    wsize_ = 0;
     base_ = 0;
+}
+
+size_t Encoder::time_index(uint32_t e) const {
+    const uint32_t a = base_ + e;
+    const size_t n = times_.size();
+    auto holds = [&](size_t i) {
+        return (int32_t)(a - times_[i].first) >= 0 && (i + 1 == n || (int32_t)(a - times_[i + 1].first) < 0);
+    };
+    size_t i = time_cur_;
+    if (i < n && holds(i)) return i;
+    if (++i < n && holds(i)) return time_cur_ = i;
+    size_t lo = 0, hi = n;
+    while (hi - lo > 1) {
+        const size_t mid = (lo + hi) / 2;
+        if ((int32_t)(a - times_[mid].first) >= 0) lo = mid;
+        else hi = mid;
+    }
+    return time_cur_ = lo;
+}
+
+void Encoder::push_time(uint32_t abs_first, uint32_t msec) {
+    if (times_.empty() || times_.back().msec != msec) times_.push_back(TimeRun{abs_first, msec});
+}
+
+void Encoder::set_msec(uint32_t e, uint32_t msec) {
+    size_t i = time_index(e);
+    if (times_[i].msec == msec) return;
+    const uint32_t a = base_ + e;
+    const uint32_t old = times_[i].msec;
+    const uint32_t end = i + 1 < times_.size() ? times_[i + 1].first : base_ + wsize_;
+    if ((int32_t)(a - times_[i].first) > 0) {
+        times_.insert(times_.begin() + (i + 1), TimeRun{a, msec});
+        ++i;
+    } else if (i > 0 && times_[i - 1].msec == msec) {
+        times_.erase(times_.begin() + i);
+        --i;
+    } else {
+        times_[i] = TimeRun{a, msec};
+    }
+    if (a + 1 != end) {
+        times_.insert(times_.begin() + (i + 1), TimeRun{a + 1, old});
+    } else if (i + 1 < times_.size() && times_[i + 1].msec == msec) {
+        times_.erase(times_.begin() + (i + 1));
+    }
+}
+
+uint32_t Encoder::longest_age(uint32_t lo, uint32_t hi, uint32_t now, uint32_t longest) const {
+    if (lo >= hi) return longest;
+    const uint32_t end = base_ + hi;
+    for (size_t i = time_index(lo); i < times_.size() && (int32_t)(times_[i].first - end) < 0; ++i) {
+        const int32_t d = (int32_t)(now - times_[i].msec);
+        if ((uint32_t)d > longest && d > 0) longest = (uint32_t)d;
+    }
+    return longest;
 }
 
 StoredOriginal Encoder::view(uint32_t e) const {
@@ -54,7 +109,7 @@
     o.row = s.row(j);
     o.bytes = s.bytes;
     o.column = to_column(e);
-    o.send_msec = win_[e].send_msec;
+    o.send_msec = msec_of(e);
     o.off = s.off(j);
     o.header_bytes = s.header_bytes;
     o.owned = s.owned;
@@ -71,12 +126,10 @@
 void Encoder::append(const RowId* rows, uint32_t k, uint32_t framed_bytes, uint32_t header_bytes, uint8_t owned,
                      void* host, uint32_t now, uint64_t layout) {
     const RowTable& rt = ctx_->rows;
-    uint32_t e_abs = base_ + (uint32_t)win_.size();
+    uint32_t e_abs = base_ + wsize_;
     uint32_t col = next_column_;
-    win_.reserve_more(k);
-    Slot* wb = win_.slot_base();
-    const size_t mask = win_.slot_mask();
-    size_t idx = win_.slot_index(win_.size());
+    push_time(e_abs, now);
+    wsize_ += k;
     if (k >= 2 && !host && col + k - 1 < kColumnPeriod && col != 0 && (layout || consecutive_handles(rows, k))) {
         const uint32_t o0 = layout ? (uint32_t)(layout >> 32) : rt.offset(rows[0]);
         const uint32_t o1 = layout ? o0 + (uint32_t)layout : rt.offset(rows[1]);
@@ -105,16 +158,14 @@
                 segs_.push_back(sg);
                 if (owned) ++held_;
             }
-            const Slot v{seg_base_ + (uint32_t)segs_.size() - 1, now};
-            for (uint32_t x = 0; x < k; ++x) wb[(idx + x) & mask] = v;
-            win_.commit(k);
             return;
         }
     }
+    auto row_at = [&](uint32_t x) { return layout ? rows[0] + x : rows[x]; };
     uint32_t j = 0;
     while (j < k) {
         Segment* last = segs_.empty() ? nullptr : &segs_.back();
-        const RowId r = rows[j];
+        const RowId r = row_at(j);
         const uint32_t off = rt.offset(r);
         const bool cont = last && !host && !last->host && last->row0 != kNoRow && last->end() == e_abs &&
                           last->bytes == framed_bytes && last->header_bytes == header_bytes && last->owned == owned &&
@@ -138,17 +189,12 @@
             if (owned || host) ++held_;
             last = &segs_.back();
         }
-        const uint32_t id = seg_base_ + (uint32_t)segs_.size() - 1;
-        wb[idx] = Slot{id, now};
-        idx = (idx + 1) & mask;
         ++e_abs;
         col = col_inc(col);
         ++j;
         if (last->count >= 2) {
             uint32_t n = last->count;
-            while (j < k && rows[j] == last->row0 + n && col != 0 && rt.offset(rows[j]) == last->off(n)) {
-                wb[idx] = Slot{id, now};
-                idx = (idx + 1) & mask;
+            while (j < k && row_at(j) == last->row0 + n && col != 0 && rt.offset(row_at(j)) == last->off(n)) {
                 ++n;
                 ++j;
                 col = col_inc(col);
@@ -157,7 +203,6 @@
             last->count = n;
         }
     }
-    win_.commit(k);
 }
 
 Result Encoder::add(RowId row, uint32_t framed_bytes, uint32_t header_bytes, uint32_t payload_bytes,
@@ -183,8 +228,8 @@
             ph.count = element;
             ph.column0 = column - element;
             segs_.push_back(ph);
-            for (uint32_t e = 0; e < element; ++e)
-                win_.push_back(Slot{seg_base_ + (uint32_t)segs_.size() - 1, placeholder_msec_[e]});
+            for (uint32_t e = 0; e < element; ++e) push_time(base_ + e, placeholder_msec_[e]);
+            wsize_ = element;
         }
     }
     append(&row, 1, framed_bytes, header_bytes, borrowed ? 0 : 1, host, now);
@@ -214,18 +259,21 @@
     count_ += m;
     const uint32_t first = next_column_;
     next_column_ = col_add(next_column_, m);
-    for (uint32_t j = 0; j < m && j < kLanes; ++j) {
-        Lane& lane = lanes_[(first + j) % kLanes];
-        if (lane.longest < framed_bytes) lane.longest = framed_bytes;
-    }
-    if (longest_ < framed_bytes) longest_ = framed_bytes;
+    if (framed_bytes > lanes_longest_min_) {
+        for (uint32_t j = 0; j < m && j < kLanes; ++j) {
+            Lane& lane = lanes_[(first + j) % kLanes];
+            if (lane.longest < framed_bytes) lane.longest = framed_bytes;
+        }
+        if (m >= kLanes) lanes_longest_min_ = framed_bytes;
+        if (longest_ < framed_bytes) longest_ = framed_bytes;
+    }
     stats_[0] += m;
     stats_[1] += (uint64_t)payload_bytes * m;
     return true;
 }
 
 void Encoder::start_new_window(uint32_t column) {
-    for (uint32_t e = 0; e < kLanes; ++e) placeholder_msec_[e] = e < win_.size() ? win_[e].send_msec : placeholder_msec_[e];
+    for (uint32_t e = 0; e < kLanes && e < wsize_; ++e) placeholder_msec_[e] = msec_of(e);
     ++window_gen_;
     drop_all();
     const uint32_t element = column % kLanes;
@@ -236,6 +284,7 @@
     count_ = element + 1;
     longest_ = 0;
     for (unsigned l = 0; l < kLanes; ++l) lanes_[l].longest = 0;
+    lanes_longest_min_ = 0;
 }
 
 void Encoder::remove_before(uint32_t first_kept_column) {
@@ -298,8 +347,11 @@
     }
 
     drop_segments_below(drop);
-    win_.pop_front(removed);
+    wsize_ -= removed;
     base_ = cut;
+    size_t gone = 0;
+    while (gone + 1 < times_.size() && (int32_t)(times_[gone + 1].first - base_) <= 0) ++gone;
+    if (gone) times_.erase(times_.begin(), times_.begin() + gone);
     count_ -= removed;
     column_start_ = to_column(removed);
     first_unremoved_ -= removed;
@@ -307,7 +359,7 @@
     uint32_t longest = 0, lane_longest[kLanes] = {0, 0, 0, 0, 0, 0, 0, 0};
     if (first_unremoved_ < count_) {
         const uint32_t lo = base_ + first_unremoved_, hi = base_ + count_;
-        for (uint32_t i = win_[first_unremoved_].seg - seg_base_; i < segs_.size(); ++i) {
+        for (size_t i = seg_index_at(lo); i < segs_.size(); ++i) {
             const Segment& sg = segs_[i];
             if (sg.first >= hi) break;
             const uint32_t a = sg.first > lo ? sg.first : lo, b = sg.end() < hi ? sg.end() : hi;
@@ -320,7 +372,11 @@
         }
     }
     longest_ = longest;
-    for (unsigned l = 0; l < kLanes; ++l) lanes_[l].longest = lane_longest[l];
+    lanes_longest_min_ = ~0u;
+    for (unsigned l = 0; l < kLanes; ++l) {
+        lanes_[l].longest = lane_longest[l];
+        if (lanes_longest_min_ > lane_longest[l]) lanes_longest_min_ = lane_longest[l];
+    }
 
     if (sum_end_ <= sum_start_) reset_sums(first_unremoved_);
 }
@@ -418,9 +474,9 @@
     uint32_t element = to_element(ack_.next_rto_column);
     if (element >= window_count) element = first_unremoved_;
 
-    for (; element < first_loss; ++element) {
-        const int32_t d = (int32_t)(now - win_[element].send_msec);
-        if ((uint32_t)d > longest && d > 0) longest = (uint32_t)d;
+    if (element < first_loss) {
+        longest = longest_age(element, first_loss, now, longest);
+        element = first_loss;
     }
 
     uint32_t remaining = ack_.data_bytes;
@@ -433,10 +489,10 @@
         remaining -= (uint32_t)n;
         if (element + 1 < first_loss) element = first_loss - 1;
         first_loss += rel;
-        for (; element < first_loss; ++element) {
-            if (element >= window_count) return;
-            const int32_t d = (int32_t)(now - win_[element].send_msec);
-            if ((uint32_t)d > longest && d > 0) longest = (uint32_t)d;
+        if (element < first_loss) {
+            if (first_loss > window_count) return;
+            longest = longest_age(element, first_loss, now, longest);
+            element = first_loss;
         }
         first_loss += lossM1 + 2;
     }
@@ -515,9 +571,8 @@
     if (ack_.found_oldest) {
         const uint32_t e = col_sub(ack_.oldest_column, column_start_);
         if (!col_delta_negative(e) && e >= first && e < count) {
-            Slot& o = win_[e];
-            if ((uint32_t)(now - o.send_msec) < rto) return kNeedMoreData;
-            o.send_msec = now;
+            if ((uint32_t)(now - msec_of(e)) < rto) return kNeedMoreData;
+            set_msec(e, now);
             ack_.found_oldest = false;
             return attempt_retransmit(e, out);
         }
@@ -526,9 +581,9 @@
 
     uint32_t nack_element = first;
     uint32_t oldest = nack_element;
-    uint32_t oldest_msec = win_[oldest].send_msec;
+    uint32_t oldest_msec = msec_of(oldest);
     if ((uint32_t)(now - oldest_msec) >= rto) {
-        win_[oldest].send_msec = now;
+        set_msec(oldest, now);
         return attempt_retransmit(oldest, out);
     }
 
@@ -538,10 +593,9 @@
         while (next_loss_column(column)) {
             nack_element = to_element(column);
             if (nack_element >= count) break;
-            Slot& o = win_[nack_element];
-            const uint32_t last = o.send_msec;
+            const uint32_t last = msec_of(nack_element);
             if ((uint32_t)(now - last) >= rto) {
-                o.send_msec = now;
+                set_msec(nack_element, now);
                 return attempt_retransmit(nack_element, out);
             }
             if ((int32_t)(oldest_msec - last) > 0) { oldest = nack_element; oldest_msec = last; }
@@ -549,10 +603,9 @@
     }
 
     for (uint32_t e = nack_element + 1; e < count; ++e) {
-        Slot& o = win_[e];
-        const uint32_t last = o.send_msec;
+        const uint32_t last = msec_of(e);
         if ((uint32_t)(now - last) >= rto) {
-            o.send_msec = now;
+            set_msec(e, now);
             return attempt_retransmit(e, out);
         }
         if ((int32_t)(oldest_msec - last) > 0) { oldest = e; oldest_msec = last; }
@@ -626,7 +679,7 @@
     uint32_t used = 0;
     {
         const uint32_t lo = base_ + first, hi = base_ + count_;
-        for (uint32_t i = win_[first].seg - seg_base_; i < segs_.size(); ++i) {
+        for (size_t i = seg_index_at(lo); i < segs_.size(); ++i) {
             const Segment& sg = segs_[i];
             if (sg.first >= hi) break;
             const uint32_t a = sg.first > lo ? sg.first : lo, b = sg.end() < hi ? sg.end() : hi;
@@ -757,8 +810,7 @@
     }
     DenseTarget& t = dgrp_[dgrp_n_];
     t.row = out.row;
-    t.ops = 0;
-    for (unsigned l = 0; l < kLanes; ++l) t.ops |= (uint64_t)row_opcode(l, row) << (6 * l);
+    t.ops = g_gf.row_ops[row];
     t.rx = row_value(row);
     t.hi = hi - lo;
     t.flen = out.footer_len;
diff --git a/tonk_amd/csrc/encoder.h b/tonk_amd/csrc/encoder.h
--- a/tonk_amd/csrc/encoder.h
+++ b/tonk_amd/csrc/encoder.h
@@ -118,23 +118,42 @@
     const uint64_t* clock_ = nullptr;
     uint64_t now_msec() const;
 
-    struct Slot { uint32_t seg, send_msec; };
-    Ring<Slot> win_;
     Ring<Segment> segs_;
     uint32_t seg_base_ = 0;
     uint32_t base_ = 0;
-    const Segment& seg_of(uint32_t e) const { return segs_[win_[e].seg - seg_base_]; }
+    uint32_t wsize_ = 0;
+    struct TimeRun { uint32_t first, msec; };
+    std::vector<TimeRun> times_;
+    mutable size_t time_cur_ = 0;
+    mutable size_t seg_cur_ = 0;
+    size_t time_index(uint32_t e) const;
+    uint32_t msec_of(uint32_t e) const { return times_[time_index(e)].msec; }
+    void set_msec(uint32_t e, uint32_t msec);
+    void push_time(uint32_t abs_first, uint32_t msec);
+    uint32_t longest_age(uint32_t lo, uint32_t hi, uint32_t now, uint32_t longest) const;
+    size_t seg_index_at(uint32_t a) const {
+        const size_t n = segs_.size();
+        size_t i = seg_cur_;
+        if (i < n && a - segs_[i].first < segs_[i].count) return i;
+        if (++i < n && a - segs_[i].first < segs_[i].count) return seg_cur_ = i;
+        size_t lo = 0, hi = n;
+        if (n && (int32_t)(a - segs_[0].first) >= 0 && a - segs_[0].first < n) {
+            hi = a - segs_[0].first + 1;
+            if ((int32_t)(a - segs_[hi - 1].first) >= 0) return seg_cur_ = hi - 1;
+        }
+        while (hi - lo > 1) {
+            const size_t mid = (lo + hi) / 2;
+            if ((int32_t)(a - segs_[mid].first) >= 0) lo = mid;
+            else hi = mid;
+        }
+        return seg_cur_ = lo;
+    }
+    const Segment& seg_of(uint32_t e) const { return segs_[seg_index_at(base_ + e)]; }
     RowId row_of(uint32_t e) const {
         const Segment& s = seg_of(e);
         return s.row(e + base_ - s.first);
     }
     StoredOriginal view(uint32_t e) const;
-    size_t seg_index_at(uint32_t a) const {
-        if ((int32_t)(a - base_) >= 0) return win_[a - base_].seg - seg_base_;
-        size_t i = 0;
-        while (i + 1 < segs_.size() && (int32_t)(segs_[i].end() - a) <= 0) ++i;
-        return i;
-    }
     uint32_t sum_abs_start() const { return base_ + sum_start_ - sum_erased_; }
     void append(const RowId* rows, uint32_t k, uint32_t framed_bytes, uint32_t header_bytes, uint8_t owned,
                 void* host, uint32_t now,
@@ -145,6 +164,7 @@
     uint32_t placeholder_msec_[8] = {0, 0, 0, 0, 0, 0, 0, 0};
     uint32_t next_column_ = 0, count_ = 0, column_start_ = 0, longest_ = 0;
     uint32_t held_ = 0;
+    uint32_t lanes_longest_min_ = 0;
     uint32_t first_unremoved_ = 0;
     uint32_t sum_start_ = 0, sum_end_ = 0, sum_column_start_ = 0, sum_erased_ = 0;
     struct Lane {
@@ -173,7 +193,7 @@
     int debug_state(char* buf, size_t n) const {
         const uint32_t now = (uint32_t)now_msec();
         const uint32_t first = col_sub(ack_.next_expected, column_start_);
-        const uint32_t age = first < count_ && first < win_.size() ? now - win_[first].send_msec : 0;
+        const uint32_t age = first < count_ && first < wsize_ ? now - msec_of(first) : 0;
         return snprintf(buf, n,
                         "count=%u first_unremoved=%u next_column=%u column_start=%u ack_next=%u ack_bytes=%u "
                         "rto=%u found_oldest=%d first_age_ms=%u disabled=%d",
diff --git a/tonk_amd/csrc/engine.h b/tonk_amd/csrc/engine.h
--- a/tonk_amd/csrc/engine.h
+++ b/tonk_amd/csrc/engine.h
@@ -368,10 +368,6 @@
 };
 
 inline uint8_t sum_coef(unsigned s, uint8_t cx) { return s == 0 ? 1 : (s == 1 ? cx : gf_sqr(cx)); }
-inline void opcode_coefs(unsigned op, uint8_t rx, uint8_t* c) {
-    for (unsigned s = 0; s < 3; ++s)
-        c[s] = (uint8_t)(((op >> s) & 1u) ^ (((op >> (s + 3)) & 1u) ? rx : 0u));
-}
 
 class ExpansionTable {
 public:
diff --git a/tonk_amd/csrc/gf256.cpp b/tonk_amd/csrc/gf256.cpp
--- a/tonk_amd/csrc/gf256.cpp
+++ b/tonk_amd/csrc/gf256.cpp
@@ -65,6 +65,14 @@
         g_gf.perm[c][6] = 0;
         g_gf.perm[c][7] = 0;
     }
+    for (unsigned row = 0; row < 256; ++row) {
+        g_gf.row_ops[row] = 0;
+        for (unsigned l = 0; l < kLanes; ++l) {
+            const unsigned op = row_opcode(l, row);
+            g_gf.row_ops[row] |= (uint64_t)op << (6 * l);
+            opcode_coefs(op, row_value(row), g_gf.row_lk[row][l]);
+        }
+    }
     g_gf.ready = self_test();
     return g_gf.ready;
 }
diff --git a/tonk_amd/csrc/gf256.h b/tonk_amd/csrc/gf256.h
--- a/tonk_amd/csrc/gf256.h
+++ b/tonk_amd/csrc/gf256.h
@@ -9,6 +9,8 @@
     uint8_t inv[256];
     uint8_t sqr[256];
     uint32_t perm[256][8];
+    uint64_t row_ops[256];
+    uint8_t row_lk[256][8][3];
     bool ready = false;
 };
 
@@ -50,6 +52,11 @@
     return op == 0 ? 16u : op;
 }
 
+inline void opcode_coefs(unsigned op, uint8_t rx, uint8_t* c) {
+    for (unsigned s = 0; s < 3; ++s)
+        c[s] = (uint8_t)(((op >> s) & 1u) ^ (((op >> (s + 3)) & 1u) ? rx : 0u));
+}
+
 inline uint8_t cauchy_element(unsigned row, unsigned column) {
     return gf_inv((uint8_t)((uint8_t)column ^ (uint8_t)(row + kCauchyMaxColumns)));
 }
diff --git a/tonk_amd/csrc/resident_backend.h b/tonk_amd/csrc/resident_backend.h
--- a/tonk_amd/csrc/resident_backend.h
+++ b/tonk_amd/csrc/resident_backend.h
@@ -15,45 +15,85 @@
     Context* ctx = nullptr;
     std::unique_ptr<Encoder> enc;
     std::unique_ptr<Decoder> dec;
-    std::vector<RowId> enc_rows, dec_rows;
     uint32_t pool = 0;
     bool pool_affine = false;
     uint32_t pool_off[2] = {0, 0}, pool_stride = 0;
+    RowId pool_row0[2] = {kNoRow, kNoRow};
+    std::vector<RowId> rows_[2];
+    uint32_t pool_mask = 0;
+    struct Cursor { uint32_t index = ~0u, slot = 0; } cur_[2];
+    RowId run_rows_[2];
+    std::vector<RowId> run_scratch_;
     bool nobatch = false;
     bool contig = true;
     uint64_t alg_bytes = 0, payload_bytes = 0;
     std::vector<RecoveredPacket*> got_;
 
     bool alloc_inputs(uint32_t n, uint32_t pool_n, uint32_t row_bytes) {
-        enc_rows.assign(n, kNoRow);
-        dec_rows.assign(n, kNoRow);
         for (int side = 0; side < 2; ++side) {
-            std::vector<RowId>& rows = side ? dec_rows : enc_rows;
+            std::vector<RowId>& rows = rows_[side];
+            rows.assign(pool_n, kNoRow);
             for (uint32_t i = 0; i < pool_n; ++i)
                 if ((rows[i] = ctx->alloc(row_bytes)) == kNoRow) return false;
-            for (uint32_t i = pool_n; i < n; ++i) rows[i] = rows[i - pool_n];
         }
         pool = pool_n;
+        pool_mask = pool && !(pool & (pool - 1)) ? pool - 1 : 0;
         pool_affine = pool >= 2;
         for (int side = 0; side < 2 && pool_affine; ++side) {
-            const std::vector<RowId>& rows = side ? dec_rows : enc_rows;
+            const std::vector<RowId>& rows = rows_[side];
             const uint32_t o0 = ctx->rows.offset(rows[0]), stride = ctx->rows.offset(rows[1]) - o0;
             pool_affine = consecutive_handles(rows.data(), pool) && stride > 0 &&
                           ctx->rows.affine(rows[0], pool, stride) && (!side || stride == pool_stride);
             pool_off[side] = o0;
+            pool_row0[side] = rows[0];
             pool_stride = stride;
+        }
+        for (int side = 0; side < 2; ++side) {
+            std::vector<RowId>& rows = rows_[side];
+            if (pool_affine) {
+                std::vector<RowId>().swap(rows);
+            } else {
+                rows.resize(n);
+                for (uint32_t i = pool_n; i < n; ++i) rows[i] = rows[i - pool_n];
+            }
         }
         return true;
     }
-    uint64_t layout(int side, uint32_t index, uint32_t k) const {
-        if (!pool_affine || !contig || index % pool + k > pool) return 0;
-        return (uint64_t)(pool_off[side] + (index % pool) * pool_stride) << 32 | pool_stride;
+    RowId row(int side, uint32_t index) const {
+        if (!pool_affine) return rows_[side][index];
+        return pool_row0[side] + (pool_mask ? index & pool_mask : index % pool);
+    }
+    uint32_t pool_slot(int side, uint32_t index, uint32_t k) {
+        if (pool_mask) return index & pool_mask;
+        Cursor& c = cur_[side];
+        const uint32_t slot = c.index == index ? c.slot : index % pool;
+        c.index = index + k;
+        c.slot = slot + k;
+        if (c.slot >= pool) c.slot = c.slot - pool < pool ? c.slot - pool : c.slot % pool;
+        return slot;
+    }
+    const RowId* run_rows(int side, uint32_t index, uint32_t k, uint64_t* layout) {
+        *layout = 0;
+        if (!pool_affine) return &rows_[side][index];
+        const uint32_t slot = pool_slot(side, index, k);
+        if (contig && slot + k <= pool) {
+            *layout = (uint64_t)(pool_off[side] + slot * pool_stride) << 32 | pool_stride;
+            run_rows_[0] = pool_row0[side] + slot;
+            run_rows_[1] = run_rows_[0] + 1;
+            return run_rows_;
+        }
+        run_scratch_.resize(k);
+        for (uint32_t j = 0, m = slot; j < k; ++j) {
+            run_scratch_[j] = pool_row0[side] + m;
+            if (++m == pool) m = 0;
+        }
+        return run_scratch_.data();
     }
 
     int enc_add(uint32_t index, uint32_t len, uint32_t* col) {
         const uint32_t hb = length_header_bytes(len);
         TAMD_PROF_SCOPE(kEncAdd);
-        const Result r = enc->add(enc_rows[index], hb + len, hb, len, nullptr, col, true);
+        const Result r = enc->add(row(0, index), hb + len, hb, len, nullptr, col, true);
         if (r == kSuccess) {
             alg_bytes += hb + len;
             payload_bytes += len;
@@ -64,7 +104,9 @@
         if (nobatch) return false;
         const uint32_t hb = length_header_bytes(len);
         TAMD_PROF_SCOPE(kEncAdd);
-        if (!enc->add_run(&enc_rows[index], k, hb + len, hb, len, true, col0, layout(0, index, k))) return false;
+        uint64_t layout;
+        const RowId* rows = run_rows(0, index, k, &layout);
+        if (!enc->add_run(rows, k, hb + len, hb, len, true, col0, layout)) return false;
         alg_bytes += (uint64_t)(hb + len) * k;
         payload_bytes += (uint64_t)len * k;
         return true;
@@ -73,7 +115,9 @@
         if (nobatch) return false;
         const uint32_t hb = length_header_bytes(len);
         TAMD_PROF_SCOPE(kDecAddOrig);
-        if (!dec->add_run_inorder(col0, &dec_rows[index], k, hb + len, hb, len, true, layout(1, index, k))) return false;
+        uint64_t layout;
+        const RowId* rows = run_rows(1, index, k, &layout);
+        if (!dec->add_run_inorder(col0, rows, k, hb + len, hb, len, true, layout)) return false;
         alg_bytes += (uint64_t)(hb + len) * k;
         return true;
     }
@@ -92,7 +136,7 @@
         const uint32_t hb = length_header_bytes(len);
         TAMD_PROF_SCOPE(kDecAddOrig);
         bool took = false;
-        const Result r = dec->add_original(col, dec_rows[index], hb + len, hb, len, nullptr, &took, true);
+        const Result r = dec->add_original(col, row(1, index), hb + len, hb, len, nullptr, &took, true);
         alg_bytes += hb + len;
         return r;
     }
diff --git a/tonk_amd/csrc/ring.h b/tonk_amd/csrc/ring.h
--- a/tonk_amd/csrc/ring.h
+++ b/tonk_amd/csrc/ring.h
@@ -18,17 +18,6 @@
         if (n_ == buf_.size()) grow();
         buf_[(head_ + n_) & mask_] = v;
         ++n_;
-    }
-    void reserve_more(size_t k) {
-        while (n_ + k > buf_.size()) grow();
-    }
-    T* slot_base() { return buf_.data(); }
-    size_t slot_index(size_t i) const { return (head_ + i) & mask_; }
-    size_t slot_mask() const { return mask_; }
-    void commit(size_t k) { n_ += k; }
-    T& push_slot() {
-        if (n_ == buf_.size()) grow();
-        return buf_[(head_ + n_++) & mask_];
     }
     void pop_front(size_t k) {
         if (k > n_) k = n_;
diff --git a/tonk_amd/csrc/session.cpp b/tonk_amd/csrc/session.cpp
--- a/tonk_amd/csrc/session.cpp
+++ b/tonk_amd/csrc/session.cpp
@@ -775,7 +775,7 @@
             if (!n) continue;
             for (int side = 0; side < 2; ++side) {
                 if (!((prm.stage_host >> side) & 1u)) continue;
-                const RowId r = (side ? st.dec_rows : st.enc_rows)[next];
+                const RowId r = st.row(side, next);
                 const uint8_t* src = host_in + (2 * i + side) * side_bytes + (size_t)next * row_cap;
                 dev.h2d((uint64_t)st.ctx->rows.offset(r) * TAMD_ROW_UNIT, src, (size_t)n * row_cap);
                 h2d_bytes += (uint64_t)n * row_cap;
@@ -960,7 +960,7 @@
         d.reserve(2 * (size_t)pool);
         for (int side = 0; side < 2; ++side)
             for (uint32_t i = 0; i < pool; ++i) {
-                const RowId r = (side ? st.dec_rows : st.enc_rows)[i];
+                const RowId r = st.row(side, i);
                 Device::GenDesc g;
                 g.row = st.ctx->rows.offset(r);
                 g.index = i;
@@ -994,10 +994,9 @@
             Stream& st = *s->streams[i];
             st.stage = s->prm.stage_host & 3u;
             for (int side = 0; side < 2; ++side) {
-                const std::vector<RowId>& rows = side ? st.dec_rows : st.enc_rows;
-                const uint64_t base = st.ctx->rows.offset(rows[0]);
+                const uint64_t base = st.ctx->rows.offset(st.row(side, 0));
                 for (uint32_t k = 0; k < st.p.n_originals; ++k)
-                    if (st.ctx->rows.offset(rows[k]) != base + (uint64_t)k * (s->row_cap / TAMD_ROW_UNIT)) {
+                    if (st.ctx->rows.offset(st.row(side, k)) != base + (uint64_t)k * (s->row_cap / TAMD_ROW_UNIT)) {
                         s->error = "input rows are not contiguous";
                         return -3;
                     }
```

Measured after the change: 1044, median of 6. 1.06x the previous value.
